# jingsenzhu/i2-sdf

Hardware: AMD Instinct MI355X
Metric: ray-samples/sec (fwd+bwd) (higher is better)
Workload: dtype f32 (bf16x3 split MFMA: fp32 operands as 3 bf16 terms, fp32 accumulate; the 256x256 weight-gradient GEMM blocks and the sampler's depth-choosing sdf-only passes: 2 bf16 terms per operand, 3 products, fp32 accumulate; the saved SDF tensors abar / G(hbar) / G(a) -- operands of those GEMMs and of the s

## Files before the change

i2sdf_amd/csrc/mlp_fwd.hip:

```cpp
#include "epi.h"
#include "mlp_args.h"

using namespace i2sdf;

int i2sdf_hip_check(hipError_t e, const char* what);
void i2sdf_launch_sdf_fwd3(int H, const float* stream, int n_stages, int L, int skip, const PointSpec& ps, const int* skip_flag, int64_t M,
                           float* sdf_out, unsigned grid, hipStream_t st);

void i2sdf_launch_sdf_fwd3h(const float* stream, int n_stages, int L, int skip, const PointSpec& ps, const int* skip_flag, int64_t M, float* sdf_out,
                            int planes, hipStream_t st);

namespace {

template <int H, int F, int LF, bool FULL>
__global__ __launch_bounds__(256) void sdf_fwd_kernel(const float* __restrict__ stream, int n_stages, int L, int skip, PointSpec ps,
                                                       const int* __restrict__ skip_flag, int64_t M, float* __restrict__ sdf_out,
                                                       float* __restrict__ feat_out, int64_t ld_feat) {
  constexpr int NT = H / 32, KC = H / 8, PEC = PE<LF>::PEC;
  extern __shared__ __attribute__((aligned(16))) float lds[];
  if (skip_flag != nullptr && skip_flag[0] != 0) return;
  const int tid = threadIdx.x, lane = tid & 63, wave = tid >> 6, hi = lane >> 5;
  const int64_t m = ((int64_t)blockIdx.x * 4 + wave) * 32 + (lane & 31);
  const bool valid = m < M;
  const int64_t mc = valid ? m : M - 1;
  float px, py, pz;
  fetch_point(ps, mc, px, py, pz);
  float pe[PEC * 4];
  {
    float full[PEC * 8];
    pe_full<LF>(px, py, pz, full);
    to_b_layout<PEC>(full, pe, hi);
  }
  WStream ws;
  ws.begin(stream, lds, n_stages, tid);
  f32x16 acc[NT];
  float h[NT * 16];
  SoftplusEpi sp{nullptr, hi, valid};
  dense_op_epi<NT, PEC, NT * 4, 0, 0, SoftplusEpi>(ws, pe, acc, sp, tid);
  commit_tiles<NT>(acc, h);
  for (int l = 1; l < L - 1; ++l) {
    if (l == skip) {
      constexpr float rs2 = RS2;
      float u[(KC + PEC) * 4];
#pragma unroll
      for (int i = 0; i < KC * 4; ++i) u[i] = h[i] * rs2;
#pragma unroll
      for (int i = 0; i < PEC * 4; ++i) u[KC * 4 + i] = pe[i] * rs2;
      dense_op_epi<NT, KC + PEC, NT * 4, 0, 0, SoftplusEpi>(ws, u, acc, sp, tid);
    } else {
      dense_op_epi<NT, KC, NT * 4, 0, 0, SoftplusEpi>(ws, h, acc, sp, tid);
    }
    commit_tiles<NT>(acc, h);
  }
  float s[1];
  rowvec_op<1, KC>(ws, h, s, tid);
  if (sdf_out != nullptr && valid && hi == 0) sdf_out[m] = s[0];
  if (FULL) {
    constexpr int FT = F / 32;
    f32x16 fa[FT];
    dense_op<FT, KC, 0>(ws, h, fa, tid);
    store_tile<FT>(feat_out + mc * ld_feat, hi, valid, fa);
  }
}

template <int H, int F, int LF>
int launch_sdf_fwd(const i2sdf_plan* p, const float* packed, PointSpec points, const int* skip_flag, int64_t M, float* sdf_out,
                   float* feat_out, int64_t ld_feat, hipStream_t st, bool sampler_pass = false) {
  const i2sdf_mlp_desc& d = p->sdf.d;
  const bool full = feat_out != nullptr;
  const unsigned grid = (unsigned)((M + PTS_PER_WG - 1) / PTS_PER_WG);
  if (!full && sdf_out != nullptr && p->sdf_fwd_bf16x3 && H == 256 && span_chunks(p->sdf, SPAN_FWD3H) > 0) {
    const int PL = (sampler_pass && p->sampler_bf16x2 && span_chunks(p->sdf, SPAN_FWD2H) > 0) ? 2 : 3;
    const Span s3 = span(p, packed, p->sdf, PL == 2 ? SPAN_FWD2H : SPAN_FWD3H_SDF);
    if (!s3.n_stages) return I2SDF_EINVAL;
    i2sdf_launch_sdf_fwd3h(s3.w, s3.n_stages, d.n_lin, d.skip_layer, points, skip_flag, M, sdf_out, PL, st);
    return i2sdf_hip_check(hipGetLastError(), "sdf_forward (bf16x3, 16-point waves) launch");
  }
  if (!full && sdf_out != nullptr && p->sdf_fwd_bf16x3 && H == 64 && span_chunks(p->sdf, SPAN_FWD3) > 0) {
    const Span s3 = span(p, packed, p->sdf, SPAN_FWD3);
    if (!s3.n_stages) return I2SDF_EINVAL;
    i2sdf_launch_sdf_fwd3(H, s3.w, s3.n_stages, d.n_lin, d.skip_layer, points, skip_flag, M, sdf_out, grid, st);
    return i2sdf_hip_check(hipGetLastError(), "sdf_forward (bf16x3) launch");
  }
  if (full && p->sdf_fwd_bf16x3 && H == 256 && F == 256 && span_chunks(p->sdf, SPAN_FWD3H) > 0) {
    const Span s3 = span(p, packed, p->sdf, SPAN_FWD3H);
    if (!s3.n_stages || skip_flag != nullptr) return I2SDF_EINVAL;
    SdfTrainFwdArgs a{};
    a.fwd = s3.w; a.n_fwd = s3.n_stages;
    a.L = d.n_lin; a.skip = d.skip_layer; a.pts = points; a.M = M; a.Mp = M; a.sdf = sdf_out; a.feat = feat_out; a.ldf = ld_feat;
    i2sdf_launch_train_fwd3h(a, grid, st);
    return i2sdf_hip_check(hipGetLastError(), "sdf_forward (features, bf16x3, 16-point waves) launch");
  }
  const Span s = span(p, packed, p->sdf, full ? SPAN_FWD : SPAN_FWD_SDF);
  if (!s.n_stages) return I2SDF_EINVAL;
  if (full)
    launch_lds(sdf_fwd_kernel<H, F, LF, true>, grid, st, s.w, s.n_stages, d.n_lin, d.skip_layer, points, skip_flag, M, sdf_out, feat_out, ld_feat);
  else
    launch_lds(sdf_fwd_kernel<H, F, LF, false>, grid, st, s.w, s.n_stages, d.n_lin, d.skip_layer, points, skip_flag, M, sdf_out, nullptr, 0);
  return i2sdf_hip_check(hipGetLastError(), "sdf_forward launch");
}

}

extern "C" int i2sdf_sdf_forward(const i2sdf_plan* p, const float* packed, const float* points, int64_t M, float* sdf_out,
                                 float* feat_out, int64_t ld_feat, void* stream) {
  if (M == 0) return I2SDF_OK;
  if (!p || !packed || !points || M < 0) return I2SDF_EINVAL;
  if (feat_out && (ld_feat < p->F || ld_feat % 4)) return I2SDF_EINVAL;
  hipStream_t st = (hipStream_t)stream;
  if (p->sdf.d.multires != 6) return I2SDF_EINVAL;
  const PointSpec ps{points, nullptr, nullptr, nullptr, 0, 0, 1};
  if (p->H == 256 && p->F == 256) return launch_sdf_fwd<256, 256, 6>(p, packed, ps, nullptr, M, sdf_out, feat_out, ld_feat, st);
  if (p->H == 64 && p->F == 64) return launch_sdf_fwd<64, 64, 6>(p, packed, ps, nullptr, M, sdf_out, feat_out, ld_feat, st);
  return I2SDF_EINVAL;
}

int i2sdf_sdf_forward_rays_flagged(const i2sdf_plan* p, const float* packed, const float* cam, const float* dirs, const float* z, int64_t ldz,
                                   int32_t n_per_ray, int64_t B, float* sdf_out, const int* skip_flag, void* stream) {
  if (p->sdf.d.multires != 6) return I2SDF_EINVAL;
  const int64_t M = B * n_per_ray;
  const PointSpec ps{nullptr, cam, dirs, z, ldz, M, n_per_ray};
  hipStream_t st = (hipStream_t)stream;
  if (p->H == 256 && p->F == 256) return launch_sdf_fwd<256, 256, 6>(p, packed, ps, skip_flag, M, sdf_out, nullptr, 0, st, true);
  if (p->H == 64 && p->F == 64) return launch_sdf_fwd<64, 64, 6>(p, packed, ps, skip_flag, M, sdf_out, nullptr, 0, st, true);
  return I2SDF_EINVAL;
}
```

i2sdf_amd/csrc/pack.hip:

```cpp
#include "plan.h"

using namespace i2sdf;

int i2sdf_hip_check(hipError_t e, const char* what);

namespace {

struct RowTab {
  int32_t n;
  int32_t rows[3 * I2SDF_MAX_LAYERS], cols[3 * I2SDF_MAX_LAYERS], scale_off[3 * I2SDF_MAX_LAYERS];
  int64_t off_v[3 * I2SDF_MAX_LAYERS], off_g[3 * I2SDF_MAX_LAYERS];
};

__global__ __launch_bounds__(256) void rowscale_kernel(RowTab tab, const float* __restrict__ params, float* __restrict__ scale,
                                                        int n_rows) {
  const int row = blockIdx.x * 4 + (threadIdx.x >> 6);
  const int lane = threadIdx.x & 63;
  if (row >= n_rows) return;
  int e = 0;
  while (e + 1 < tab.n && row >= tab.scale_off[e + 1]) ++e;
  const int r = row - tab.scale_off[e];
  const int cols = tab.cols[e];
  const float* v = params + tab.off_v[e] + (int64_t)r * cols;
  float s = 0.f;
  for (int c = lane; c < cols; c += 64) { float x = v[c]; s = fmaf(x, x, s); }
#pragma unroll
  for (int o = 32; o > 0; o >>= 1) s += __shfl_xor(s, o);
  if (lane == 0) scale[row] = params[tab.off_g[e] + r] / sqrtf(s);
}

__device__ __forceinline__ int map_col(const ColMap& cm, int kp) {
  if (kp < cm.split) return kp < cm.valid0 ? cm.base0 + kp : -1;
  const int j = kp - cm.split;
  return j < cm.valid1 ? cm.base1 + j : -1;
}

__global__ __launch_bounds__(256) void pack_kernel(const Seg* __restrict__ segs, int n_segs, const float* __restrict__ params,
                                                    const float* __restrict__ scale, float* __restrict__ chunks,
                                                    int64_t total_chunks) {
  const int64_t gid = (int64_t)blockIdx.x * 256 + threadIdx.x;
  const int64_t chunk = gid >> 6;
  const int lane = (int)(gid & 63);
  if (chunk >= total_chunks) return;
  int lo = 0, hi_ = n_segs - 1;
  while (lo < hi_) {
    const int mid = (lo + hi_ + 1) >> 1;
    if (segs[mid].chunk0 <= chunk) lo = mid; else hi_ = mid - 1;
  }
  const Seg s = segs[lo];
  const int c = (int)(chunk - s.chunk0);
  const int i32 = lane & 31, hi = lane >> 5;
  f32x4 out = {0.f, 0.f, 0.f, 0.f};
  if (c < s.used) {
    if (s.type == SEG_BIAS) {
      const int nt = c / 4, q = c % 4;
#pragma unroll
      for (int t = 0; t < 4; ++t) {
        const int r = 32 * nt + 8 * q + 4 * hi + t;
        out[t] = (r < s.nrows) ? params[s.off_bias + s.row_off + r] : 0.f;
      }
    } else if (s.type == SEG_WFWD) {
      const int nt = c / s.KC, kc = c % s.KC;
      const int r = 32 * nt + i32;
      if (r < s.nrows) {
        const int row = s.row_off + r;
        const float sc = scale[s.scale_off + row] * s.mult;
        const float* v = params + s.off_v + (int64_t)row * s.cols;
#pragma unroll
        for (int t = 0; t < 4; ++t) {
          const int col = map_col(s.cm, 8 * kc + 4 * hi + t);
          out[t] = col >= 0 ? v[col] * sc : 0.f;
        }
      }
    } else if (s.type == SEG_WFWD3) {
      const int G = s.NT / 2, w = c >> 1, e = c & 1;
      const int kc = w / (3 * G), g = (w / 3) % G, sp = w % 3;
      const int r = 32 * (2 * g + e) + i32;
      unsigned q[4] = {0u, 0u, 0u, 0u};
      if (r < s.nrows) {
        const int row = s.row_off + r;
        const float sc = scale[s.scale_off + row] * s.mult;
        const float* v = params + s.off_v + (int64_t)row * s.cols;
#pragma unroll
        for (int i = 0; i < 4; ++i) {
          float x[2];
#pragma unroll
          for (int h2 = 0; h2 < 2; ++h2) {
            const int j = 2 * i + h2;
            const int col = map_col(s.cm, 16 * kc + (j & 3) + 8 * (j >> 2) + 4 * hi);
            x[h2] = col >= 0 ? v[col] * sc : 0.f;
          }
          unsigned p0, p1, p2;
          split3_pair(x[0], x[1], p0, p1, p2);
          q[i] = sp == 0 ? p0 : (sp == 1 ? p1 : p2);
        }
      }
      out = __builtin_bit_cast(f32x4, u32x4{q[0], q[1], q[2], q[3]});
    } else if (s.type == SEG_WBWD3) {
      const int G = s.NT / 2, w = c >> 1, e = c & 1;
      const int kc = w / (3 * G), g = (w / 3) % G, sp = w % 3;
      const int col = map_col(s.cm, 32 * (2 * g + e) + i32);
      unsigned q[4] = {0u, 0u, 0u, 0u};
      if (col >= 0) {
#pragma unroll
        for (int i = 0; i < 4; ++i) {
          float x[2];
#pragma unroll
          for (int h2 = 0; h2 < 2; ++h2) {
            const int j = 2 * i + h2;
            const int r = 16 * kc + (j & 3) + 8 * (j >> 2) + 4 * hi;
            x[h2] = 0.f;
            if (r < s.nrows) {
              const int row = s.row_off + r;
              x[h2] = params[s.off_v + (int64_t)row * s.cols + col] * scale[s.scale_off + row] * s.mult;
            }
          }
          unsigned p0, p1, p2;
          split3_pair(x[0], x[1], p0, p1, p2);
          q[i] = sp == 0 ? p0 : (sp == 1 ? p1 : p2);
        }
      }
      out = __builtin_bit_cast(f32x4, u32x4{q[0], q[1], q[2], q[3]});
    } else if (s.type == SEG_BIAS_H) {
      const int kg = lane >> 4;
#pragma unroll
      for (int t = 0; t < 4; ++t) {
        const int r = 16 * c + 4 * kg + t;
        out[t] = (r < s.nrows) ? params[s.off_bias + s.row_off + r] : 0.f;
      }
    } else if (s.type == SEG_WFWD3H || s.type == SEG_WBWD3H || s.type == SEG_WFWD2H) {
      const int G = s.NT / 2, w = c >> 1, e = c & 1, PL = s.type == SEG_WFWD2H ? 2 : 3;
      const int kc = w / (PL * G), g = (w / PL) % G, sp = w % PL;
      const int i16 = lane & 15, kg = lane >> 4;
      const int arow = 16 * (2 * g + e) + i16;
      const bool fwd = s.type != SEG_WBWD3H;
      const int acol = fwd ? -1 : map_col(s.cm, arow);
      unsigned q[4] = {0u, 0u, 0u, 0u};
      if (fwd ? (arow < s.nrows) : (acol >= 0)) {
#pragma unroll
        for (int i = 0; i < 4; ++i) {
          float x[2];
#pragma unroll
          for (int h2 = 0; h2 < 2; ++h2) {
            const int j = 2 * i + h2;
            const int k = 32 * kc + 16 * (j >> 2) + 4 * kg + (j & 3);
            x[h2] = 0.f;
            if (fwd) {
              const int row = s.row_off + arow, col = map_col(s.cm, k);
              if (col >= 0) x[h2] = params[s.off_v + (int64_t)row * s.cols + col] * (scale[s.scale_off + row] * s.mult);
            } else if (k < s.nrows) {
              const int row = s.row_off + k;
              x[h2] = params[s.off_v + (int64_t)row * s.cols + acol] * scale[s.scale_off + row] * s.mult;
            }
          }
          unsigned p0, p1, p2;
          split3_pair(x[0], x[1], p0, p1, p2);
          q[i] = sp == 0 ? p0 : (sp == 1 ? p1 : p2);
        }
      }
      out = __builtin_bit_cast(f32x4, u32x4{q[0], q[1], q[2], q[3]});
    } else if (s.type == SEG_ROWVEC_H) {
      const int rr = c / s.KC, nt = c % s.KC, kg = lane >> 4;
      const int row = s.row_off + rr;
      const float sc = scale[s.scale_off + row] * s.mult;
#pragma unroll
      for (int t = 0; t < 4; ++t) {
        const int col = map_col(s.cm, 16 * nt + 4 * kg + t);
        out[t] = col >= 0 ? params[s.off_v + (int64_t)row * s.cols + col] * sc : 0.f;
      }
    } else if (s.type == SEG_WBWD) {
      const int kt = c / s.KC, nc = c % s.KC;
      const int col = map_col(s.cm, 32 * kt + i32);
      if (col >= 0) {
#pragma unroll
        for (int t = 0; t < 4; ++t) {
          const int r = 8 * nc + 4 * hi + t;
          if (r < s.nrows) {
            const int row = s.row_off + r;
            out[t] = params[s.off_v + (int64_t)row * s.cols + col] * scale[s.scale_off + row] * s.mult;
          }
        }
      }
    } else if (s.type == SEG_ROWVEC) {
      const int rr = c / s.KC, kc = c % s.KC;
      const int row = s.row_off + rr;
      const float sc = scale[s.scale_off + row] * s.mult;
#pragma unroll
      for (int t = 0; t < 4; ++t) {
        const int col = map_col(s.cm, 8 * kc + 4 * hi + t);
        out[t] = col >= 0 ? params[s.off_v + (int64_t)row * s.cols + col] * sc : 0.f;
      }
    } else if (s.type == SEG_SCALAR) {
#pragma unroll
      for (int t = 0; t < 4; ++t) out[t] = (t < s.nrows) ? params[s.off_bias + s.row_off + t] : 0.f;
    }
  }
  reinterpret_cast<f32x4*>(chunks)[chunk * 64 + lane] = out;
}

void fill_tab(RowTab& tab, const NetPlan& np) {
  for (int l = 0; l < np.d.n_lin; ++l) {
    const int e = tab.n++;
    tab.rows[e] = np.d.out_dim[l]; tab.cols[e] = np.d.in_dim[l]; tab.scale_off[e] = np.scale_off[l];
    tab.off_v[e] = np.d.off_v[l]; tab.off_g[e] = np.d.off_g[l];
  }
}

}

extern "C" int i2sdf_pack_weights(const i2sdf_plan* p, const float* params, float* packed, void* stream) {
  if (!p || !params || !packed) return I2SDF_EINVAL;
  if (!p->d_segs) return I2SDF_EHIP;
  hipStream_t st = (hipStream_t)stream;
  RowTab tab{};
  fill_tab(tab, p->sdf); fill_tab(tab, p->rgb);
  if (p->light.d.n_lin) fill_tab(tab, p->light);
  rowscale_kernel<<<cdiv(p->n_scale, 4), 256, 0, st>>>(tab, params, packed, p->n_scale);
  const int64_t threads = p->total_chunks * 64;
  pack_kernel<<<(unsigned)((threads + 255) / 256), 256, 0, st>>>(p->d_segs, p->n_segs, params, packed, packed + p->scale_floats,
                                                                 p->total_chunks);
  return i2sdf_hip_check(hipGetLastError(), "pack_weights launch");
}
```

i2sdf_amd/csrc/plan.h:

```cpp
#pragma once
#include <stdint.h>
#include <vector>
#include "../../include/i2sdf.h"
#include "x3h.h"

namespace i2sdf {

enum SegType : int32_t { SEG_ZERO = 0, SEG_BIAS = 1, SEG_WFWD = 2, SEG_WBWD = 3, SEG_ROWVEC = 4, SEG_SCALAR = 5,
                         SEG_WFWD3 = 6 ,
                         SEG_WBWD3 = 7 ,
                         SEG_BIAS_H = 8, SEG_WFWD3H = 9, SEG_WBWD3H = 10, SEG_ROWVEC_H = 11,
                         SEG_WFWD2H = 12  };

struct ColMap { int32_t split, base0, valid0, base1, valid1; };

struct Seg {
  int64_t chunk0;
  int32_t nchunks;
  int32_t type;
  int64_t off_v, off_bias;
  int32_t scale_off;
  int32_t rows, cols;
  int32_t row_off;
  int32_t nrows;
  int32_t NT, KC;
  int32_t used;
  ColMap cm;
  float mult;
};

enum Mark : int {
  FWD, FWD_HIDDEN_END, FWD_SDF_END, FWD_END,
  REV, REV_CHAIN, REV_W0, REV_END,
  FWD3, FWD3_HIDDEN_END, FWD3_END,
  REV3, REV3_CHAIN, REV3_W0, REV3_END,
  FWD3H, FWD3H_SDF_END, FWD3H_END,
  REV3H, REV3H_END,
  FWD2H, FWD2H_END,
  N_MARKS
};
struct SpanId { Mark from, to; int stage_chunks; };
constexpr SpanId SPAN_FWD_HIDDEN{FWD, FWD_HIDDEN_END, SC};
constexpr SpanId SPAN_FWD_SDF{FWD, FWD_SDF_END, SC};
constexpr SpanId SPAN_FWD{FWD, FWD_END, SC};
constexpr SpanId SPAN_REV_SWEEP2{REV, REV_W0, SC};
constexpr SpanId SPAN_REV_CHAIN{REV_CHAIN, REV_END, SC};
constexpr SpanId SPAN_REV{REV, REV_END, SC};
constexpr SpanId SPAN_FWD3_HIDDEN{FWD3, FWD3_HIDDEN_END, SC};
constexpr SpanId SPAN_FWD3{FWD3, FWD3_END, SC};
constexpr SpanId SPAN_REV3_SWEEP2{REV3, REV3_W0, SC};
constexpr SpanId SPAN_REV3_CHAIN{REV3_CHAIN, REV3_END, SC};
constexpr SpanId SPAN_FWD3H_SDF{FWD3H, FWD3H_SDF_END, SCH};
constexpr SpanId SPAN_FWD3H{FWD3H, FWD3H_END, SCH};
constexpr SpanId SPAN_REV3H{REV3H, REV3H_END, SCH};
constexpr SpanId SPAN_FWD2H{FWD2H, FWD2H_END, SCH};

struct NetPlan {
  i2sdf_mlp_desc d;
  int32_t scale_off[I2SDF_MAX_LAYERS];
  int64_t mark[N_MARKS] = {};
  int64_t wgrad_off[I2SDF_MAX_LAYERS];
  int32_t wg_rows[I2SDF_MAX_LAYERS], wg_cols[I2SDF_MAX_LAYERS];
};

}

struct i2sdf_plan {
  i2sdf_net_desc desc;
  i2sdf::NetPlan sdf, rgb, light;
  std::vector<i2sdf::Seg> segs;
  i2sdf::Seg* d_segs = nullptr;
  int32_t n_segs = 0;
  int32_t n_scale = 0;
  int64_t scale_floats = 0;
  int64_t total_chunks = 0;
  int64_t wgrad_floats = 0;
  int32_t H = 0, F = 0;
  int32_t n_cu = 256;
  int32_t rgb_bf16x3 = 0;
  int32_t sdf_bwd_bf16x3 = 0;
  int32_t train_fwd_bf16x3 = 0;
  int32_t wgrad_bf16x3 = 0;
  int32_t sdf_fwd_bf16x3 = 0;
  int32_t sampler_bf16x2 = 0;
  i2sdf_exchange exchange{nullptr, nullptr};
  int32_t dp_flags = 0;
  int32_t wgrad_bf16x2 = 0;
  int32_t blocked_saves = 0;
  int32_t saves24 = 0;
  int32_t tail_overlap = 0;
  mutable hipStream_t side = nullptr;
  mutable hipEvent_t ev_fork = nullptr, ev_join = nullptr;
  int32_t parts = 0;
  mutable hipStream_t part_st[I2SDF_MAX_PARTS - 1] = {nullptr, nullptr, nullptr};
  mutable hipEvent_t part_ev[I2SDF_MAX_PARTS] = {nullptr, nullptr, nullptr, nullptr};
  mutable int32_t chain_active = 0;
  mutable int64_t chain_M = 0;
};

namespace i2sdf {
struct Span { const float* w = nullptr; int n_stages = 0; };
inline int64_t span_chunks(const NetPlan& np, SpanId id) { return np.mark[id.to] - np.mark[id.from]; }
inline Span span(const i2sdf_plan* p, const float* packed, const NetPlan& np, SpanId id) {
  const int64_t n = span_chunks(np, id);
  if (n <= 0 || n % id.stage_chunks) return Span{};
  return Span{packed + p->scale_floats + np.mark[id.from] * CHUNK_FLOATS, (int)(n / id.stage_chunks)};
}
}

struct PartRun {
  int n = 1;
  hipStream_t st[I2SDF_MAX_PARTS];
  int64_t lo[I2SDF_MAX_PARTS], hi[I2SDF_MAX_PARTS];
  bool own = false;
};
bool i2sdf_parts_begin(const i2sdf_plan* p, hipStream_t st, int64_t M, PartRun* pr);
void i2sdf_parts_end(const i2sdf_plan* p, hipStream_t st, PartRun* pr);
void i2sdf_parts_join_all(const i2sdf_plan* p, hipStream_t st);
void i2sdf_parts_fence(const i2sdf_plan* p, hipStream_t st);
#ifndef I2SDF_WG_CH
#define I2SDF_WG_CH 2048
#endif
inline bool i2sdf_parts_on(const i2sdf_plan* p) { return p->parts >= 2; }
struct ChainGuard {
  const i2sdf_plan* p; hipStream_t st; bool on;
  ChainGuard(const i2sdf_plan* p_, hipStream_t st_, bool ranged) : p(p_), st(st_), on(!ranged && p_->chain_active != 0) {
    if (on) i2sdf_parts_join_all(p, st);
  }
  ~ChainGuard() { if (on) i2sdf_parts_fence(p, st); }
};

hipStream_t i2sdf_tail_fork(const i2sdf_plan* p, hipStream_t st);
void i2sdf_tail_join(const i2sdf_plan* p, hipStream_t st, hipStream_t side);

inline int64_t split_bulk_points(int64_t M, int n_cu) {
  const int64_t n_wg = (M + i2sdf::PTS_PER_WG - 1) / i2sdf::PTS_PER_WG;
  const int64_t full = (n_wg / n_cu) * n_cu, rem = n_wg - full;
  if (full == 0 || rem == 0 || rem * 4 > n_cu) return 0;
  if ((full * i2sdf::PTS_PER_WG) % I2SDF_WG_CH != 0) return 0;
  return full * i2sdf::PTS_PER_WG;
}

enum TailOrder { TAIL_FORKED, TAIL_BEHIND };
template <class Full, class Tail>
inline void i2sdf_dispatch_points(const i2sdf_plan* p, hipStream_t st, int64_t M, bool ranged, bool may_split, TailOrder order, Full full, Tail tail) {
  constexpr int64_t WG = i2sdf::PTS_PER_WG;
  if (ranged) {
    PartRun pr;
    i2sdf_parts_begin(p, st, M, &pr);
    for (int q = 0; q < pr.n; ++q)
      if (pr.hi[q] > pr.lo[q]) full(pr.st[q], (int)(pr.lo[q] / WG), (unsigned)((pr.hi[q] - pr.lo[q] + WG - 1) / WG), M);
    i2sdf_parts_end(p, st, &pr);
    return;
  }
  const int64_t bulk = may_split ? split_bulk_points(M, p->n_cu) : 0;
  if (bulk == 0) {
    full(st, 0, (unsigned)((M + WG - 1) / WG), M);
  } else if (order == TAIL_FORKED) {
    hipStream_t ts = i2sdf_tail_fork(p, st);
    tail(ts, bulk);
    full(st, 0, (unsigned)(bulk / WG), bulk);
    i2sdf_tail_join(p, st, ts);
  } else {
    full(st, 0, (unsigned)(bulk / WG), bulk);
    tail(st, bulk);
  }
}
```

i2sdf_amd/csrc/sampler.hip:

```cpp
#include "plan.h"

using namespace i2sdf;

int i2sdf_hip_check(hipError_t e, const char* what);

namespace {

constexpr int NMAX = 640;
constexpr int NNEW = 128;
constexpr int EMAX = NMAX / 64;

enum { ST_DONE = 0, ST_ITERS = 1, ST_FLAG0 = 2 , ST_CNT0 = 16 , ST_WORDS = 32 };

#ifndef SAMPLER_DPP
#define SAMPLER_DPP 1
#endif
template <int CTRL, int ROW_MASK>
__device__ __forceinline__ float dpp_mov(float old, float v) {
  return __builtin_bit_cast(float, __builtin_amdgcn_update_dpp(__builtin_bit_cast(int, old), __builtin_bit_cast(int, v), CTRL, ROW_MASK, 0xf, false));
}
constexpr int DPP_ROW_SHR1 = 0x111, DPP_ROW_SHR2 = 0x112, DPP_ROW_SHR4 = 0x114, DPP_ROW_SHR8 = 0x118, DPP_ROW_BCAST15 = 0x142, DPP_ROW_BCAST31 = 0x143;
__device__ __forceinline__ float wscan_incl(float v, int lane) {
#if SAMPLER_DPP
  (void)lane;
  v += dpp_mov<DPP_ROW_SHR1, 0xf>(0.f, v);
  v += dpp_mov<DPP_ROW_SHR2, 0xf>(0.f, v);
  v += dpp_mov<DPP_ROW_SHR4, 0xf>(0.f, v);
  v += dpp_mov<DPP_ROW_SHR8, 0xf>(0.f, v);
  v += dpp_mov<DPP_ROW_BCAST15, 0xa>(0.f, v);
  v += dpp_mov<DPP_ROW_BCAST31, 0xc>(0.f, v);
  return v;
#else
#pragma unroll
  for (int o = 1; o < 64; o <<= 1) {
    const float t = __shfl_up(v, o);
    if (lane >= o) v += t;
  }
  return v;
#endif
}
__device__ __forceinline__ float wsum(float v) {
#if SAMPLER_DPP
  return __builtin_bit_cast(float, __builtin_amdgcn_readlane(__builtin_bit_cast(int, wscan_incl(v, 0)), 63));
#else
#pragma unroll
  for (int o = 32; o > 0; o >>= 1) v += __shfl_xor(v, o);
  return v;
#endif
}
__device__ __forceinline__ float wmax(float v) {
#if SAMPLER_DPP
  const float lo = -3.4028234663852886e38f;
  v = fmaxf(v, dpp_mov<DPP_ROW_SHR1, 0xf>(lo, v));
  v = fmaxf(v, dpp_mov<DPP_ROW_SHR2, 0xf>(lo, v));
  v = fmaxf(v, dpp_mov<DPP_ROW_SHR4, 0xf>(lo, v));
  v = fmaxf(v, dpp_mov<DPP_ROW_SHR8, 0xf>(lo, v));
  v = fmaxf(v, dpp_mov<DPP_ROW_BCAST15, 0xa>(lo, v));
  v = fmaxf(v, dpp_mov<DPP_ROW_BCAST31, 0xc>(lo, v));
  return __builtin_bit_cast(float, __builtin_amdgcn_readlane(__builtin_bit_cast(int, v), 63));
#else
#pragma unroll
  for (int o = 32; o > 0; o >>= 1) v = fmaxf(v, __shfl_xor(v, o));
  return v;
#endif
}
template <int E>
__device__ __forceinline__ void row_scan_incl(float (&v)[E], int lane) {
#pragma unroll
  for (int e = 1; e < E; ++e) v[e] += v[e - 1];
  const float tot = v[E - 1];
  const float pre = wscan_incl(tot, lane) - tot;
#pragma unroll
  for (int e = 0; e < E; ++e) v[e] += pre;
}

__device__ __forceinline__ float laplace_density(float s, float inv_beta) {
  const float e = expm1f(-fabsf(s) * inv_beta);
  const float sg = (s > 0.f) ? 1.f : ((s < 0.f) ? -1.f : 0.f);
  return inv_beta * (0.5f + 0.5f * sg * e);
}

template <int E>
struct Row {
  float z[E], s[E];
  float a[E], ds[E];
  int n;
};

template <int E>
__device__ __forceinline__ void row_intervals(Row<E>& r, int lane) {
  const float zn_next = __shfl_down(r.z[0], 1), sn_next = __shfl_down(r.s[0], 1);
#pragma unroll
  for (int e = 0; e < E; ++e) {
    const int j = lane * E + e;
    const float z1 = (e + 1 < E) ? r.z[(e + 1 < E) ? e + 1 : e] : zn_next;
    const float s1 = (e + 1 < E) ? r.s[(e + 1 < E) ? e + 1 : e] : sn_next;
    float a = 0.f, d = 0.f;
    if (j < r.n - 1) {
      a = z1 - r.z[e];
      const float b = fabsf(r.s[e]), c = fabsf(s1);
      const bool first = a * a + b * b <= c * c;
      const bool second = a * a + c * c <= b * b;
      const float sp = (a + b + c) / 2.0f;
      const float area = sp * (sp - a) * (sp - b) * (sp - c);
      const bool mask = !first && !second && (b + c - a > 0.f);
      float h = (2.0f * sqrtf(area)) / a;
      if (!(h == h)) h = 0.f;
      else if (h > 3.4028234663852886e38f) h = 3.4028234663852886e38f;
      else if (h < -3.4028234663852886e38f) h = -3.4028234663852886e38f;
      d = ((first && !second) ? b : 0.f) + (second ? c : 0.f) + (mask ? h : 0.f);
      const float sg0 = (r.s[e] > 0.f) ? 1.f : ((r.s[e] < 0.f) ? -1.f : 0.f);
      const float sg1 = (s1 > 0.f) ? 1.f : ((s1 < 0.f) ? -1.f : 0.f);
      if (!(sg0 * sg1 == 1.f)) d = 0.f;
    }
    r.a[e] = a; r.ds[e] = d;
  }
}

template <int E>
__device__ __forceinline__ float row_error_bound(const Row<E>& r, float beta, int lane) {
  const float ib = 1.0f / beta;
  float fe[E], er[E];
#pragma unroll
  for (int e = 0; e < E; ++e) {
    const int j = lane * E + e;
    const bool ok = j < r.n - 1;
    fe[e] = ok ? r.a[e] * laplace_density(r.s[e], ib) : 0.f;
    er[e] = ok ? expf(-r.ds[e] / beta) * (r.a[e] * r.a[e]) / (4.0f * beta * beta) : 0.f;
  }
  float fi[E], ei[E];
#pragma unroll
  for (int e = 0; e < E; ++e) { fi[e] = fe[e]; ei[e] = er[e]; }
  row_scan_incl<E>(fi, lane);
  row_scan_incl<E>(ei, lane);
  float mx = -3.4e38f;
#pragma unroll
  for (int e = 0; e < E; ++e) {
    const int j = lane * E + e;
    if (j < r.n - 1) {
      const float integ = fi[e] - fe[e];
      const float bo = (fminf(expf(ei[e]), 1.0e6f) - 1.0f) * expf(-integ);
      mx = fmaxf(mx, bo);
    }
  }
  return wmax(mx);
}

struct SamplerArgs {
  int64_t B;
  int it, n, n_new;
  int N_eval, N_final, max_iters, beta_iters, force_iters;
  float eps, add_tiny, near, far;
  const float* beta_param; float beta_min;
  int* state;
  float* z_cur; float* z_nxt;
  float* sdf_prev; float* sdf_cur;
  const int* idx;
  int* idx_nxt;
  const float* sdf_new;
  float* samples;
  float* beta;
  const float* u_more; const float* u_final; int64_t ldu_final;
};

template <int E>
__device__ __forceinline__ void load_row(Row<E>& r, const float* z, const float* s, int n, int lane) {
  r.n = n;
#pragma unroll
  for (int e = 0; e < E; ++e) {
    const int j = lane * E + e;
    r.z[e] = (j < n) ? z[j] : 3.0e38f;
    r.s[e] = (j < n) ? s[j] : 0.f;
  }
}

template <int E>
__device__ __forceinline__ float beta_step(const SamplerArgs& a, Row<E>& r, int64_t rc, bool active, int lane) {
  const float beta0 = fabsf(a.beta_param[0]) + a.beta_min;
  const int n = a.n;
  float* sc = a.sdf_cur + rc * NMAX;
  const float* zc = a.z_cur + rc * NMAX;
  r.n = n;
  {
    const int n_old = n - a.n_new;
    const int* ix = a.idx + rc * NMAX;
    const float* sp = a.sdf_prev + rc * NMAX;
    const float* sn = a.sdf_new + rc * a.n_new;
#pragma unroll
    for (int e = 0; e < E; ++e) {
      const int j = lane * E + e;
      float sv = 0.f, zv = 3.0e38f;
      if (j < n) {
        zv = zc[j];
        if (a.it == 0) sv = sn[j];
        else { const int k = ix[j]; sv = (k < n_old) ? sp[k] : sn[k - n_old]; }
        if (active) sc[j] = sv;
      }
      r.z[e] = zv; r.s[e] = sv;
    }
  }
  row_intervals<E>(r, lane);
  float beta = a.beta[rc];
  const float err0 = row_error_bound<E>(r, beta0, lane);
  if (err0 <= a.eps) beta = beta0;
  float bmin = beta0, bmax = beta;
  for (int k = 0; k < a.beta_iters; ++k) {
    const float bmid = (bmin + bmax) / 2.0f;
    const float err = row_error_bound<E>(r, bmid, lane);
    if (err <= a.eps) bmax = bmid; else bmin = bmid;
  }
  return bmax;
}
template <int E>
__global__ __launch_bounds__(256) void sampler_beta_kernel(SamplerArgs a) {
  if (a.state[ST_DONE]) return;
  const int lane = threadIdx.x & 63;
  const int64_t ray = (int64_t)blockIdx.x * 4 + (threadIdx.x >> 6);
  if (ray >= a.B) return;
  Row<E> r;
  const float beta = beta_step<E>(a, r, ray, true, lane);
  if (lane == 0) {
    a.beta[ray] = beta;
    if (beta > fabsf(a.beta_param[0]) + a.beta_min) atomicOr(&a.state[ST_FLAG0 + a.it], 1);
  }
}

template <int E>
__device__ __forceinline__ void resample_step(const SamplerArgs& a, const Row<E>& r, float beta, bool more, int64_t ray, int64_t rc, bool active,
                                              float (&s_cdf)[4][NMAX + 1], float (&s_z)[4][NMAX], float (&s_new)[4][NNEW], int lane, int wv) {
  const int n = a.n;
  const float ib = 1.0f / beta;
  float fe[E], cum[E];
#pragma unroll
  for (int e = 0; e < E; ++e) {
    const int j = lane * E + e;
    const float dist = (j < n - 1) ? r.a[e] : 1.0e10f;
    fe[e] = (j < n) ? dist * laplace_density(r.s[e], ib) : 0.f;
    cum[e] = (j < n - 1) ? fe[e] : 0.f;
  }
  row_scan_incl<E>(cum, lane);
  float pdf[E];
  if (more) {
    float er[E];
#pragma unroll
    for (int e = 0; e < E; ++e) {
      const int j = lane * E + e;
      er[e] = (j < n - 1) ? expf(-r.ds[e] / beta) * (r.a[e] * r.a[e]) / (4.0f * beta * beta) : 0.f;
    }
    row_scan_incl<E>(er, lane);
#pragma unroll
    for (int e = 0; e < E; ++e) {
      const int j = lane * E + e;
      const float T = expf(-(cum[e] - ((j < n - 1) ? fe[e] : 0.f)));
      pdf[e] = (j < n - 1) ? (fminf(expf(er[e]), 1.0e6f) - 1.0f) * T + a.add_tiny : 0.f;
    }
  } else {
#pragma unroll
    for (int e = 0; e < E; ++e) {
      const int j = lane * E + e;
      const float T = expf(-(cum[e] - ((j < n - 1) ? fe[e] : 0.f)));
      const float w = (1.0f - expf(-fe[e])) * T;
      pdf[e] = (j < n - 1) ? w + 1e-5f : 0.f;
    }
  }
  float tot = 0.f;
#pragma unroll
  for (int e = 0; e < E; ++e) tot += pdf[e];
  tot = wsum(tot);
  float cd[E];
#pragma unroll
  for (int e = 0; e < E; ++e) { pdf[e] = pdf[e] / tot; cd[e] = pdf[e]; }
  row_scan_incl<E>(cd, lane);
#pragma unroll
  for (int e = 0; e < E; ++e) {
    const int j = lane * E + e;
    if (j < n) { s_cdf[wv][j] = cd[e] - pdf[e]; s_z[wv][j] = r.z[e]; }
  }
  __syncthreads();
  const int N = more ? a.N_eval : a.N_final;
  for (int k = lane; k < N; k += 64) {
    float u;
    if (more) u = a.u_more[k];
    else u = a.u_final[rc * a.ldu_final + k];
    int lo = 0, hi = n;
    while (lo < hi) {
      const int mid = (lo + hi) >> 1;
      if (s_cdf[wv][mid] <= u) lo = mid + 1; else hi = mid;
    }
    const int below = (lo - 1 > 0) ? lo - 1 : 0;
    const int above = (lo < n - 1) ? lo : n - 1;
    const float c0 = s_cdf[wv][below], c1 = s_cdf[wv][above];
    const float b0 = s_z[wv][below], b1 = s_z[wv][above];
    float denom = c1 - c0;
    if (denom < 1e-5f) denom = 1.0f;
    const float t = (u - c0) / denom;
    const float smp = b0 + t * (b1 - b0);
    s_new[wv][k] = smp;
    if (active) a.samples[ray * NNEW + k] = smp;
  }
  __syncthreads();
  if (!more) return;
  if (active) {
    float* zn = a.z_nxt + ray * NMAX;
    int* ixn = a.idx_nxt + ray * NMAX;
    for (int j = lane; j < n; j += 64) {
      const float v = s_z[wv][j];
      int lo = 0, hi = N;
      while (lo < hi) { const int mid = (lo + hi) >> 1; if (s_new[wv][mid] < v) lo = mid + 1; else hi = mid; }
      zn[j + lo] = v; ixn[j + lo] = j;
    }
    for (int k = lane; k < N; k += 64) {
      const float v = s_new[wv][k];
      int lo = 0, hi = n;
      while (lo < hi) { const int mid = (lo + hi) >> 1; if (s_z[wv][mid] <= v) lo = mid + 1; else hi = mid; }
      zn[k + lo] = v; ixn[k + lo] = n + k;
    }
  }
}

__device__ __forceinline__ void iteration_done(const SamplerArgs& a, bool more) {
  __syncthreads();
  if (threadIdx.x == 0) {
    __threadfence();
    const int c = atomicAdd(&a.state[ST_CNT0 + a.it], 1);
    if (c == (int)gridDim.x - 1 && !more) { a.state[ST_ITERS] = a.it + 1; __threadfence(); a.state[ST_DONE] = 1; }
  }
}

template <int E>
__global__ __launch_bounds__(256) void sampler_resample_kernel(SamplerArgs a) {
  __shared__ float s_cdf[4][NMAX + 1];
  __shared__ float s_z[4][NMAX];
  __shared__ float s_new[4][NNEW];
  if (a.state[ST_DONE]) return;
  const int lane = threadIdx.x & 63, wv = threadIdx.x >> 6;
  const int64_t ray = (int64_t)blockIdx.x * 4 + wv;
  const bool active = ray < a.B;
  const int64_t rc = active ? ray : a.B - 1;
  bool not_conv = a.state[ST_FLAG0 + a.it] != 0;
  if (a.force_iters > 0) not_conv = (a.it + 1) < a.force_iters;
  const bool more = not_conv && (a.it + 1 < a.max_iters);
  Row<E> r;
  load_row<E>(r, a.z_cur + rc * NMAX, a.sdf_cur + rc * NMAX, a.n, lane);
  row_intervals<E>(r, lane);
  resample_step<E>(a, r, a.beta[rc], more, ray, rc, active, s_cdf, s_z, s_new, lane, wv);
  iteration_done(a, more);
}

template <int E>
__global__ __launch_bounds__(256) void sampler_iter_fixed_kernel(SamplerArgs a) {
  __shared__ float s_cdf[4][NMAX + 1];
  __shared__ float s_z[4][NMAX];
  __shared__ float s_new[4][NNEW];
  const int lane = threadIdx.x & 63, wv = threadIdx.x >> 6;
  const int64_t ray = (int64_t)blockIdx.x * 4 + wv;
  const bool active = ray < a.B;
  const int64_t rc = active ? ray : a.B - 1;
  const bool more = ((a.it + 1) < a.force_iters) && (a.it + 1 < a.max_iters);
  Row<E> r;
  const float beta = beta_step<E>(a, r, rc, active, lane);
  if (active && lane == 0) a.beta[ray] = beta;
  resample_step<E>(a, r, beta, more, ray, rc, active, s_cdf, s_z, s_new, lane, wv);
  iteration_done(a, more);
}

__global__ __launch_bounds__(256) void sampler_init_kernel(int64_t B, int N, const float* __restrict__ t_lin, const float* __restrict__ strat_u,
                                                            float near, float far, float eps, float* __restrict__ z_cur,
                                                            float* __restrict__ samples, float* __restrict__ beta, int* __restrict__ state) {
  const int lane = threadIdx.x & 63;
  const int64_t ray = (int64_t)blockIdx.x * 4 + (threadIdx.x >> 6);
  if (blockIdx.x == 0 && threadIdx.x < ST_WORDS) state[threadIdx.x] = 0;
  if (ray >= B) return;
  float acc = 0.f, carry = 0.f;
  for (int base = 0; base < N; base += 64) {
    const int j = base + lane;
    float z = 0.f;
    if (j < N) {
      const float t = t_lin[j];
      z = near * (1.0f - t) + far * t;
      if (strat_u) {
        const float tm = t_lin[j > 0 ? j - 1 : 0], tp = t_lin[j < N - 1 ? j + 1 : N - 1];
        const float zm = near * (1.0f - tm) + far * tm, zq = near * (1.0f - tp) + far * tp;
        const float lower = (j > 0) ? 0.5f * (z + zm) : z;
        const float upper = (j < N - 1) ? 0.5f * (zq + z) : z;
        z = lower + (upper - lower) * strat_u[ray * N + j];
      }
      z_cur[ray * NMAX + j] = z;
      samples[ray * NNEW + j] = z;
    }
    float zp = __shfl_up(z, 1);
    if (lane == 0) zp = carry;
    if (j < N && j > 0) { const float d = z - zp; acc = fmaf(d, d, acc); }
    carry = __shfl(z, 63);
  }
  acc = wsum(acc);
  if (lane == 0) beta[ray] = sqrtf((1.0f / (4.0f * logf(eps + 1.0f))) * acc);
}

__global__ __launch_bounds__(256) void sampler_final_kernel(int64_t B, const int* __restrict__ state, int N_eval, const float* z_a,
                                                             const float* z_b, const float* __restrict__ samples, int N_final, int N_extra,
                                                             const int* __restrict__ extra_idx, const int* __restrict__ extra_tab,
                                                             float near, float far, const int* __restrict__ eik_idx, float* __restrict__ z_out,
                                                             int64_t ldz, float* __restrict__ z_eik, int* __restrict__ iters_out) {
  __shared__ float buf[4][256];
  const int lane = threadIdx.x & 63, wv = threadIdx.x >> 6;
  const int64_t ray = (int64_t)blockIdx.x * 4 + wv;
  const bool active = ray < B;
  const int64_t rc = active ? ray : B - 1;
  const int iters = state[ST_ITERS];
  if (iters_out != nullptr && blockIdx.x == 0 && threadIdx.x == 0) iters_out[0] = iters;
  const int n_row = N_eval * iters;
  const float* zr = ((iters & 1) ? z_a : z_b) + rc * NMAX;
  const int total = N_final + 2 + N_extra;
  for (int k = lane; k < 256; k += 64) {
    float v = 3.0e38f;
    if (k < N_final) v = samples[rc * NNEW + k];
    else if (k == N_final) v = near;
    else if (k == N_final + 1) v = far;
    else if (k < total) {
      const int e = k - N_final - 2;
      int id;
      if (extra_idx) id = extra_idx[(iters - 1) * N_extra + e];
      else id = extra_tab[(iters - 1) * N_extra + e];
      id = id < 0 ? 0 : (id > n_row - 1 ? n_row - 1 : id);
      v = zr[id];
    }
    buf[wv][k] = v;
  }
  __syncthreads();
  for (int k = 2; k <= 256; k <<= 1) {
    for (int j = k >> 1; j > 0; j >>= 1) {
      for (int i = lane; i < 256; i += 64) {
        const int l = i ^ j;
        if (l > i) {
          const float x = buf[wv][i], y = buf[wv][l];
          const bool up = (i & k) == 0;
          if ((x > y) == up) { buf[wv][i] = y; buf[wv][l] = x; }
        }
      }
      __syncthreads();
    }
  }
  if (active) {
    for (int k = lane; k < total; k += 64) z_out[ray * ldz + k] = buf[wv][k];
    if (lane == 0 && z_eik) {
      int id = eik_idx ? eik_idx[ray] : 0;
      id = id < 0 ? 0 : (id > total - 1 ? total - 1 : id);
      z_eik[ray] = buf[wv][id];
    }
  }
}

template <int E>
__global__ __launch_bounds__(256) void error_bound_kernel(int64_t B, int n, const float* __restrict__ z, const float* __restrict__ sdf,
                                                           const float* __restrict__ beta, int64_t ldbeta, const float* __restrict__ d_star_in,
                                                           float* __restrict__ d_star_out, float* __restrict__ bound) {
  const int lane = threadIdx.x & 63;
  const int64_t ray = (int64_t)blockIdx.x * 4 + (threadIdx.x >> 6);
  if (ray >= B) return;
  Row<E> r;
  load_row<E>(r, z + ray * n, sdf + ray * n, n, lane);
  row_intervals<E>(r, lane);
#pragma unroll
  for (int e = 0; e < E; ++e) {
    const int j = lane * E + e;
    if (j < n - 1) {
      if (d_star_in) r.ds[e] = d_star_in[ray * (n - 1) + j];
      if (d_star_out) d_star_out[ray * (n - 1) + j] = r.ds[e];
    }
  }
  if (bound) {
    const float eb = row_error_bound<E>(r, beta[ray * ldbeta], lane);
    if (lane == 0) bound[ray] = eb;
  }
}

template <int E>
int launch_iter(const SamplerArgs& a, hipStream_t st, const i2sdf_exchange* ex) {
  const unsigned grid = (unsigned)((a.B + 3) / 4);
  if (a.force_iters > 0 && !ex) {
    sampler_iter_fixed_kernel<E><<<grid, 256, 0, st>>>(a);
    return I2SDF_OK;
  }
  sampler_beta_kernel<E><<<grid, 256, 0, st>>>(a);
  if (ex) {
    const int rc = ex->allreduce(ex->ctx, a.state + ST_FLAG0 + a.it, 1, I2SDF_XCHG_I32, I2SDF_XCHG_MAX, (void*)st);
    if (rc) return rc;
  }
  sampler_resample_kernel<E><<<grid, 256, 0, st>>>(a);
  return I2SDF_OK;
}

}

extern "C" int64_t i2sdf_sampler_workspace_floats(int64_t B) {
  return B * (int64_t)(NMAX * 6 + NNEW * 2 + 1) + ST_WORDS + 64;
}

extern "C" int i2sdf_error_bound(const float* z, const float* sdf, int64_t B, int32_t n, const float* beta, int64_t ldbeta,
                                 const float* d_star_in, float* d_star_out, float* bound, void* stream) {
  if (B == 0) return I2SDF_OK;
  if (!z || !sdf || B < 0 || n < 2 || n > NMAX || (bound && !beta) || (!bound && !d_star_out) || (ldbeta != 0 && ldbeta != 1)) return I2SDF_EINVAL;
  hipStream_t st = (hipStream_t)stream;
  const unsigned grid = (unsigned)((B + 3) / 4);
#define I2SDF_EB(E_) error_bound_kernel<E_><<<grid, 256, 0, st>>>(B, n, z, sdf, beta, ldbeta, d_star_in, d_star_out, bound)
  switch (cdiv(n, 64)) {
    case 1: I2SDF_EB(1); break;
    case 2: I2SDF_EB(2); break;
    case 3: I2SDF_EB(3); break;
    case 4: I2SDF_EB(4); break;
    case 5: I2SDF_EB(5); break;
    case 6: I2SDF_EB(6); break;
    case 7: I2SDF_EB(7); break;
    case 8: I2SDF_EB(8); break;
    case 9: I2SDF_EB(9); break;
    default: I2SDF_EB(10); break;
  }
#undef I2SDF_EB
  return i2sdf_hip_check(hipGetLastError(), "error_bound launch");
}

int i2sdf_sdf_forward_rays_flagged(const i2sdf_plan* p, const float* packed, const float* cam, const float* dirs, const float* z, int64_t ldz,
                                   int32_t n_per_ray, int64_t B, float* sdf_out, const int* skip_flag, void* stream);

extern "C" int i2sdf_sample_rays(const i2sdf_plan* p, const float* packed, const float* params, const i2sdf_sampler_cfg* sc,
                                 const float* cam, const float* dirs, int64_t B, int32_t training, const float* t_lin, const float* u_more,
                                 const float* u_final, int64_t ldu_final, const int32_t* extra_tab, const float* strat_u,
                                 const int32_t* extra_idx, const int32_t* eik_idx, int32_t force_iters, float* workspace, float* z_out,
                                 int64_t ldz, float* z_eik, int32_t* iters_out, void* stream) {
  if (B == 0) return I2SDF_OK;
  if (!p || !packed || !params || !sc || !cam || !dirs || !t_lin || !u_more || !u_final || !workspace || !z_out || B < 0) return I2SDF_EINVAL;
  if (sc->N_samples_eval > NNEW || sc->N_samples > NNEW || sc->N_samples_eval * sc->max_total_iters > NMAX || sc->max_total_iters > 12)
    return I2SDF_EINVAL;
  if (sc->N_samples + 2 + sc->N_samples_extra > 256 || ldz < sc->N_samples + 2 + sc->N_samples_extra) return I2SDF_EINVAL;
  if (training && (!strat_u || (sc->N_samples_extra > 0 && !extra_idx))) return I2SDF_EINVAL;
  if (!training && sc->N_samples_extra > 0 && !extra_tab) return I2SDF_EINVAL;
  hipStream_t st = (hipStream_t)stream;
  float* w = workspace;
  float* zA = w; w += B * NMAX;
  float* zB = w; w += B * NMAX;
  float* sA = w; w += B * NMAX;
  float* sB = w; w += B * NMAX;
  int* iA = (int*)w; w += B * NMAX;
  int* iB = (int*)w; w += B * NMAX;
  float* samples = w; w += B * NNEW;
  float* sdf_new = w; w += B * NNEW;
  float* beta = w; w += B;
  int* state = (int*)w;
  const float near = sc->near, far = 2.0f * p->desc.scene_bounding_sphere;
  const unsigned grid = (unsigned)((B + 3) / 4);
  const i2sdf_exchange* gcomm = (training && p->exchange.allreduce && (p->dp_flags & I2SDF_DP_GLOBAL_SAMPLER) && force_iters <= 0) ? &p->exchange : nullptr;
  sampler_init_kernel<<<grid, 256, 0, st>>>(B, sc->N_samples_eval, t_lin, training ? strat_u : nullptr, near, far, sc->eps, zA, samples, beta, state);
  const int n_it = (force_iters > 0 && force_iters < sc->max_total_iters) ? force_iters : sc->max_total_iters;
  for (int it = 0; it < n_it; ++it) {
    const int n_new = sc->N_samples_eval;
    int rc = i2sdf_sdf_forward_rays_flagged(p, packed, cam, dirs, samples, NNEW, n_new, B, sdf_new, state + ST_DONE, stream);
    if (rc) return rc;
    SamplerArgs a{};
    a.B = B; a.it = it; a.n = sc->N_samples_eval * (it + 1); a.n_new = n_new;
    a.N_eval = sc->N_samples_eval; a.N_final = sc->N_samples; a.max_iters = sc->max_total_iters; a.beta_iters = sc->beta_iters;
    a.force_iters = force_iters;
    a.eps = sc->eps; a.add_tiny = sc->add_tiny; a.near = near; a.far = far;
    a.beta_param = params + p->desc.off_beta; a.beta_min = p->desc.beta_min;
    a.state = state;
    const bool even = (it & 1) == 0;
    a.z_cur = even ? zA : zB; a.z_nxt = even ? zB : zA;
    a.sdf_cur = even ? sA : sB; a.sdf_prev = even ? sB : sA;
    a.idx = even ? iB : iA; a.idx_nxt = even ? iA : iB;
    a.sdf_new = sdf_new; a.samples = samples; a.beta = beta;
    a.u_more = u_more; a.u_final = u_final; a.ldu_final = ldu_final;
    const int E = cdiv(a.n, 64);
    int xrc = I2SDF_OK;
    switch (E) {
      case 1: xrc = launch_iter<1>(a, st, gcomm); break;
      case 2: xrc = launch_iter<2>(a, st, gcomm); break;
      case 3: xrc = launch_iter<3>(a, st, gcomm); break;
      case 4: xrc = launch_iter<4>(a, st, gcomm); break;
      case 5: xrc = launch_iter<5>(a, st, gcomm); break;
      case 6: xrc = launch_iter<6>(a, st, gcomm); break;
      case 7: xrc = launch_iter<7>(a, st, gcomm); break;
      case 8: xrc = launch_iter<8>(a, st, gcomm); break;
      case 9: xrc = launch_iter<9>(a, st, gcomm); break;
      default: xrc = launch_iter<10>(a, st, gcomm); break;
    }
    if (xrc) return xrc;
  }
  sampler_final_kernel<<<grid, 256, 0, st>>>(B, state, sc->N_samples_eval, zA, zB, samples, sc->N_samples, sc->N_samples_extra,
                                             training ? (const int*)extra_idx : nullptr, (const int*)extra_tab, near, far, (const int*)eik_idx, z_out, ldz,
                                             z_eik, iters_out);
  return i2sdf_hip_check(hipGetLastError(), "sample_rays launch");
}
```

i2sdf_amd/csrc/wgrad.hip:

```cpp
#include <algorithm>
#include <stdlib.h>
#include "mlp_common.h"

using namespace i2sdf;

int i2sdf_hip_check(hipError_t e, const char* what);

namespace {

#ifndef WGN_AUX
#define WGN_AUX 2
#endif
#ifndef W3_NT_LD
#define W3_NT_LD 1
#endif
#ifndef W3_RAW_SETS
#define W3_RAW_SETS 1
#endif
#ifndef W3_P24_NT
#define W3_P24_NT 0
#endif
constexpr int WG_CH = I2SDF_WG_CH;
constexpr int PFW = 6;
constexpr int MAX_TASKS = 30;

struct WgJob { const float* A; const float* B; int32_t lda, ldb, a_w, b_w; int64_t m_count; int64_t a_blk, b_blk; int32_t a_c0, b_c0; int32_t a_p24, b_p24; };
struct WgTask {
  WgJob j[2];
  int32_t njobs, relu_b, has_bias, rows_store, cols_store, ldo;
  int32_t variant, pad;
  int64_t out_off, bias_off;
};
struct WgLaunch { WgTask t[MAX_TASKS]; int32_t n; int32_t chunk0; int64_t chunk_stride; float* partials; };

template <int AM, int BM, int PF>
__device__ __forceinline__ void wgrad_accumulate(const WgTask& t, int64_t lo, int64_t hi_cap, int lane,
                                                 f32x16 (&acc)[AM ? 1 : 4][BM ? BM : 4], float (&bsum)[AM ? 1 : 4]) {
  constexpr int TA = AM ? 1 : 4, TB = BM ? BM : 4;
  const int i32 = lane & 31, hi = lane >> 5;
#pragma unroll
  for (int a = 0; a < TA; ++a)
#pragma unroll
    for (int b = 0; b < TB; ++b)
#pragma unroll
      for (int r = 0; r < 16; ++r) acc[a][b][r] = 0.f;
#pragma unroll
  for (int a = 0; a < TA; ++a) bsum[a] = 0.f;
  for (int jb = 0; jb < t.njobs; ++jb) {
    const WgJob job = t.j[jb];
    const int64_t m_lo = lo;
    const int64_t m_hi = (hi_cap < job.m_count) ? hi_cap : job.m_count;
    if (m_hi <= m_lo) continue;
    const int npairs = (int)((m_hi - m_lo + 1) / 2);
    const int rows = (int)(m_hi - m_lo);
    const __amdgpu_buffer_rsrc_t ra = __builtin_amdgcn_make_buffer_rsrc(const_cast<float*>(job.A + m_lo * job.lda), 0,
                                                                      rows * job.lda * 4, 0x00020000);
    const __amdgpu_buffer_rsrc_t rb = __builtin_amdgcn_make_buffer_rsrc(const_cast<float*>(job.B + m_lo * job.ldb), 0,
                                                                      rows * job.ldb * 4, 0x00020000);
    const unsigned OOB = 0x7fffffffu;
    const int a_col = AM ? i32 : 4 * i32;
    const unsigned a_off = (a_col < job.a_w) ? (unsigned)((hi * job.lda + a_col) * 4) : OOB;
    unsigned b_off[BM ? BM : 1];
    if (BM) {
#pragma unroll
      for (int tb = 0; tb < (BM ? BM : 1); ++tb) b_off[tb] = (i32 + 32 * tb < job.b_w) ? (unsigned)((hi * job.ldb + i32 + 32 * tb) * 4) : OOB;
    } else {
      b_off[0] = (4 * i32 < job.b_w) ? (unsigned)((hi * job.ldb + 4 * i32) * 4) : OOB;
    }
    const unsigned a_step = 2u * job.lda * 4u, b_step = 2u * job.ldb * 4u;
    const bool ablk = !AM && m_lo < job.a_blk, bblk = !BM && m_lo < job.b_blk;
    const unsigned a_cb = ablk ? (unsigned)((((job.a_c0 + 4 * i32) >> 4) * 512 + ((4 * i32) & 15)) * 4) : (unsigned)((job.a_c0 + 4 * i32) * 4);
    const unsigned b_cb = bblk ? (unsigned)((((job.b_c0 + 4 * i32) >> 4) * 512 + ((4 * i32) & 15)) * 4) : (unsigned)((job.b_c0 + 4 * i32) * 4);
    const __amdgpu_buffer_rsrc_t ra_b = __builtin_amdgcn_make_buffer_rsrc(const_cast<float*>(job.A - job.a_c0 + m_lo * job.lda), 0, 0x7ffffff0, 0x00020000);
    const __amdgpu_buffer_rsrc_t rb_b = __builtin_amdgcn_make_buffer_rsrc(const_cast<float*>(job.B - job.b_c0 + m_lo * job.ldb), 0, 0x7ffffff0, 0x00020000);
    auto off16 = [&](unsigned cb, bool is_blk, unsigned ld, unsigned pn, bool col_ok) -> unsigned {
      const unsigned r = 2u * pn + (unsigned)hi;
      const unsigned ro = is_blk ? ((r >> 5) * 8192u + (r & 31u) * 16u) * 4u : r * ld * 4u;
      return (col_ok && (int)r < rows) ? cb + ro : OOB;
    };
    const float relu_lo = t.relu_b != 0 ? 0.f : -3.0e38f;
    const float bias_w = (t.has_bias && jb == 0) ? 1.f : 0.f;
    float a0[PF][TA], b0[PF][TB], a1[PF][TA], b1[PF][TB];
    auto ldw = [&](const __amdgpu_buffer_rsrc_t& rs, unsigned off, unsigned add) -> float {
      return __builtin_bit_cast(float, __builtin_amdgcn_raw_buffer_load_b32(rs, off == OOB ? OOB : off + add, 0, 0));
    };
    auto load_group = [&](float (&A)[PF][TA], float (&Bv)[PF][TB], unsigned pbase) {
#pragma unroll
      for (int u = 0; u < PF; ++u) {
        const unsigned pn = pbase + u;
        if (AM) A[u][0] = ldw(ra, a_off, pn * a_step);
        else {
          const f32x4 x = __builtin_bit_cast(f32x4, __builtin_amdgcn_raw_buffer_load_b128(ra_b, off16(a_cb, ablk, (unsigned)job.lda, pn, a_off != OOB), 0, 0));
#pragma unroll
          for (int q = 0; q < TA; ++q) A[u][q] = x[q];
        }
        if (BM) {
#pragma unroll
          for (int tb = 0; tb < TB; ++tb) Bv[u][tb] = ldw(rb, b_off[tb < (BM ? BM : 1) ? tb : 0], pn * b_step);
        } else {
          const f32x4 x = __builtin_bit_cast(f32x4, __builtin_amdgcn_raw_buffer_load_b128(rb_b, off16(b_cb, bblk, (unsigned)job.ldb, pn, b_off[0] != OOB), 0, 0));
#pragma unroll
          for (int q = 0; q < TB; ++q) Bv[u][q] = x[q];
        }
      }
    };
    auto compute_group = [&](const float (&A)[PF][TA], const float (&Bv)[PF][TB]) {
#pragma unroll
      for (int u = 0; u < PF; ++u) {
        float bq[TB];
#pragma unroll
        for (int tb = 0; tb < TB; ++tb) bq[tb] = fmaxf(Bv[u][tb], relu_lo);
#pragma unroll
        for (int ta = 0; ta < TA; ++ta) bsum[ta] = fmaf(A[u][ta], bias_w, bsum[ta]);
#pragma unroll
        for (int ta = 0; ta < TA; ++ta)
#pragma unroll
          for (int tb = 0; tb < TB; ++tb) acc[ta][tb] = mfma(A[u][ta], bq[tb], acc[ta][tb]);
      }
    };
    load_group(a0, b0, 0);
    for (int p = 0; p < npairs; p += 2 * PF) {
      load_group(a1, b1, (unsigned)(p + PF));
      __builtin_amdgcn_sched_barrier(0);
      compute_group(a0, b0);
      __builtin_amdgcn_sched_barrier(0);
      load_group(a0, b0, (unsigned)(p + 2 * PF));
      __builtin_amdgcn_sched_barrier(0);
      compute_group(a1, b1);
      __builtin_amdgcn_sched_barrier(0);
    }
  }
}

#define W3_ALL_AGPRS "a0","a1","a2","a3","a4","a5","a6","a7","a8","a9","a10","a11","a12","a13","a14","a15","a16","a17","a18","a19","a20","a21","a22","a23","a24","a25","a26","a27","a28","a29","a30","a31","a32","a33","a34","a35","a36","a37","a38","a39","a40","a41","a42","a43","a44","a45","a46","a47","a48","a49","a50","a51","a52","a53","a54","a55","a56","a57","a58","a59","a60","a61","a62","a63","a64","a65","a66","a67","a68","a69","a70","a71","a72","a73","a74","a75","a76","a77","a78","a79","a80","a81","a82","a83","a84","a85","a86","a87","a88","a89","a90","a91","a92","a93","a94","a95","a96","a97","a98","a99","a100","a101","a102","a103","a104","a105","a106","a107","a108","a109","a110","a111","a112","a113","a114","a115","a116","a117","a118","a119","a120","a121","a122","a123","a124","a125","a126","a127","a128","a129","a130","a131","a132","a133","a134","a135","a136","a137","a138","a139","a140","a141","a142","a143","a144","a145","a146","a147","a148","a149","a150","a151","a152","a153","a154","a155","a156","a157","a158","a159","a160","a161","a162","a163","a164","a165","a166","a167","a168","a169","a170","a171","a172","a173","a174","a175","a176","a177","a178","a179","a180","a181","a182","a183","a184","a185","a186","a187","a188","a189","a190","a191","a192","a193","a194","a195","a196","a197","a198","a199","a200","a201","a202","a203","a204","a205","a206","a207","a208","a209","a210","a211","a212","a213","a214","a215","a216","a217","a218","a219","a220","a221","a222","a223","a224","a225","a226","a227","a228","a229","a230","a231","a232","a233","a234","a235","a236","a237","a238","a239","a240","a241","a242","a243","a244","a245","a246","a247","a248","a249","a250","a251","a252","a253","a254","a255"
__device__ __forceinline__ void w3_mfma(int k, f32x16& c, u32x4 a, u32x4 b) {
  (void)c;
  asm volatile("v_mfma_f32_32x32x16_bf16 a[%0:%1], %2, %3, a[%0:%1]" :: "n"(16 * k), "n"(16 * k + 15), "v"(a), "v"(b) : W3_ALL_AGPRS);
}
__device__ __forceinline__ void w3_acc_zero() {
  asm volatile(".set w3i, 0\n.rept 256\n\tv_accvgpr_write_b32 a[w3i], 0\n\t.set w3i, w3i+1\n.endr" ::: W3_ALL_AGPRS);
}
__device__ __forceinline__ float w3_acc_read(int n) {
  float x;
  asm volatile("v_accvgpr_read_b32 %0, a[%1]" : "=v"(x) : "n"(n));
  return x;
}
__device__ __forceinline__ void w3_mfma_drain() {
  asm volatile("s_nop 15\n\ts_nop 15" ::: "memory");
}
__device__ __forceinline__ void w3_mfma_valu(int k, u32x4 a, u32x4 b) {
  asm volatile("s_nop 1\n\tv_mfma_f32_32x32x16_bf16 a[%0:%1], %2, %3, a[%0:%1]" :: "n"(16 * k), "n"(16 * k + 15), "v"(a), "v"(b) : W3_ALL_AGPRS);
}

template <int AM, int BM, int NPL, bool A24 = false>
__device__ __forceinline__ void wgrad_accumulate_x_core(const WgTask& t, int64_t lo, int64_t hi_cap, int lane, float (&bsum)[AM ? 1 : 4]) {
  constexpr int TA = AM ? 1 : 4, TB = BM ? BM : 4, NBV = BM ? BM : 1;
  const int i32 = lane & 31, hi = lane >> 5;
  w3_acc_zero();
#pragma unroll
  for (int a = 0; a < TA; ++a) bsum[a] = 0.f;
  for (int jb = 0; jb < t.njobs; ++jb) {
    const WgJob job = t.j[jb];
    const int64_t m_lo = lo;
    const int64_t m_hi = (hi_cap < job.m_count) ? hi_cap : job.m_count;
    if (m_hi <= m_lo) continue;
    const int rows = (int)(m_hi - m_lo);
    const int nst = (rows + 15) / 16;
    const unsigned OOB = 0x7fffffffu;
    const bool ablk = !AM && m_lo < job.a_blk, bblk = !BM && m_lo < job.b_blk;
    constexpr bool a24 = A24 && !AM;
    const __amdgpu_buffer_rsrc_t ra = __builtin_amdgcn_make_buffer_rsrc(const_cast<float*>(job.A - (AM ? 0 : job.a_c0) + m_lo * (a24 ? P24_BLOCK / 32 : job.lda)), 0, 0x7ffffff0, 0x00020000);
    const __amdgpu_buffer_rsrc_t rb = __builtin_amdgcn_make_buffer_rsrc(const_cast<float*>(job.B - (BM ? 0 : job.b_c0) + m_lo * job.ldb), 0, 0x7ffffff0, 0x00020000);
    const char* pa24 = reinterpret_cast<const char*>(job.A - (AM ? 0 : job.a_c0) + m_lo * (P24_BLOCK / 32));
    unsigned aoff[8], boff[8][NBV], amid_k = 0;
    auto p24_offs = [&](unsigned col, unsigned c, unsigned& oh, unsigned& mid_k) __attribute__((always_inline)) {
      const unsigned kc = col >> 4, q = (col >> 2) & 3u;
      oh = (kc * P24_KCS + c * 8u + (q & 1u) * 4u + (q >> 1) * 2u) * 4u;
      mid_k = (kc * P24_KCS * 4u >> 1) + P24_MID * 4u;
    };
#pragma unroll
    for (int q = 0; q < 8; ++q) {
      const unsigned c = (unsigned)(2 * q + hi);
      if (AM) aoff[q] = (i32 < job.a_w) ? (c * (unsigned)job.lda + (unsigned)i32) * 4u : OOB;
      else {
        const unsigned col = (unsigned)(job.a_c0 + 4 * i32);
        aoff[q] = (4 * i32 < job.a_w) ? (ablk ? ((col >> 4) * 512u + (col & 15u) + c * 16u) * 4u : (c * (unsigned)job.lda + col) * 4u) : OOB;
        if (a24) p24_offs(col, c, aoff[q], amid_k);
      }
      if (BM) {
#pragma unroll
        for (int tb = 0; tb < NBV; ++tb) boff[q][tb] = (i32 + 32 * tb < job.b_w) ? (c * (unsigned)job.ldb + (unsigned)(i32 + 32 * tb)) * 4u : OOB;
      } else {
        const unsigned col = (unsigned)(job.b_c0 + 4 * i32);
        boff[q][0] = (4 * i32 < job.b_w) ? (bblk ? ((col >> 4) * 512u + (col & 15u) + c * 16u) * 4u : (c * (unsigned)job.ldb + col) * 4u) : OOB;
      }
    }
    auto stage_off = [&](int s, bool blk, int ld) -> unsigned {
      return blk ? (unsigned)(((s >> 1) * 8192 + (s & 1) * 256) * 4) : (unsigned)(s * 16 * ld * 4);
    };
    auto stage_off24 = [&](int s, int part) -> unsigned { return part == 0 ? (unsigned)(((s >> 1) * P24_BLOCK + (s & 1) * 128) * 4) : (unsigned)((s >> 1) * P24_BLOCK * 2); };
    const float relu_lo = t.relu_b != 0 ? 0.f : -3.0e38f;
    const float bias_w = (t.has_bias && jb == 0) ? 1.f : 0.f;
    float A0[8][TA], B0[8][TB], A1[8][TA], B1[8][TB];
    auto load_stage = [&](float (&A)[8][TA], float (&Bv)[8][TB], int s) __attribute__((always_inline)) {
      const unsigned sa = stage_off(s, ablk, job.lda), sb = stage_off(s, bblk, job.ldb);
      if (!AM && a24) {
        const unsigned sh = stage_off24(s, 0), sm = stage_off24(s, 1);
#pragma unroll
        for (int q = 0; q < 8; ++q) {
          const f32x2 hh = *reinterpret_cast<const f32x2*>(pa24 + (sh + aoff[q]));
          A[q][0] = hh[0]; A[q][1 % TA] = hh[1];
          A[q][2 % TA] = *reinterpret_cast<const float*>(pa24 + sm + (((aoff[q] + sh) >> 1) + amid_k));
        }
      }
#pragma unroll
      for (int q = 0; q < 8; ++q) {
        if (AM) A[q][0] = __builtin_bit_cast(float, __builtin_amdgcn_raw_buffer_load_b32(ra, aoff[q], sa, WGN_AUX));
        else if (!a24) {
          const f32x4 x = __builtin_bit_cast(f32x4, __builtin_amdgcn_raw_buffer_load_b128(ra, aoff[q], sa, WGN_AUX));
#pragma unroll
          for (int ta = 0; ta < TA; ++ta) A[q][ta] = x[ta];
        }
        if (BM) {
#pragma unroll
          for (int tb = 0; tb < TB; ++tb) Bv[q][tb] = __builtin_bit_cast(float, __builtin_amdgcn_raw_buffer_load_b32(rb, boff[q][tb < NBV ? tb : 0], sb, WGN_AUX));
        } else {
          const f32x4 x = __builtin_bit_cast(f32x4, __builtin_amdgcn_raw_buffer_load_b128(rb, boff[q][0], sb, WGN_AUX));
#pragma unroll
          for (int tb = 0; tb < TB; ++tb) Bv[q][tb] = x[tb];
        }
      }
    };
    auto unpack24 = [&](float (&X)[4]) __attribute__((always_inline)) {
      const unsigned h0 = __builtin_bit_cast(unsigned, X[0]), h1 = __builtin_bit_cast(unsigned, X[1]), mm = __builtin_bit_cast(unsigned, X[2]);
      X[0] = __builtin_bit_cast(float, __builtin_amdgcn_perm(h0, mm, 0x0504000cu));
      X[1] = __builtin_bit_cast(float, __builtin_amdgcn_perm(h0, mm, 0x0706010cu));
      X[2] = __builtin_bit_cast(float, __builtin_amdgcn_perm(h1, mm, 0x0504020cu));
      X[3] = __builtin_bit_cast(float, __builtin_amdgcn_perm(h1, mm, 0x0706030cu));
    };
    auto split = [&](const float (&X)[8], u32x4 (&pl)[NPL]) __attribute__((always_inline)) {
#pragma unroll
      for (int i = 0; i < 4; ++i) {
        if (NPL == 2) { unsigned p0, p1; split2_pair(X[2 * i], X[2 * i + 1], p0, p1); pl[0][i] = p0; pl[1][i] = p1; }
        else { unsigned p0, p1, p2; split3_pair(X[2 * i], X[2 * i + 1], p0, p1, p2); pl[0][i] = p0; pl[1][i] = p1; pl[NPL - 1][i] = p2; }
      }
    };
    auto compute_stage = [&](float (&A)[8][TA], float (&Bv)[8][TB], int nv) __attribute__((always_inline)) {
      if constexpr (!AM) {
        if (a24) {
#pragma unroll
          for (int q = 0; q < 8; ++q) unpack24(A[q]);
        }
      }
      if (nv < 16) {
#pragma unroll
        for (int q = 0; q < 8; ++q) {
          const bool ok = 2 * q + hi < nv;
#pragma unroll
          for (int ta = 0; ta < TA; ++ta) A[q][ta] = ok ? A[q][ta] : 0.f;
#pragma unroll
          for (int tb = 0; tb < TB; ++tb) Bv[q][tb] = ok ? Bv[q][tb] : 0.f;
        }
      }
      u32x4 pa[TA][NPL], pb[TB][NPL];
#pragma unroll
      for (int ta = 0; ta < TA; ++ta) {
        float x[8];
#pragma unroll
        for (int q = 0; q < 8; ++q) { x[q] = A[q][ta]; bsum[ta] = fmaf(x[q], bias_w, bsum[ta]); }
        split(x, pa[ta]);
      }
#pragma unroll
      for (int tb = 0; tb < TB; ++tb) {
        float x[8];
#pragma unroll
        for (int q = 0; q < 8; ++q) x[q] = fmaxf(Bv[q][tb], relu_lo);
        split(x, pb[tb]);
      }
#pragma unroll
      for (int pa_i = 0; pa_i < NPL; ++pa_i)
#pragma unroll
        for (int pb_i = 0; pb_i < NPL; ++pb_i) {
          if (pa_i + pb_i >= NPL) continue;
#pragma unroll
          for (int ta = 0; ta < TA; ++ta)
#pragma unroll
            for (int tb = 0; tb < TB; ++tb) w3_mfma_valu(ta + 4 * tb, pa[ta][pa_i], pb[tb][pb_i]);
        }
    };
    load_stage(A0, B0, 0);
    for (int s = 0; s < nst; s += 2) {
      load_stage(A1, B1, s + 1 < nst ? s + 1 : nst - 1);
      __builtin_amdgcn_sched_barrier(0);
      compute_stage(A0, B0, rows - 16 * s);
      __builtin_amdgcn_sched_barrier(0);
      load_stage(A0, B0, s + 2 < nst ? s + 2 : nst - 1);
      __builtin_amdgcn_sched_barrier(0);
      if (s + 1 < nst) compute_stage(A1, B1, rows - 16 * (s + 1));
      __builtin_amdgcn_sched_barrier(0);
    }
  }
  w3_mfma_drain();
}
template <int AM, int BM, int NPL>
__device__ __forceinline__ void wgrad_accumulate_x(const WgTask& t, int64_t lo, int64_t hi_cap, int lane,
                                                   f32x16 (&acc)[AM ? 1 : 4][BM ? BM : 4], float (&bsum)[AM ? 1 : 4]) {
  constexpr int TA = AM ? 1 : 4, TB = BM ? BM : 4;
  wgrad_accumulate_x_core<AM, BM, NPL>(t, lo, hi_cap, lane, bsum);
#pragma unroll
  for (int ta = 0; ta < TA; ++ta)
#pragma unroll
    for (int tb = 0; tb < TB; ++tb)
#pragma unroll
      for (int r = 0; r < 16; ++r) acc[ta][tb][r] = w3_acc_read(16 * (ta + 4 * tb) + r);
}

template <int AM, int BM>
__device__ __forceinline__ void wgrad_store(const WgTask& t, float* __restrict__ out, int lane,
                                            const f32x16 (&acc)[AM ? 1 : 4][BM ? BM : 4], float (&bsum)[AM ? 1 : 4]) {
  constexpr int TA = AM ? 1 : 4, TB = BM ? BM : 4;
  const int i32 = lane & 31, hi = lane >> 5;
#pragma unroll
  for (int ta = 0; ta < TA; ++ta)
#pragma unroll
    for (int r = 0; r < 16; ++r) {
      const int ri = (r & 3) + 8 * (r >> 2) + 4 * hi;
      const int n = AM ? ri : 4 * ri + ta;
      if (n < t.rows_store) {
        if (BM) {
#pragma unroll
          for (int tb = 0; tb < TB; ++tb)
            if (i32 + 32 * tb < t.cols_store) out[t.out_off + (int64_t)n * t.ldo + i32 + 32 * tb] = acc[ta][tb][r];
        } else if (4 * i32 < t.cols_store) {
          const f32x4 v = {acc[ta][0][r], acc[ta][1][r], acc[ta][2][r], acc[ta][3][r]};
          *reinterpret_cast<f32x4*>(out + t.out_off + (int64_t)n * t.ldo + 4 * i32) = v;
        }
      }
    }
  if (t.has_bias) {
#pragma unroll
    for (int ta = 0; ta < TA; ++ta) bsum[ta] += __shfl_xor(bsum[ta], 32);
    if (hi == 0) {
      if (AM) { if (i32 < t.rows_store) out[t.bias_off + i32] = bsum[0]; }
      else if (4 * i32 < t.rows_store) *reinterpret_cast<f32x4*>(out + t.bias_off + 4 * i32) = f32x4{bsum[0], bsum[TA > 1 ? 1 : 0], bsum[TA > 2 ? 2 : 0], bsum[TA > 3 ? 3 : 0]};
    }
  }
}

template <int AM, int BM>
__global__ __launch_bounds__(64) void wgrad_kernel(WgLaunch L) {
  constexpr int TA = AM ? 1 : 4, TB = BM ? BM : 4;
  const int lane = threadIdx.x & 63;
  const WgTask& t = L.t[blockIdx.y];
  const int64_t chunk = blockIdx.x + L.chunk0;
  f32x16 acc[TA][TB];
  float bsum[TA];
  wgrad_accumulate<AM, BM, PFW>(t, chunk * WG_CH, chunk * WG_CH + WG_CH, lane, acc, bsum);
  wgrad_store<AM, BM>(t, L.partials + chunk * L.chunk_stride, lane, acc, bsum);
}

constexpr int PFN = 8;
constexpr int WGW_SLOT = (16 * 16 + 4) * 64;
constexpr int WGN_LDS_BYTES = 2 * WGW_SLOT * 4;

template <int AM, int BM, int NPL, bool A24 = false>
__device__ __forceinline__ void wgrad_narrow_body(const WgLaunch& L, const WgTask& t, int64_t chunk, int wave, int lane, float* lds) {
  constexpr int TA = AM ? 1 : 4, TB = BM ? BM : 4, NW = TA * TB * 16 + TA;
  const int64_t lo = chunk * WG_CH + wave * (WG_CH / 4);
  if constexpr (NPL != 0 && BM != 0) {
    float bsum[TA];
    wgrad_accumulate_x_core<AM, BM, NPL == 0 ? 2 : NPL, A24>(t, lo, lo + WG_CH / 4, lane, bsum);
    if (wave > 0) {
      float* dst = lds + (wave - 1) * NW * 64 + lane;
#pragma unroll
      for (int a = 0; a < TA; ++a)
#pragma unroll
        for (int b = 0; b < TB; ++b) {
#pragma unroll
          for (int r = 0; r < 16; ++r) dst[((a * TB + b) * 16 + r) * 64] = w3_acc_read(16 * (a + 4 * b) + r);
          __builtin_amdgcn_sched_barrier(0);
        }
#pragma unroll
      for (int a = 0; a < TA; ++a) dst[(TA * TB * 16 + a) * 64] = bsum[a];
    }
    __syncthreads();
    if (wave == 0) {
      const int i32 = lane & 31, hi = lane >> 5;
      float* out = L.partials + chunk * L.chunk_stride;
#pragma unroll
      for (int a = 0; a < TA; ++a)
#pragma unroll
        for (int b = 0; b < TB; ++b) {
          float x[16];
#pragma unroll
          for (int r = 0; r < 16; ++r) x[r] = w3_acc_read(16 * (a + 4 * b) + r);
#pragma unroll
          for (int w = 0; w < 3; ++w)
#pragma unroll
            for (int r = 0; r < 16; ++r) x[r] += lds[(w * NW + (a * TB + b) * 16 + r) * 64 + lane];
          if (i32 + 32 * b < t.cols_store) {
#pragma unroll
            for (int r = 0; r < 16; ++r) {
              const int ri = (r & 3) + 8 * (r >> 2) + 4 * hi, n = AM ? ri : 4 * ri + a;
              if (n < t.rows_store) out[t.out_off + (int64_t)n * t.ldo + i32 + 32 * b] = x[r];
            }
          }
          __builtin_amdgcn_sched_barrier(0);
        }
      if (t.has_bias) {
#pragma unroll
        for (int w = 0; w < 3; ++w)
#pragma unroll
          for (int a = 0; a < TA; ++a) bsum[a] += lds[(w * NW + TA * TB * 16 + a) * 64 + lane];
#pragma unroll
        for (int a = 0; a < TA; ++a) bsum[a] += __shfl_xor(bsum[a], 32);
        if (hi == 0) {
          if (AM) { if (i32 < t.rows_store) out[t.bias_off + i32] = bsum[0]; }
          else if (4 * i32 < t.rows_store) *reinterpret_cast<f32x4*>(out + t.bias_off + 4 * i32) = f32x4{bsum[0], bsum[TA > 1 ? 1 : 0], bsum[TA > 2 ? 2 : 0], bsum[TA > 3 ? 3 : 0]};
        }
      }
    }
    return;
  }
  f32x16 acc[TA][TB];
  float bsum[TA];
  if (NPL == 0) wgrad_accumulate<AM, BM, PFN>(t, lo, lo + WG_CH / 4, lane, acc, bsum);
  else wgrad_accumulate_x<AM, BM, NPL == 0 ? 2 : NPL>(t, lo, lo + WG_CH / 4, lane, acc, bsum);
  if (wave > 0) {
    float* dst = lds + (wave - 1) * NW * 64 + lane;
#pragma unroll
    for (int a = 0; a < TA; ++a)
#pragma unroll
      for (int b = 0; b < TB; ++b) {
#pragma unroll
        for (int r = 0; r < 16; ++r) dst[((a * TB + b) * 16 + r) * 64] = acc[a][b][r];
        __builtin_amdgcn_sched_barrier(0);
      }
#pragma unroll
    for (int a = 0; a < TA; ++a) dst[(TA * TB * 16 + a) * 64] = bsum[a];
  }
  __syncthreads();
  if (wave == 0) {
#pragma unroll
    for (int a = 0; a < TA; ++a)
#pragma unroll
      for (int b = 0; b < TB; ++b) {
#pragma unroll
        for (int w = 0; w < 3; ++w)
#pragma unroll
          for (int r = 0; r < 16; ++r) acc[a][b][r] += lds[(w * NW + (a * TB + b) * 16 + r) * 64 + lane];
        __builtin_amdgcn_sched_barrier(0);
      }
#pragma unroll
    for (int w = 0; w < 3; ++w)
#pragma unroll
      for (int a = 0; a < TA; ++a) bsum[a] += lds[(w * NW + TA * TB * 16 + a) * 64 + lane];
    wgrad_store<AM, BM>(t, L.partials + chunk * L.chunk_stride, lane, acc, bsum);
  }
}

template <int NPL>
__device__ __forceinline__ void wgrad_wide_body(const WgLaunch& L, const WgTask& t, int64_t chunk, int wave, int lane, float* lds) {
  float bsum[4];
  const int64_t lo = chunk * WG_CH + wave * (WG_CH / 4);
  wgrad_accumulate_x_core<0, 0, NPL>(t, lo, lo + WG_CH / 4, lane, bsum);
  if (wave >= 2) {
    float* d = lds + (wave - 2) * WGW_SLOT + lane;
#pragma unroll
    for (int k = 0; k < 16; ++k)
#pragma unroll
      for (int r = 0; r < 16; ++r) d[(k * 16 + r) * 64] = w3_acc_read(16 * k + r);
#pragma unroll
    for (int a = 0; a < 4; ++a) d[(256 + a) * 64] = bsum[a];
  }
  __syncthreads();
  if (wave == 1) {
    float* d = lds + WGW_SLOT + lane;
#pragma unroll
    for (int k = 0; k < 16; ++k)
#pragma unroll
      for (int r = 0; r < 16; ++r) d[(k * 16 + r) * 64] += w3_acc_read(16 * k + r);
#pragma unroll
    for (int a = 0; a < 4; ++a) d[(256 + a) * 64] += bsum[a];
  }
  __syncthreads();
  if (wave == 0) {
    const float* s0 = lds + lane;
    const float* s1 = lds + WGW_SLOT + lane;
    const int i32 = lane & 31, hi = lane >> 5;
    float* out = L.partials + chunk * L.chunk_stride;
#pragma unroll
    for (int ta = 0; ta < 4; ++ta) {
#pragma unroll
      for (int r = 0; r < 16; ++r) {
        f32x4 v;
#pragma unroll
        for (int tb = 0; tb < 4; ++tb) {
          const int k = ta + 4 * tb;
          v[tb] = (w3_acc_read(16 * (ta + 4 * tb) + r) + s0[(k * 16 + r) * 64]) + s1[(k * 16 + r) * 64];
        }
        const int ri = (r & 3) + 8 * (r >> 2) + 4 * hi, n = 4 * ri + ta;
        if (n < t.rows_store && 4 * i32 < t.cols_store) *reinterpret_cast<f32x4*>(out + t.out_off + (int64_t)n * t.ldo + 4 * i32) = v;
      }
      __builtin_amdgcn_sched_barrier(0);
    }
    if (t.has_bias) {
#pragma unroll
      for (int a = 0; a < 4; ++a) {
        bsum[a] = (bsum[a] + s0[(256 + a) * 64]) + s1[(256 + a) * 64];
        bsum[a] += __shfl_xor(bsum[a], 32);
      }
      if (hi == 0 && 4 * i32 < t.rows_store) *reinterpret_cast<f32x4*>(out + t.bias_off + 4 * i32) = f32x4{bsum[0], bsum[1], bsum[2], bsum[3]};
    }
  }
}

template <int NPL>
__global__ __launch_bounds__(256) void wgrad_narrow_kernel(WgLaunch L) {
  extern __shared__ __attribute__((aligned(16))) float wgn_lds[];
  const int lane = threadIdx.x & 63, wave = __builtin_amdgcn_readfirstlane(threadIdx.x >> 6);
  const WgTask& t = L.t[blockIdx.y];
  const int64_t chunk = blockIdx.x + L.chunk0;
  if (NPL != 0 && t.variant == 0) wgrad_wide_body<NPL == 0 ? 3 : NPL>(L, t, chunk, wave, lane, wgn_lds);
  else if (t.variant == 1) wgrad_narrow_body<1, 0, NPL>(L, t, chunk, wave, lane, wgn_lds);
  else if (t.variant == 2) { if (NPL != 0 && t.j[0].a_p24) wgrad_narrow_body<0, 1, NPL, NPL != 0>(L, t, chunk, wave, lane, wgn_lds); else wgrad_narrow_body<0, 1, NPL>(L, t, chunk, wave, lane, wgn_lds); }
  else { if (NPL != 0 && t.j[0].a_p24) wgrad_narrow_body<0, 2, NPL, NPL != 0>(L, t, chunk, wave, lane, wgn_lds); else wgrad_narrow_body<0, 2, NPL>(L, t, chunk, wave, lane, wgn_lds); }
}

constexpr int W3_PTS = 16;

constexpr int W3P_PL = 4 * 4 * 3 * 256;
constexpr int W3P_SLOTS = 2;
constexpr int W3P_LDS_BYTES = W3P_SLOTS * W3P_PL * 4;

template <int LAY, int NPL, bool PLAIN>
__device__ __forceinline__ void w3p_job(const WgTask& t, const WgJob& job, int jb, int64_t chunk, float* plb, float (&bsum)[4], int w, int lane) {
  const int wa = w >> 1, wb = w & 1, i32 = lane & 31, kg = lane >> 5;
  const bool opB = (w >> 1) != 0;
  f32x16 acc_unused;
  {
    const int64_t m_lo = chunk * WG_CH;
    const int64_t m_hi = (m_lo + WG_CH < job.m_count) ? m_lo + WG_CH : job.m_count;
    const int rows = (int)(m_hi - m_lo);
    const int nst = (rows + W3_PTS - 1) / W3_PTS;
    const int dld = opB ? job.ldb : job.lda;
    constexpr bool blk = LAY != 0, P24 = LAY == 2;
    const float* ubase = P24 ? (opB ? job.B - job.b_c0 : job.A - job.a_c0) + m_lo * (P24_BLOCK / 32) + (8 * wb) * P24_KCS
                       : blk ? (opB ? job.B - job.b_c0 : job.A - job.a_c0) + m_lo * 256 + (8 * wb) * 512
                             : (opB ? job.B : job.A) + m_lo * dld + 128 * wb;
    unsigned voff[4];
    unsigned voffm[P24 ? 4 : 1];
    const unsigned vnext = 2u * 4u * (unsigned)(P24 ? 8 : (blk ? 16 : dld));
#pragma unroll
    for (int i = 0; i < 4; ++i) {
      const int r = 4 * i + kg;
      voff[i] = 4u * (unsigned)(P24 ? (i32 >> 2) * P24_KCS + r * 8 + (i32 & 1) * 4 + ((i32 >> 1) & 1) * 2
                                    : (blk ? r * 16 + (i32 >> 2) * 512 + 4 * (i32 & 3) : r * dld + 4 * i32));
      if (P24) voffm[i] = 4u * (unsigned)((i32 >> 2) * P24_KCS + P24_MID + r * 4 + (i32 & 1) * 2 + ((i32 >> 1) & 1));
    }
    const float relu_lo = (opB && t.relu_b != 0) ? 0.f : -3.0e38f;
    const float bias_w = (!opB && t.has_bias != 0 && jb == 0) ? 1.f : 0.f;
    constexpr int RS = W3_RAW_SETS;
    f32x4 rlo[RS][P24 ? 1 : 4], rhi[RS][P24 ? 1 : 4];
    u32x2 hlo[RS][P24 ? 4 : 1], hhi[RS][P24 ? 4 : 1];
    unsigned mlo[RS][P24 ? 4 : 1], mhi[RS][P24 ? 4 : 1];
    auto gload = [&](int st, int s, int i, int half) __attribute__((always_inline)) {
      const int sc = s < nst ? s : nst - 1;
      if constexpr (P24) {
        const int64_t sblk = (int64_t)(sc >> 1) * P24_BLOCK;
        const char* sh = reinterpret_cast<const char*>(ubase + sblk + (sc & 1) * 128) + voff[i];
        const char* sm = reinterpret_cast<const char*>(ubase + sblk + (sc & 1) * 64) + voffm[i];
#if W3_P24_NT
        if (half == 0) { hlo[st][i] = __builtin_nontemporal_load(reinterpret_cast<const u32x2*>(sh)); mlo[st][i] = __builtin_nontemporal_load(reinterpret_cast<const unsigned*>(sm)); }
        else { hhi[st][i] = __builtin_nontemporal_load(reinterpret_cast<const u32x2*>(sh + vnext)); mhi[st][i] = __builtin_nontemporal_load(reinterpret_cast<const unsigned*>(sm + vnext / 2)); }
#else
        if (half == 0) { hlo[st][i] = *reinterpret_cast<const u32x2*>(sh); mlo[st][i] = *reinterpret_cast<const unsigned*>(sm); }
        else { hhi[st][i] = *reinterpret_cast<const u32x2*>(sh + vnext); mhi[st][i] = *reinterpret_cast<const unsigned*>(sm + vnext / 2); }
#endif
      } else {
      const int64_t soff = blk ? (int64_t)(sc >> 1) * 8192 + (sc & 1) * 256 : (int64_t)sc * W3_PTS * dld;
      const char* src = reinterpret_cast<const char*>(ubase + soff) + voff[i];
#if W3_NT_LD
      if (half == 0) rlo[st][i] = __builtin_nontemporal_load(reinterpret_cast<const f32x4*>(src));
      else rhi[st][i] = __builtin_nontemporal_load(reinterpret_cast<const f32x4*>(src + vnext));
#else
      if (half == 0) rlo[st][i] = *reinterpret_cast<const f32x4*>(src);
      else rhi[st][i] = *reinterpret_cast<const f32x4*>(src + vnext);
#endif
      }
    };
    auto raw_lo = [&](int st, int i, int tt) __attribute__((always_inline)) -> float {
      if constexpr (P24) return p24_quad_value(hlo[st][i], mlo[st][i], tt);
      else return rlo[st][i][tt];
    };
    auto raw_hi = [&](int st, int i, int tt) __attribute__((always_inline)) -> float {
      if constexpr (P24) return p24_quad_value(hhi[st][i], mhi[st][i], tt);
      else return rhi[st][i][tt];
    };
    unsigned pl[4][NPL][4];
    auto prep = [&](int s, int i, float lo, float hi_, float& x0, float& x1) __attribute__((always_inline)) {
      if (PLAIN) { x0 = lo; x1 = hi_; return; }
      const int p0 = s * W3_PTS + (4 * i + kg);
      x0 = p0 < rows ? fmaxf(lo, relu_lo) : 0.f;
      x1 = p0 + (2) < rows ? fmaxf(hi_, relu_lo) : 0.f;
    };
    auto write_tile = [&](int so, int tt, int p) __attribute__((always_inline)) {
      float* dst = plb + so + w * (4 * 3 * 256) + lane * 4;
      *reinterpret_cast<u32x4*>(dst + (tt * 3 + p) * 256) = u32x4{pl[tt][p][0], pl[tt][p][1], pl[tt][p][2], pl[tt][p][3]};
    };
    auto plane = [&](int so, int quarter, int tile, int p) __attribute__((always_inline)) -> u32x4 {
      return *reinterpret_cast<const u32x4*>(plb + so + quarter * (4 * 3 * 256) + (tile * 3 + p) * 256 + lane * 4);
    };
    auto load_all = [&](int st, int s) __attribute__((always_inline)) {
#pragma unroll
      for (int i = 0; i < 4; ++i) { gload(st, s, i, 0); gload(st, s, i, 1); }
    };
    auto split_all = [&](int s) __attribute__((always_inline)) {
#pragma unroll
      for (int i = 0; i < 4; ++i) {
#pragma unroll
        for (int tt = 0; tt < 4; ++tt) {
          float x0, x1;
          prep(s, i, raw_lo(0, i, tt), raw_hi(0, i, tt), x0, x1);
          bsum[tt] = fmaf(x0 + x1, bias_w, bsum[tt]);
          if (NPL == 3) split3_pair(x0, x1, pl[tt][0][i], pl[tt][1][i], pl[tt][NPL - 1][i]);
          else split2_pair(x0, x1, pl[tt][0][i], pl[tt][1][i]);
        }
      }
    };
    auto write_all = [&](int so) __attribute__((always_inline)) {
#pragma unroll
      for (int tt = 0; tt < 4; ++tt)
#pragma unroll
        for (int p = 0; p < NPL; ++p) write_tile(so, tt, p);
    };
    constexpr int NQ = (NPL == 3 ? 6 : 3), PH = 4 * NQ, NM = 4 * PH, GPI = NM / 16;
    using BT = std::integral_constant<bool, true>; using BF = std::integral_constant<bool, false>;
    load_all(0, 0);
    __syncthreads();
    split_all(0);
    load_all(1 % RS, 1);
    if (RS == 2) load_all(0, 2);
    write_all(0);
    auto stage = [&](int s, auto Mc, auto Pc) __attribute__((always_inline)) {
      constexpr bool MORE = decltype(Mc)::value;
      constexpr int so0 = decltype(Pc)::value * W3P_PL, so1 = W3P_PL - so0;
      constexpr int NX = (decltype(Pc)::value + 1) % RS;
      __syncthreads();
      u32x4 ap[4][NPL], bp[2][NPL];
#pragma unroll
      for (int p = 0; p < NPL; ++p) {
        bp[0][p] = plane(so0, 2 + wb, 0, p);
#pragma unroll
        for (int ta = 0; ta < 4; ++ta) ap[ta][p] = plane(so0, wa, ta, p);
      }
      float x0 = 0.f, x1 = 0.f, ra = 0.f, rb = 0.f;
      __builtin_amdgcn_sched_barrier(0);
#pragma unroll
      for (int g = 0; g < NM; ++g) {
        const int tb = g / PH, gg = g % PH, q = gg / 4, ta = g % 4;
        const int sa = (q == 2 || q == 5) ? 1 : (q == 4 ? NPL - 1 : 0);
        const int sb = (q == 1 || q == 5) ? 1 : (q == 3 ? NPL - 1 : 0);
        w3_mfma(ta + 4 * tb, acc_unused, ap[ta][sa], bp[tb & 1][sb]);
        if (MORE) {
          const int it = g / GPI, st = g % GPI, i = it / 4, tt = it % 4;
          if (st == 0) prep(s + 1, i, raw_lo(NX, i, tt), raw_hi(NX, i, tt), x0, x1);
          if (st == 1) { pl[tt][0][i] = pk_bf16(x0, x1); bsum[tt] = fmaf(x0 + x1, bias_w, bsum[tt]); }
          if (NPL == 3) {
            if (st == 2) { ra = x0 - bf16_lo(pl[tt][0][i]); rb = x1 - bf16_hi(pl[tt][0][i]); }
            if (st == 3) pl[tt][1][i] = pk_bf16(ra, rb);
            if (st == 4) { ra -= bf16_lo(pl[tt][1][i]); rb -= bf16_hi(pl[tt][1][i]); }
            if (st == 5) pl[tt][NPL - 1][i] = pk_bf16(ra, rb);
          } else {
            if (st == 2) pl[tt][1][i] = pk_bf16(x0 - bf16_lo(pl[tt][0][i]), x1 - bf16_hi(pl[tt][0][i]));
          }
          if (it >= 13 && st < NPL) write_tile(so1, tt - 1, st);
          if (tt == 3 && st == 1) gload(NX, s + 1 + RS, i, 0);
          if (tt == 3 && st == 2) gload(NX, s + 1 + RS, i, 1);
        }
        if (tb < 3 && gg >= PH / 2 && gg < PH / 2 + NPL) bp[(tb + 1) & 1][gg - PH / 2] = plane(so0, 2 + wb, tb + 1, gg - PH / 2);
        __builtin_amdgcn_sched_barrier(0);
      }
      if (MORE) {
#pragma unroll
        for (int p = 0; p < NPL; ++p) write_tile(so1, 3, p);
      }
    };
    using P0 = std::integral_constant<int, 0>; using P1 = std::integral_constant<int, 1>;
    {
      int s = 0;
      for (; s + 2 < nst; s += 2) { stage(s, BT{}, P0{}); stage(s + 1, BT{}, P1{}); }
      if (s + 1 < nst) { stage(s, BT{}, P0{}); stage(s + 1, BF{}, P1{}); }
      else stage(s, BF{}, P0{});
    }
  }
  (void)wa;
}

template <int NPL, bool PLAIN>
__device__ __forceinline__ void wgrad3p_body(const WgLaunch& L, float* lds) {
  float* plb = lds;
  const int tid = threadIdx.x, lane = tid & 63;
  const int w = __builtin_amdgcn_readfirstlane(tid >> 6);
  const int wa = w >> 1, wb = w & 1, i32 = lane & 31, kg = lane >> 5;
  const WgTask& t = L.t[blockIdx.y];
  const int64_t chunk = blockIdx.x + L.chunk0;
  w3_acc_zero();
  float bsum[4] = {0.f, 0.f, 0.f, 0.f};
  const bool opB = (w >> 1) != 0;
  for (int jb = 0; jb < t.njobs; ++jb) {
    const WgJob& job = t.j[jb];
    const int64_t m_lo = chunk * WG_CH;
    const int64_t m_hi = (m_lo + WG_CH < job.m_count) ? m_lo + WG_CH : job.m_count;
    if (m_hi <= m_lo) continue;
    const bool blk = m_lo < (opB ? job.b_blk : job.a_blk);
    const int lay = __builtin_amdgcn_readfirstlane(!blk ? 0 : ((opB ? job.b_p24 : job.a_p24) != 0 ? 2 : 1));
    if (lay == 2) {
      if constexpr (NPL == 2) w3p_job<2, NPL, PLAIN>(t, job, jb, chunk, plb, bsum, w, lane);
    } else if (lay == 1) w3p_job<1, NPL, PLAIN>(t, job, jb, chunk, plb, bsum, w, lane);
    else w3p_job<0, NPL, PLAIN>(t, job, jb, chunk, plb, bsum, w, lane);
  }
  w3_mfma_drain();
  float* out = L.partials + chunk * L.chunk_stride;
  const int64_t toff = t.out_off + (int64_t)(wa * 128) * t.ldo + wb * 128;
#pragma unroll
  for (int ta = 0; ta < 4; ++ta)
#pragma unroll
    for (int r = 0; r < 16; ++r) {
      const int ri = (r & 3) + 8 * (r >> 2) + 4 * kg;
      const f32x4 v = {w3_acc_read(16 * ta + r), w3_acc_read(16 * (ta + 4) + r), w3_acc_read(16 * (ta + 8) + r), w3_acc_read(16 * (ta + 12) + r)};
      *reinterpret_cast<f32x4*>(out + toff + (int64_t)(4 * ri + ta) * t.ldo + 4 * i32) = v;
    }
  if (t.has_bias != 0 && !opB) {
#pragma unroll
    for (int tt = 0; tt < 4; ++tt) bsum[tt] += __shfl_xor(bsum[tt], 32);
    if (kg == 0) *reinterpret_cast<f32x4*>(out + t.bias_off + (w & 1) * 128 + 4 * i32) = f32x4{bsum[0], bsum[1], bsum[2], bsum[3]};
  }
}

template <int NPL>
__global__ __launch_bounds__(256) void wgrad3p_kernel(WgLaunch L) {
  extern __shared__ __attribute__((aligned(16))) float lds[];
  const WgTask& t = L.t[blockIdx.y];
  const int64_t m_lo = (int64_t)(blockIdx.x + L.chunk0) * WG_CH;
  bool plain = t.relu_b == 0;
  for (int jb = 0; jb < t.njobs; ++jb) {
    const int64_t left = t.j[jb].m_count - m_lo;
    plain = plain && (left >= WG_CH || left <= 0 || left % W3_PTS == 0);
  }
  if (plain) wgrad3p_body<NPL, true>(L, lds);
  else wgrad3p_body<NPL, false>(L, lds);
}

template <int NPL>
__global__ __launch_bounds__(256) void wgrad_all_kernel(WgLaunch L) {
  extern __shared__ __attribute__((aligned(16))) float lds[];
  const WgTask& t = L.t[blockIdx.y];
  if (t.variant == 4) {
    const int64_t m_lo = (int64_t)(blockIdx.x + L.chunk0) * WG_CH;
    bool plain = t.relu_b == 0;
    for (int jb = 0; jb < t.njobs; ++jb) {
      const int64_t left = t.j[jb].m_count - m_lo;
      plain = plain && (left >= WG_CH || left <= 0 || left % W3_PTS == 0);
    }
    if (plain) wgrad3p_body<NPL, true>(L, lds);
    else wgrad3p_body<NPL, false>(L, lds);
    return;
  }
  const int lane = threadIdx.x & 63, wave = __builtin_amdgcn_readfirstlane(threadIdx.x >> 6);
  const int64_t chunk = blockIdx.x + L.chunk0;
  if (t.variant == 0) wgrad_wide_body<3>(L, t, chunk, wave, lane, lds);
  else if (t.variant == 1) wgrad_narrow_body<1, 0, 3>(L, t, chunk, wave, lane, lds);
  else if (t.variant == 2) { if (t.j[0].a_p24) wgrad_narrow_body<0, 1, 3, true>(L, t, chunk, wave, lane, lds); else wgrad_narrow_body<0, 1, 3>(L, t, chunk, wave, lane, lds); }
  else { if (t.j[0].a_p24) wgrad_narrow_body<0, 2, 3, true>(L, t, chunk, wave, lane, lds); else wgrad_narrow_body<0, 2, 3>(L, t, chunk, wave, lane, lds); }
}

struct WnLayer {
  int64_t off_v, off_g, off_bias, blk_off, bias_blk_off;
  int32_t rows, cols, row0, ldo, rsplit, rbase, split, base1, valid0;
  float mult;
};
struct WnTab { WnLayer l[3 * I2SDF_MAX_LAYERS]; int32_t n; int32_t n_rows; };

__global__ __launch_bounds__(256) void wn_backward_kernel(WnTab tab, const float* __restrict__ params, const float* __restrict__ partials,
                                                           int n_chunks, int64_t chunk_stride, float* __restrict__ grad) {
  __shared__ float s_dw[4][5 * 64];
  __shared__ float s_b[4];
  const int row = blockIdx.x;
  const int lane = threadIdx.x & 63, wv = threadIdx.x >> 6;
  int e = 0;
  while (e + 1 < tab.n && row >= tab.l[e + 1].row0) ++e;
  const WnLayer& y = tab.l[e];
  const int r = row - y.row0;
  const int brow = r < y.rsplit ? r : r - y.rsplit + y.rbase;
  const float* v = params + y.off_v + (int64_t)r * y.cols;
  constexpr int MAXC = 5;
  const float* src[MAXC];
  float sacc[MAXC];
#pragma unroll
  for (int q = 0; q < MAXC; ++q) {
    const int c = lane + 64 * q;
    const int kp = c < y.valid0 ? c : y.split + (c - y.base1);
    src[q] = (c < y.cols) ? partials + y.blk_off + (int64_t)brow * y.ldo + kp : nullptr;
    sacc[q] = 0.f;
  }
#pragma unroll 2
  for (int ch = wv; ch < n_chunks; ch += 4) {
    float x[MAXC];
#pragma unroll
    for (int q = 0; q < MAXC; ++q) x[q] = src[q] ? src[q][ch * chunk_stride] : 0.f;
#pragma unroll
    for (int q = 0; q < MAXC; ++q) sacc[q] += x[q];
  }
#pragma unroll
  for (int q = 0; q < MAXC; ++q) s_dw[wv][lane + 64 * q] = sacc[q];
  if (lane == 0) {
    float b = 0.f;
    const float* bs = partials + y.bias_blk_off + brow;
    for (int ch = wv; ch < n_chunks; ch += 4) b += bs[ch * chunk_stride];
    s_b[wv] = b;
  }
  __syncthreads();
  if (wv != 0) return;
  float dw[MAXC], vv[MAXC];
  float dot = 0.f, nrm2 = 0.f;
#pragma unroll
  for (int q = 0; q < MAXC; ++q) {
    const int c = lane + 64 * q;
    dw[q] = 0.f; vv[q] = 0.f;
    if (c < y.cols) {
      dw[q] = (s_dw[0][c] + s_dw[1][c] + s_dw[2][c] + s_dw[3][c]) * y.mult;
      vv[q] = v[c];
      dot = fmaf(dw[q], vv[q], dot);
      nrm2 = fmaf(vv[q], vv[q], nrm2);
    }
  }
#pragma unroll
  for (int o = 32; o > 0; o >>= 1) { dot += __shfl_xor(dot, o); nrm2 += __shfl_xor(nrm2, o); }
  const float nrm = sqrtf(nrm2);
  const float g = params[y.off_g + r];
  const float gs = g / nrm, dn = dot / nrm2;
#pragma unroll
  for (int q = 0; q < MAXC; ++q) {
    const int c = lane + 64 * q;
    if (c < y.cols) grad[y.off_v + (int64_t)r * y.cols + c] = gs * (dw[q] - vv[q] * dn);
  }
  if (lane == 0) {
    grad[y.off_g + r] = dot / nrm;
    grad[y.off_bias + r] = s_b[0] + s_b[1] + s_b[2] + s_b[3];
  }
}

struct Src { const float* p; int ld; int w; int64_t blk = 0; int p24 = 0; };

struct TaskList {
  std::vector<WgTask> tasks;
  bool quads = false;
  void add_block(int64_t blk_off, int ldo, int64_t bias_off, const std::vector<Src>& A0, const std::vector<Src>& A1,
                 const std::vector<int>& row0, const std::vector<int64_t>& mA0, const std::vector<Src>& B0, const std::vector<Src>& B1,
                 int64_t m1, bool relu_b) {
    int col0 = 0;
    for (size_t k = 0; k < B0.size(); ++k) {
      if (quads && B0[k].w == 256) {
        for (size_t i = 0; i < A0.size(); ++i) {
          if (A0[i].w != 256) continue;
          WgTask t{};
          t.j[0] = WgJob{A0[i].p, B0[k].p, A0[i].ld, B0[k].ld, 256, 256, mA0[i], A0[i].blk, B0[k].blk, 0, 0, A0[i].p24, B0[k].p24};
          t.njobs = 1;
          if (!A1.empty() && A1[i].p != nullptr && !B1.empty()) {
            t.j[1] = WgJob{A1[i].p, B1[k].p, A1[i].ld, B1[k].ld, 256, 256, m1, A1[i].blk, B1[k].blk, 0, 0, A1[i].p24, B1[k].p24};
            t.njobs = 2;
          }
          t.relu_b = relu_b ? 1 : 0;
          t.has_bias = (k == 0) ? 1 : 0;
          t.rows_store = 256; t.cols_store = 256; t.ldo = ldo;
          t.out_off = blk_off + (int64_t)row0[i] * ldo + col0;
          t.bias_off = bias_off + row0[i];
          tasks.push_back(t);
        }
      }
      for (int ct = 0; ct * 128 < B0[k].w; ++ct) {
        for (size_t i = 0; i < A0.size(); ++i) {
          if (quads && B0[k].w == 256 && A0[i].w == 256) continue;
          for (int rt = 0; rt * 128 < A0[i].w; ++rt) {
            WgTask t{};
            const int aw = std::min(128, A0[i].w - rt * 128), bw = std::min(128, B0[k].w - ct * 128);
            t.j[0] = WgJob{A0[i].p + rt * 128, B0[k].p + ct * 128, A0[i].ld, B0[k].ld, aw, bw, mA0[i], A0[i].blk, B0[k].blk, rt * 128, ct * 128, A0[i].p24, B0[k].p24};
            t.njobs = 1;
            if (!A1.empty() && A1[i].p != nullptr && !B1.empty()) {
              t.j[1] = WgJob{A1[i].p + rt * 128, B1[k].p + ct * 128, A1[i].ld, B1[k].ld, aw, bw, m1, A1[i].blk, B1[k].blk, rt * 128, ct * 128, A1[i].p24, B1[k].p24};
              t.njobs = 2;
            }
            t.relu_b = relu_b ? 1 : 0;
            t.has_bias = (k == 0 && ct == 0) ? 1 : 0;
            t.rows_store = aw; t.cols_store = bw; t.ldo = ldo;
            t.out_off = blk_off + (int64_t)(row0[i] + rt * 128) * ldo + col0 + ct * 128;
            t.bias_off = bias_off + row0[i] + rt * 128;
            tasks.push_back(t);
          }
        }
      }
      col0 += B0[k].w;
    }
  }
};

void fill_wn(WnTab& tab, const NetPlan& np, int kind, int& row0) {
  const i2sdf_mlp_desc& d = np.d;
  const int PEC8 = (d.multires > 0 ? cdiv(d.d_in + 2 * d.d_in * d.multires, 8) : 0) * 8;
  const int PED = d.multires > 0 ? d.d_in + 2 * d.d_in * d.multires : d.d_in;
  for (int l = 0; l < d.n_lin; ++l) {
    WnLayer& y = tab.l[tab.n++];
    y.off_v = d.off_v[l]; y.off_g = d.off_g[l]; y.off_bias = d.off_bias[l];
    y.rows = d.out_dim[l]; y.cols = d.in_dim[l]; y.row0 = row0; row0 += y.rows;
    y.ldo = np.wg_cols[l];
    y.blk_off = np.wgrad_off[l];
    y.bias_blk_off = np.wgrad_off[l] + (int64_t)np.wg_rows[l] * np.wg_cols[l];
    y.rsplit = 1 << 30; y.rbase = 0; y.split = 0; y.base1 = 0; y.valid0 = y.cols; y.mult = 1.0f;
    const bool last = l == d.n_lin - 1;
    if (kind == 0) {
      if (l == d.skip_layer) { y.valid0 = y.cols - PED; y.split = d.hidden; y.base1 = y.cols - PED; y.mult = 0.70710678118654752440f; }
      if (last) { y.rsplit = 1; y.rbase = 32; }
    } else if (kind == 1) {
      if (l == 0) { y.valid0 = PED; y.split = PEC8; y.base1 = PED; }
    }
  }
}

}

extern "C" int64_t i2sdf_wgrad_chunk_points(void) { return WG_CH; }

extern "C" int i2sdf_weight_grads(const i2sdf_plan* p, const i2sdf_train_buffers* tb, const float* params, float* partials,
                                  int64_t n_chunks_cap, float* grad_flat, void* stream) {
  if (!p || !tb || !params || !partials || !grad_flat) return I2SDF_EINVAL;
  const int64_t Mp = tb->Mp, Ms = tb->M_sdf, Mm = tb->M_main;
  if (Ms <= 0 || Mm < 0 || Mm > Ms || Mp < Ms || Mp % 128 != 0) return I2SDF_EINVAL;
  const int n_chunks = (int)((Ms + WG_CH - 1) / WG_CH);
  if (n_chunks > n_chunks_cap) return I2SDF_EWORKSPACE;
  hipStream_t st = (hipStream_t)stream;
  TaskList tl;
  tl.quads = p->wgrad_bf16x3 != 0;
  {
    const NetPlan& np = p->sdf;
    const i2sdf_mlp_desc& d = np.d;
    const int L = d.n_lin, H = d.hidden, F = p->F, PEC8 = cdiv(d.in0, 8) * 8;
    const int64_t ls = Mp * H;
    const int64_t bs = (H == 256) ? sdf_blocked_points(p, Ms, Mp) : 0;
    const int s24 = (H == 256 && sdf_saves24(p) && bs == Mp) ? 1 : 0;
    for (int l = 0; l < L - 1; ++l) {
      std::vector<Src> B0, B1;
      if (l == 0) { B0 = {{tb->pe, PEC8, PEC8}}; B1 = {{tb->gpbar, PEC8, PEC8}}; }
      else {
        B0 = {{tb->hs + (l - 1) * ls, H, H, bs}}; B1 = {{tb->gus + l * ls, H, H, bs, s24}};
        if (l == d.skip_layer) { B0.push_back({tb->pe, PEC8, PEC8}); B1.push_back({tb->gpbar, PEC8, PEC8}); }
      }
      tl.add_block(np.wgrad_off[l], np.wg_cols[l], np.wgrad_off[l] + (int64_t)np.wg_rows[l] * np.wg_cols[l],
                   {{tb->gas + l * ls, H, H, bs, s24}}, {{tb->abars + l * ls, H, H, bs, s24}}, {0}, {Ms}, B0, B1, Ms, false);
    }
    {
      const int l = L - 1;
      std::vector<Src> A0 = {{tb->ga_last4, 4, 4}}, A1 = {{tb->ones4, 4, 4}};
      std::vector<int> row0 = {0};
      std::vector<int64_t> mA0 = {Ms};
      if (F > 0 && Mm > 0 && tb->fbar) { A0.push_back({tb->fbar, F, F}); A1.push_back({nullptr, 0, 0}); row0.push_back(32); mA0.push_back(Mm); }
      tl.add_block(np.wgrad_off[l], np.wg_cols[l], np.wgrad_off[l] + (int64_t)np.wg_rows[l] * np.wg_cols[l], A0, A1, row0, mA0,
                   {{tb->hs + (L - 2) * ls, H, H, bs}}, {{tb->gus + (L - 1) * ls, H, H, bs}}, Ms, false);
    }
  }
  if (Mm > 0 && tb->gar) {
    const NetPlan& np = p->rgb;
    const i2sdf_mlp_desc& d = np.d;
    const int L = d.n_lin, H = d.hidden, F = p->F, PV8 = cdiv(d.in0 - F, 8) * 8;
    const int64_t ls = Mp * H;
    const int64_t br = (H == 256) ? rgb_blocked_points(p, Mm, Mp) : 0;
    for (int l = 0; l < L; ++l) {
      std::vector<Src> B0;
      if (l == 0) B0 = {{tb->pev, PV8, PV8}, {tb->feat, F, F}};
      else B0 = {{tb->rs + (l - 1) * ls, H, H, br}};
      std::vector<Src> A0;
      if (l < L - 1) A0 = {{tb->gar + l * ls, H, H, br}};
      else A0 = {{tb->ga_last_rgb, 4, 4}};
      tl.add_block(np.wgrad_off[l], np.wg_cols[l], np.wgrad_off[l] + (int64_t)np.wg_rows[l] * np.wg_cols[l], A0, {}, {0}, {Mm}, B0, {}, 0,
                   false);
    }
  }
  const bool has_light = p->light.d.n_lin > 0 && Mm > 0 && tb->gal0;
  if (has_light) {
    const NetPlan& np = p->light;
    const int H = np.d.hidden, F = p->F;
    tl.add_block(np.wgrad_off[0], np.wg_cols[0], np.wgrad_off[0] + (int64_t)np.wg_rows[0] * np.wg_cols[0], {{tb->gal0, H, H}}, {}, {0}, {Mm},
                 {{tb->feat, F, F}}, {}, 0, true);
    tl.add_block(np.wgrad_off[1], np.wg_cols[1], np.wgrad_off[1] + (int64_t)np.wg_rows[1] * np.wg_cols[1], {{tb->gal_last, 4, 4}}, {}, {0},
                 {Mm}, {{tb->hl, H, H}}, {}, 0, false);
  }
  auto variant = [](const WgTask& x) {
    return x.j[0].a_w == 256 ? 4 : (x.j[0].a_w <= 32 ? 1 : (x.j[0].b_w <= 32 ? 2 : (x.j[0].b_w <= 64 ? 3 : 0)));
  };
  for (WgTask& x : tl.tasks) x.variant = variant(x);
  hipStream_t st_main = st;
  int c_lo = 0, c_hi = n_chunks;
  auto launch = [&](const std::vector<WgTask>& sel, int var) {
    for (size_t off = 0; off < sel.size(); off += MAX_TASKS) {
      WgLaunch L{};
      L.n = (int32_t)std::min<size_t>(MAX_TASKS, sel.size() - off);
      for (int i = 0; i < L.n; ++i) L.t[i] = sel[off + i];
      L.chunk_stride = p->wgrad_floats; L.partials = partials;
      L.chunk0 = c_lo;
      dim3 grid((unsigned)(c_hi - c_lo), (unsigned)L.n);
      if (var == 5) {
        constexpr int LB = W3P_LDS_BYTES > WGN_LDS_BYTES ? W3P_LDS_BYTES : WGN_LDS_BYTES;
        if (p->wgrad_bf16x2) {
          (void)hipFuncSetAttribute((const void*)wgrad_all_kernel<2>, hipFuncAttributeMaxDynamicSharedMemorySize, LB);
          wgrad_all_kernel<2><<<grid, 256, LB, st>>>(L);
        } else {
          (void)hipFuncSetAttribute((const void*)wgrad_all_kernel<3>, hipFuncAttributeMaxDynamicSharedMemorySize, LB);
          wgrad_all_kernel<3><<<grid, 256, LB, st>>>(L);
        }
      } else if (var == 4) {
        if (p->wgrad_bf16x2) {
          (void)hipFuncSetAttribute((const void*)wgrad3p_kernel<2>, hipFuncAttributeMaxDynamicSharedMemorySize, W3P_LDS_BYTES);
          wgrad3p_kernel<2><<<grid, 256, W3P_LDS_BYTES, st>>>(L);
        } else {
          (void)hipFuncSetAttribute((const void*)wgrad3p_kernel<3>, hipFuncAttributeMaxDynamicSharedMemorySize, W3P_LDS_BYTES);
          wgrad3p_kernel<3><<<grid, 256, W3P_LDS_BYTES, st>>>(L);
        }
      } else if (var == 0) {
        wgrad_kernel<0, 0><<<grid, 64, 0, st>>>(L);
      } else {
        if (p->wgrad_bf16x3) {
          (void)hipFuncSetAttribute((const void*)wgrad_narrow_kernel<3>, hipFuncAttributeMaxDynamicSharedMemorySize, WGN_LDS_BYTES);
          wgrad_narrow_kernel<3><<<grid, 256, WGN_LDS_BYTES, st>>>(L);
        } else {
          (void)hipFuncSetAttribute((const void*)wgrad_narrow_kernel<0>, hipFuncAttributeMaxDynamicSharedMemorySize, WGN_LDS_BYTES);
          wgrad_narrow_kernel<0><<<grid, 256, WGN_LDS_BYTES, st>>>(L);
        }
      }
    }
  };
  std::vector<WgTask> sel_narrow, sel_blocks[2];
  const bool wide_in_narrow = p->wgrad_bf16x3 != 0;
  if (wide_in_narrow)
    for (const WgTask& x : tl.tasks) if (x.variant == 0) sel_narrow.push_back(x);
  for (int var : {3, 1, 2})
    for (int nj = 2; nj >= 1; --nj)
      for (const WgTask& x : tl.tasks) if (x.variant == var && x.njobs == nj) sel_narrow.push_back(x);
  for (int v = 0; v < 2; ++v) {
    for (const WgTask& x : tl.tasks) if (x.variant == (v == 0 ? 4 : 0) && !(v == 1 && wide_in_narrow)) sel_blocks[v].push_back(x);
    std::stable_sort(sel_blocks[v].begin(), sel_blocks[v].end(), [](const WgTask& x, const WgTask& y) { return x.njobs > y.njobs; });
  }
  static const bool merged_env = [] { const char* e = getenv("I2SDF_WGRAD_MERGED"); return !(e && e[0] == '0'); }();
  const bool merged = merged_env && p->wgrad_bf16x3 != 0 && sel_narrow.size() + sel_blocks[0].size() <= (size_t)MAX_TASKS && !sel_blocks[0].empty();
  std::vector<WgTask> sel_all;
  static const bool blocks_first = [] { const char* e = getenv("I2SDF_WGRAD_BLOCKS_FIRST"); return !(e && e[0] == '0'); }();
  if (merged) {
    if (blocks_first) { sel_all = sel_blocks[0]; sel_all.insert(sel_all.end(), sel_narrow.begin(), sel_narrow.end()); }
    else { sel_all = sel_narrow; sel_all.insert(sel_all.end(), sel_blocks[0].begin(), sel_blocks[0].end()); }
  }
  PartRun pr;
  if (i2sdf_parts_on(p) && i2sdf_parts_begin(p, st_main, Ms, &pr)) {
    for (int q = 0; q < pr.n; ++q) {
      if (pr.hi[q] <= pr.lo[q]) continue;
      c_lo = (int)(pr.lo[q] / WG_CH); c_hi = (int)((pr.hi[q] + WG_CH - 1) / WG_CH);
      st = pr.st[q];
      if (merged) launch(sel_all, 5);
      else {
        launch(sel_narrow, 1);
        launch(sel_blocks[0], 4);
      }
      launch(sel_blocks[1], 0);
    }
    st = st_main; c_lo = 0; c_hi = n_chunks;
    i2sdf_parts_join_all(p, st_main);
  } else {
    hipStream_t side = i2sdf_tail_fork(p, st_main);
    st = side;
    launch(sel_narrow, 1);
    st = st_main;
    launch(sel_blocks[0], 4);
    launch(sel_blocks[1], 0);
    i2sdf_tail_join(p, st_main, side);
  }
  WnTab tab{};
  int row0 = 0;
  fill_wn(tab, p->sdf, 0, row0);
  if (Mm > 0 && tb->gar) fill_wn(tab, p->rgb, 1, row0);
  if (has_light) fill_wn(tab, p->light, 2, row0);
  tab.n_rows = row0;
  wn_backward_kernel<<<row0, 256, 0, st>>>(tab, params, partials, n_chunks, p->wgrad_floats, grad_flat);
  return i2sdf_hip_check(hipGetLastError(), "weight_grads launch");
}
```

i2sdf_amd/engine.py:

```python
from __future__ import annotations

import ctypes as C
from typing import Optional

import os

import torch

from . import lib as L
from .config import NetConfig
from .params import ParamLayout


class RenderEngine:
    def __init__(self, cfg: NetConfig, device="cuda"):
        self.cfg = cfg
        self.layout = ParamLayout(cfg)
        self.device = torch.device(device)
        self._lib = L.load()
        self._desc = self.layout.net_desc()
        plan = C.c_void_p()
        L.check(self._lib.i2sdf_plan_create(C.byref(self._desc), C.byref(plan)), "i2sdf_plan_create")
        self._plan = plan
        self.pack_floats = int(self._lib.i2sdf_plan_pack_floats(plan))
        self.wgrad_floats = int(self._lib.i2sdf_plan_wgrad_floats(plan))
        self.packed = torch.zeros(self.pack_floats, dtype=torch.float32, device=self.device)
        self._pack_stream, self._pack_event, self._pack_readers = None, None, {}
        self.F = cfg.feature_size
        wide = cfg.sdf.hidden == 256 and cfg.feature_size == 256
        self.set_sdf_forward_bf16x3(bool(cfg.bf16x3 and cfg.sdf.hidden % 64 == 0))
        self.set_wgrad_bf16x3(bool(cfg.bf16x3))
        self.set_train_forward_bf16x3(bool(cfg.bf16x3 and wide))
        self.set_sdf_backward_bf16x3(bool(cfg.bf16x3 and wide))
        self.set_rgb_bf16x3(bool(cfg.bf16x3 and cfg.rgb.hidden == 256 and cfg.feature_size == 256 and cfg.rgb.n_lin >= 3))
        self.wgrad_bf16x2 = False
        x2 = os.environ.get("I2SDF_WGRAD_BF16X2", "")
        self.set_wgrad_bf16x2(bool(cfg.bf16x3 and ((x2 != "0") if x2 != "" else cfg.wgrad_bf16x2)))
        self.sampler_bf16x2 = False
        sx2 = os.environ.get("I2SDF_SAMPLER_BF16X2", "")
        if wide:
            self.set_sampler_bf16x2(bool(self.sdf_forward_bf16x3 and ((sx2 != "0") if sx2 != "" else getattr(cfg, "sampler_bf16x2", False))))
        self.set_blocked_saves(bool(cfg.bf16x3 and os.environ.get("I2SDF_BLOCKED_SAVES", "1") != "0"))
        self.saves24 = False
        s24 = os.environ.get("I2SDF_SAVES24", "")
        if wide:
            self.set_saves24(bool(cfg.bf16x3 and ((s24 != "0") if s24 != "" else getattr(cfg, "saves24", True))))
        self.set_tail_overlap(os.environ.get("I2SDF_TAIL_OVERLAP", "1") != "0")
        self.parts = 0
        n_parts = int(os.environ.get("I2SDF_PARTS", "2"))
        self._parts_wanted = n_parts if (cfg.bf16x3 and n_parts >= 2) else 0
        self._sync_parts()
        sc = cfg.sampler
        self._scfg = L.SamplerCfg(near=sc.near, eps=sc.eps, add_tiny=sc.add_tiny, N_samples=sc.N_samples, N_samples_eval=sc.N_samples_eval,
                                  N_samples_extra=sc.N_samples_extra, beta_iters=sc.beta_iters, max_total_iters=sc.max_total_iters)
        dev = self.device
        self.t_lin = torch.linspace(0.0, 1.0, steps=sc.N_samples_eval, device=dev)
        self.u_more = torch.linspace(0.0, 1.0, steps=sc.N_samples_eval, device=dev)
        self.u_final = torch.linspace(0.0, 1.0, steps=sc.N_samples, device=dev)
        if sc.N_samples_extra > 0:
            self.extra_tab = torch.stack([torch.linspace(0, sc.N_samples_eval * (it + 1) - 1, sc.N_samples_extra).long()
                                          for it in range(sc.max_total_iters)]).to(torch.int32).to(dev).contiguous()
        else:
            self.extra_tab = None
        self.n_z = sc.N_samples + sc.N_samples_extra + 2

    def start_timing(self):
        self._timing = []
        eng = self

        class _Timed:
            def __init__(self, fn, name):
                self.fn, self.name = fn, name

            def __call__(self, *a):
                e0, e1 = torch.cuda.Event(enable_timing=True), torch.cuda.Event(enable_timing=True)
                e0.record()
                rc = self.fn(*a)
                e1.record()
                eng._timing.append((self.name, e0, e1))
                return rc

        self._timed_lib = type("TimedLib", (), {})()
        for name in L.SIGNATURES:
            fn = getattr(self._lib, name)
            if name in ("i2sdf_sdf_forward", "i2sdf_sdf_forward_grad", "i2sdf_rgb_forward", "i2sdf_rgb_backward", "i2sdf_sdf_backward",
                        "i2sdf_weight_grads", "i2sdf_sample_rays", "i2sdf_composite_forward", "i2sdf_composite_backward", "i2sdf_pack_weights",
                        "i2sdf_ray_setup", "i2sdf_light_forward", "i2sdf_light_backward"):
                fn = _Timed(fn, name)
            setattr(self._timed_lib, name, fn)
        self._real_lib, self._lib = self._lib, self._timed_lib

    def stop_timing(self):
        self._lib = self._real_lib
        out = {}
        for name, e0, e1 in self._timing:
            tot, cnt = out.get(name, (0.0, 0))
            out[name] = (tot + e0.elapsed_time(e1), cnt + 1)
        self._timing = []
        return out

    def __del__(self):
        try:
            if getattr(self, "_plan", None):
                self._lib.i2sdf_plan_destroy(self._plan)
                self._plan = None
        except Exception:
            pass

    def pack(self, flat_params: torch.Tensor):
        assert flat_params.is_cuda and flat_params.dtype == torch.float32 and flat_params.numel() == self.layout.n_params
        if os.environ.get("I2SDF_PACK_ASYNC", "1") == "0":
            L.check(self._lib.i2sdf_pack_weights(self._plan, L.ptr(flat_params), L.ptr(self.packed), L.stream_ptr()), "i2sdf_pack_weights")
            return
        dev = flat_params.device
        side = self._pack_stream
        if side is None:
            side = self._pack_stream = torch.cuda.Stream(device=dev)
        cur = torch.cuda.current_stream(dev)
        side.wait_stream(cur)
        for st in getattr(self, "_pack_readers", {}):
            if st != cur:
                side.wait_stream(st)
        with torch.cuda.stream(side):
            L.check(self._lib.i2sdf_pack_weights(self._plan, L.ptr(flat_params), L.ptr(self.packed), L.stream_ptr()), "i2sdf_pack_weights")
            self._pack_event = side.record_event()
        flat_params.record_stream(side)
        self._pack_readers = {}

    def _pk(self):
        ev = self._pack_event
        if ev is not None:
            cur = torch.cuda.current_stream(self.packed.device)
            readers = self.__dict__.setdefault("_pack_readers", {})
            if cur not in readers:
                cur.wait_event(ev)
                readers[cur] = True
        return L.ptr(self.packed)

    def set_sdf_forward_bf16x3(self, on: bool):
        L.check(self._lib.i2sdf_plan_set_option(self._plan, L.OPT_SDF_FWD_BF16X3, int(bool(on))), "i2sdf_plan_set_option")
        self.sdf_forward_bf16x3 = bool(on)

    def set_train_forward_bf16x3(self, on: bool):
        L.check(self._lib.i2sdf_plan_set_option(self._plan, L.OPT_TRAIN_FWD_BF16X3, int(bool(on))), "i2sdf_plan_set_option")
        self.train_forward_bf16x3 = bool(on)
        if hasattr(self, "_parts_wanted"):
            self._sync_parts()

    def set_sdf_backward_bf16x3(self, on: bool):
        L.check(self._lib.i2sdf_plan_set_option(self._plan, L.OPT_SDF_BWD_BF16X3, int(bool(on))), "i2sdf_plan_set_option")
        self.sdf_backward_bf16x3 = bool(on)
        if hasattr(self, "_parts_wanted"):
            self._sync_parts()

    def set_rgb_bf16x3(self, on: bool):
        L.check(self._lib.i2sdf_plan_set_option(self._plan, L.OPT_RGB_BF16X3, int(bool(on))), "i2sdf_plan_set_option")
        self.rgb_bf16x3 = bool(on)
        if hasattr(self, "_parts_wanted"):
            self._sync_parts()

    def set_wgrad_bf16x2(self, on: bool):
        L.check(self._lib.i2sdf_plan_set_option(self._plan, L.OPT_WGRAD_BF16X2, int(bool(on))), "i2sdf_plan_set_option")
        self.wgrad_bf16x2 = bool(on)

    def set_sampler_bf16x2(self, on: bool):
        rc = self._lib.i2sdf_plan_set_option(self._plan, L.OPT_SAMPLER_BF16X2, int(bool(on)))
        if on or rc == 0:
            L.check(rc, "i2sdf_plan_set_option")
        self.sampler_bf16x2 = bool(on) and rc == 0

    def set_blocked_saves(self, on: bool):
        L.check(self._lib.i2sdf_plan_set_option(self._plan, L.OPT_BLOCKED_SAVES, int(bool(on))), "i2sdf_plan_set_option")
        self.blocked_saves = bool(on)

    def set_saves24(self, on: bool):
        rc = self._lib.i2sdf_plan_set_option(self._plan, L.OPT_SAVES24, int(bool(on)))
        if on or rc == 0:
            L.check(rc, "i2sdf_plan_set_option")
        self.saves24 = bool(on) and rc == 0

    def blocked_points(self, which: int, M: int, Mp: int, has_feat: bool = True) -> int:
        return int(self._lib.i2sdf_blocked_points(self._plan, which, M, Mp, int(has_feat)))

    def saves24_points(self, M: int, Mp: int, has_feat: bool = True) -> int:
        return int(self._lib.i2sdf_blocked_points(self._plan, 2, M, Mp, int(has_feat))) if self.saves24 else 0

    @staticmethod
    def saved_to_point_major(t: torch.Tensor, n_blocked: int, p24_layers=None) -> torch.Tensor:
        if n_blocked <= 0:
            return t.clone()
        Lr, Mp, H = t.shape
        assert H == 256 and n_blocked % 32 == 0
        out = t.clone()
        out[:, :n_blocked] = t[:, :n_blocked].reshape(Lr, n_blocked // 32, 16, 32, 16).permute(0, 1, 3, 2, 4).reshape(Lr, n_blocked, 256)
        if p24_layers is not None and any(p24_layers):
            assert n_blocked == Mp, "packed records: every point is blocked"
            nb = Mp // 32
            for l in range(Lr):
                if not p24_layers[l]:
                    continue
                raw = t[l].reshape(-1)[: nb * 6144].view(torch.int32).reshape(nb, 16, 384)
                hi16 = raw[:, :, :256].contiguous().view(torch.int16).reshape(nb, 16, 32, 2, 8).to(torch.int32) & 0xFFFF
                mid = raw[:, :, 256:].contiguous().view(torch.uint8).reshape(nb, 16, 32, 2, 8).to(torch.int32)
                val = ((hi16 << 16) | (mid << 8)).view(torch.float32)
                v = val.reshape(nb, 16, 32, 2, 2, 4).permute(0, 2, 1, 4, 3, 5)
                out[l] = v.reshape(Mp, 256)
        return out

    def saved_pm(self, name: str, t: torch.Tensor, M: int, has_feat: bool = True) -> torch.Tensor:
        Mp = t.shape[1]
        if name in ("rs", "gar"):
            return self.saved_to_point_major(t, self.blocked_points(1, M, Mp))[:, :M]
        nb = self.blocked_points(0, M, Mp, has_feat)
        p24 = None
        if name in ("abars", "gus", "gas") and self.saves24_points(M, Mp, has_feat) == Mp:
            p24 = [True] * t.shape[0]
            if name == "gus":
                p24[-1] = False
                p24[0] = False
        return self.saved_to_point_major(t, nb, p24)[:, :M]

    def set_tail_overlap(self, on: bool):
        L.check(self._lib.i2sdf_plan_set_option(self._plan, L.OPT_TAIL_OVERLAP, int(bool(on))), "i2sdf_plan_set_option")
        self.tail_overlap = bool(on)

    def _sync_parts(self):
        want = self._parts_wanted if (self.train_forward_bf16x3 and self.sdf_backward_bf16x3 and self.rgb_bf16x3) else 0
        if want != self.parts:
            n = int(want) if int(want) >= 2 else 0
            L.check(self._lib.i2sdf_plan_set_option(self._plan, L.OPT_PARTS, n), "i2sdf_plan_set_option")
            self.parts = n

    def set_parts(self, n: int):
        self._parts_wanted = int(n) if int(n) >= 2 else 0
        self._sync_parts()

    def chain(self, M: int):
        eng = self
        if not getattr(self, "use_chain", True) or not self.parts:
            import contextlib
            return contextlib.nullcontext()

        class _Chain:
            def __enter__(self_):
                L.check(eng._lib.i2sdf_chain_begin(eng._plan, int(M), L.stream_ptr()), "i2sdf_chain_begin")
                return self_

            def __exit__(self_, *exc):
                L.check(eng._lib.i2sdf_chain_end(eng._plan, L.stream_ptr()), "i2sdf_chain_end")
                return False

            def fence(self_):
                L.check(eng._lib.i2sdf_chain_fence(eng._plan, L.stream_ptr()), "i2sdf_chain_fence")

        return _Chain()

    def set_exchange(self, ex, flags: int = 0):
        self._exchange = ex
        L.check(self._lib.i2sdf_plan_set_exchange(self._plan, C.byref(ex) if ex is not None else None, int(flags)), "i2sdf_plan_set_exchange")

    def set_wgrad_bf16x3(self, on: bool):
        L.check(self._lib.i2sdf_plan_set_option(self._plan, L.OPT_WGRAD_BF16X3, int(bool(on))), "i2sdf_plan_set_option")
        self.wgrad_bf16x3 = bool(on)

    def sdf_forward(self, points: torch.Tensor, want_features: bool = False):
        pts = points.detach().to(torch.float32).contiguous()
        M = pts.shape[0]
        sdf = torch.empty(M, 1, dtype=torch.float32, device=pts.device)
        feat = torch.empty(M, self.F, dtype=torch.float32, device=pts.device) if want_features else None
        L.check(self._lib.i2sdf_sdf_forward(self._plan, self._pk(), L.ptr(pts), M, L.ptr(sdf), L.ptr(feat), self.F,
                                            L.stream_ptr()), "i2sdf_sdf_forward")
        return (sdf, feat) if want_features else sdf

    @staticmethod
    def pad_rows(M: int) -> int:
        return (M + 127) // 128 * 128

    def _ws(self, *shape, device=None):
        return torch.empty(*shape, dtype=torch.float32, device=device)

    def sdf_forward_grad(self, points=None, rays=None, want_grad=True, save=True, want_feat=True):
        cfgs = self.cfg.sdf
        H, NL = cfgs.hidden, cfgs.n_lin
        pts = cam = dirs = z = None
        n_ray, ldz, npr = 0, 0, 1
        if rays is not None:
            cam, dirs, z = (t.detach().to(torch.float32).contiguous() for t in rays[:3])
            npr = rays[3] if len(rays) > 3 else z.shape[1]
            n_ray, ldz = z.shape[0] * npr, z.shape[1]
            dev = z.device
        if points is not None:
            pts = points.detach().to(torch.float32).contiguous()
            dev = pts.device
        M = n_ray + (pts.shape[0] if pts is not None else 0)
        Mp = self.pad_rows(M)
        out = {"Mp": Mp, "M": M, "n_ray_pts": n_ray, "pts": pts, "rays": (cam, dirs, z, npr), "sdf": torch.empty(M, 1, dtype=torch.float32, device=dev),
               "blk": self.blocked_points(0, M, Mp, want_feat)}
        out["feat"] = self._ws(Mp, self.F, device=dev) if want_feat else None
        out["grad"] = torch.empty(M, 3, dtype=torch.float32, device=dev) if want_grad else None
        out["hs"] = self._ws(NL - 1, Mp, H, device=dev) if (save or want_grad) else None
        out["abars"] = self._ws(NL - 1, Mp, H, device=dev) if (save and want_grad) else None
        out["pe"] = self._ws(Mp, 40, device=dev) if save else None
        L.check(self._lib.i2sdf_sdf_forward_grad(self._plan, self._pk(), L.ptr(pts), L.ptr(cam), L.ptr(dirs), L.ptr(z),
                                                  ldz, npr, n_ray, M, Mp, L.ptr(out["sdf"]), L.ptr(out["feat"]), L.ptr(out["grad"]),
                                                  L.ptr(out["hs"]), L.ptr(out["abars"]), L.ptr(out["pe"]), L.stream_ptr()),
                 "i2sdf_sdf_forward_grad")
        return out

    def rgb_forward(self, dirs, n_per_ray, feat, M, save=True):
        Mp = feat.shape[0]
        rgb = torch.empty(M, 3, dtype=torch.float32, device=feat.device)
        Lr, Hr = self.cfg.rgb.n_lin, self.cfg.rgb.hidden
        rs = self._ws(Lr - 1, Mp, Hr, device=feat.device) if save else None
        pev = self._ws(Mp, 32, device=feat.device) if save else None
        L.check(self._lib.i2sdf_rgb_forward(self._plan, self._pk(), L.ptr(dirs.contiguous()), n_per_ray, L.ptr(feat), M, Mp,
                                             L.ptr(rgb), L.ptr(rs), L.ptr(pev), L.stream_ptr()), "i2sdf_rgb_forward")
        return rgb, rs, pev

    def rgb_backward(self, rgb, rgb_bar, rs, M):
        Mp, dev = rs.shape[1], rs.device
        Lr, Hr = self.cfg.rgb.n_lin, self.cfg.rgb.hidden
        gar = self._ws(Lr - 1, Mp, Hr, device=dev)
        ga_last = self._ws(Mp, 4, device=dev)
        fbar = self._ws(Mp, self.F, device=dev)
        L.check(self._lib.i2sdf_rgb_backward(self._plan, self._pk(), L.ptr(rgb), L.ptr(rgb_bar.contiguous()), L.ptr(rs), M, Mp,
                                              L.ptr(gar), L.ptr(ga_last), L.ptr(fbar), L.stream_ptr()), "i2sdf_rgb_backward")
        return gar, ga_last, fbar

    def sdf_backward(self, fw, sbar=None, fbar=None, m_fbar=0, nbar=None):
        cfgs = self.cfg.sdf
        H, NL = cfgs.hidden, cfgs.n_lin
        Mp, M, dev = fw["Mp"], fw["M"], fw["hs"].device
        cam, dirs, z, npr = fw["rays"]
        o = {"gus": self._ws(NL, Mp, H, device=dev), "gpbar": self._ws(Mp, 40, device=dev), "gas": self._ws(NL - 1, Mp, H, device=dev),
             "ga_last4": self._ws(Mp, 4, device=dev), "ones4": self._ws(Mp, 4, device=dev)}
        c = lambda t: None if t is None else t.contiguous()
        L.check(self._lib.i2sdf_sdf_backward(self._plan, self._pk(), L.ptr(fw["pts"]), L.ptr(cam), L.ptr(dirs), L.ptr(z),
                                              z.shape[1] if z is not None else 0, npr, fw["n_ray_pts"], M, Mp,
                                              L.ptr(fw["hs"]), L.ptr(fw["abars"]), L.ptr(c(sbar)), L.ptr(c(fbar)), m_fbar, L.ptr(c(nbar)),
                                              L.ptr(o["gus"]), L.ptr(o["gpbar"]), L.ptr(o["gas"]), L.ptr(o["ga_last4"]), L.ptr(o["ones4"]),
                                              L.stream_ptr()), "i2sdf_sdf_backward")
        return o

    def weight_grads(self, flat_params, grad_flat, fw, bw, M_main=0, fbar=None, rgb_fw=None, rgb_bw=None, light=None):
        tb = L.TrainBuffers()
        tb.M_sdf, tb.M_main, tb.Mp = fw["M"], M_main, fw["Mp"]
        P = lambda t: None if t is None else t.data_ptr()
        tb.pe, tb.hs, tb.abars = P(fw["pe"]), P(fw["hs"]), P(fw["abars"])
        tb.gus, tb.gpbar, tb.gas, tb.ga_last4, tb.ones4 = P(bw["gus"]), P(bw["gpbar"]), P(bw["gas"]), P(bw["ga_last4"]), P(bw["ones4"])
        tb.fbar = P(fbar)
        tb.feat = P(fw["feat"])
        if rgb_fw is not None:
            tb.pev, tb.rs = P(rgb_fw["pev"]), P(rgb_fw["rs"])
            tb.gar, tb.ga_last_rgb = P(rgb_bw["gar"]), P(rgb_bw["ga_last"])
        if light is not None:
            tb.hl, tb.gal0, tb.gal_last = P(light["hl"]), P(light["gal0"]), P(light["gal_last"])
        ch = int(self._lib.i2sdf_wgrad_chunk_points())
        n_chunks = (fw["M"] + ch - 1) // ch
        partials = torch.empty(n_chunks * self.wgrad_floats, dtype=torch.float32, device=flat_params.device)
        L.check(self._lib.i2sdf_weight_grads(self._plan, C.byref(tb), L.ptr(flat_params), L.ptr(partials), n_chunks, L.ptr(grad_flat),
                                              L.stream_ptr()), "i2sdf_weight_grads")
        return partials

    def ray_setup(self, uv, pose, intrinsics):
        uv, pose, intrinsics = (t.detach().to(torch.float32).contiguous() for t in (uv, pose, intrinsics))
        quat = pose.dim() == 2 and pose.shape[1] == 7
        if not quat and tuple(pose.shape[1:]) != (4, 4):
            raise ValueError(f"pose must be (batch,4,4) or (batch,7), got {tuple(pose.shape)}")
        batch, pixels = uv.shape[0], uv.shape[1]
        N = batch * pixels
        cam = torch.empty(N, 3, dtype=torch.float32, device=uv.device)
        dirs = torch.empty_like(cam)
        dnorm = torch.empty(N, dtype=torch.float32, device=uv.device)
        L.check(self._lib.i2sdf_ray_setup_ex(L.ptr(uv), L.ptr(pose), int(quat), L.ptr(intrinsics), batch, pixels, L.ptr(cam),
                                              L.ptr(dirs), L.ptr(dnorm), L.stream_ptr()), "i2sdf_ray_setup_ex")
        return cam, dirs, dnorm

    def sphere_intersections(self, cam_loc, dirs, radius):
        cam_loc, dirs = cam_loc.detach().float().contiguous(), dirs.detach().float().contiguous()
        N = cam_loc.shape[0]
        out = torch.empty(N, 2, dtype=torch.float32, device=cam_loc.device)
        miss = torch.zeros(1, dtype=torch.int32, device=cam_loc.device)
        L.check(self._lib.i2sdf_sphere_intersections(L.ptr(cam_loc), L.ptr(dirs), N, float(radius), L.ptr(out), L.ptr(miss),
                                                      L.stream_ptr()), "i2sdf_sphere_intersections")
        if int(miss.item()) > 0:
            raise ValueError(f"BOUNDING SPHERE PROBLEM: {int(miss.item())} rays do not intersect the sphere of radius {radius}")
        return out

    def composite_forward(self, beta_param, z_all, sdf, rgb, grad, lmask, dnorm, want_normal, save=True, eik_grad=None):
        B, n = z_all.shape[0], z_all.shape[1] - 1
        dev = z_all.device
        o = {"rgb": torch.empty(B, 3, device=dev), "depth": torch.empty(B, device=dev), "wsum": torch.empty(B, 1, device=dev)}
        o["normal"] = torch.empty(B, 3, device=dev) if want_normal else None
        o["lmask"] = torch.empty(B, 1, device=dev) if lmask is not None else None
        o["w"] = torch.empty(B, n, device=dev) if save else None
        o["nsum"] = torch.empty(B, 3, device=dev) if (save and want_normal) else None
        if eik_grad is not None and eik_grad.shape[0] == 3 * B and B > 0:
            o["grad_theta"], o["diff_norm"] = torch.empty(2 * B, 3, device=dev), torch.empty(B, device=dev)
            L.check(self._lib.i2sdf_composite_forward_eik(L.ptr(beta_param), self.cfg.beta_min, L.ptr(z_all), z_all.shape[1], L.ptr(sdf),
                                                           L.ptr(rgb), L.ptr(grad) if want_normal else None, L.ptr(lmask), L.ptr(dnorm), B, n,
                                                           L.ptr(o["rgb"]), L.ptr(o["depth"]), L.ptr(o["wsum"]), L.ptr(o["normal"]),
                                                           L.ptr(o["lmask"]), L.ptr(o["w"]), L.ptr(o["nsum"]), L.ptr(eik_grad.contiguous()),
                                                           L.ptr(o["grad_theta"]), L.ptr(o["diff_norm"]), L.stream_ptr()), "i2sdf_composite_forward_eik")
            return o
        L.check(self._lib.i2sdf_composite_forward(L.ptr(beta_param), self.cfg.beta_min, L.ptr(z_all), z_all.shape[1], L.ptr(sdf),
                                                   L.ptr(rgb), L.ptr(grad) if want_normal else None, L.ptr(lmask), L.ptr(dnorm), B, n,
                                                   L.ptr(o["rgb"]), L.ptr(o["depth"]), L.ptr(o["wsum"]), L.ptr(o["normal"]),
                                                   L.ptr(o["lmask"]), L.ptr(o["w"]), L.ptr(o["nsum"]), L.stream_ptr()),
                 "i2sdf_composite_forward")
        return o

    def composite_backward(self, beta_param, z_all, sdf, rgb, grad, dnorm, nsum, g_rgb, g_depth, g_wsum, g_normal, g_lmask,
                           beta_grad_accum=None, sdf_bar_out=None, grad_bar_out=None):
        B, n = z_all.shape[0], z_all.shape[1] - 1
        dev = z_all.device
        M = B * n
        o = {"sdf_bar": sdf_bar_out if sdf_bar_out is not None else torch.empty(M, device=dev), "rgb_bar": torch.empty(M, 3, device=dev)}
        o["grad_bar"] = grad_bar_out if grad_bar_out is not None else (torch.empty(M, 3, device=dev) if g_normal is not None else None)
        o["lmask_bar"] = torch.empty(M, device=dev) if g_lmask is not None else None
        part = torch.empty(B, device=dev)
        c = lambda t: None if t is None else t.contiguous()
        L.check(self._lib.i2sdf_composite_backward(L.ptr(beta_param), self.cfg.beta_min, L.ptr(z_all), z_all.shape[1], L.ptr(sdf),
                                                    L.ptr(rgb), L.ptr(grad), L.ptr(dnorm), L.ptr(nsum), B, n, L.ptr(c(g_rgb)),
                                                    L.ptr(c(g_depth)), L.ptr(c(g_wsum)), L.ptr(c(g_normal)), L.ptr(c(g_lmask)),
                                                    L.ptr(o["sdf_bar"]), L.ptr(o["rgb_bar"]), L.ptr(o["grad_bar"]), L.ptr(o["lmask_bar"]),
                                                    L.ptr(part), L.ptr(beta_grad_accum), L.stream_ptr()), "i2sdf_composite_backward")
        o["beta_partial"] = part
        return o

    def training_draws(self, B: int, seed: int, device, eik_radius: float = 0.0, want_eik: bool = True):
        sc = self.cfg.sampler
        e = lambda *s, dt=torch.float32: torch.empty(*s, dtype=dt, device=device)
        d = {"strat_u": e(B, sc.N_samples_eval), "cdf_u": e(B, sc.N_samples),
             "extra_idx": e(sc.max_total_iters, sc.N_samples_extra, dt=torch.int32) if sc.N_samples_extra > 0 else None,
             "eik_idx": e(B, dt=torch.int32), "eik_pts": e(B, 3) if want_eik else None, "nbr_off": e(B, 3) if want_eik else None}
        L.check(self._lib.i2sdf_training_draws(int(seed) & (2 ** 64 - 1), B, sc.N_samples_eval, sc.N_samples, sc.N_samples_extra, sc.max_total_iters,
                                               self.n_z, float(eik_radius), 0.005, L.ptr(d["strat_u"]), L.ptr(d["cdf_u"]), L.ptr(d["extra_idx"]),
                                               L.ptr(d["eik_idx"]), L.ptr(d["eik_pts"]), L.ptr(d["nbr_off"]), L.stream_ptr()), "i2sdf_training_draws")
        return d

    def sample_rays(self, flat_params, cam, dirs, training=False, strat_u=None, cdf_u=None, extra_idx=None, eik_idx=None, force_iters=0):
        B, dev = cam.shape[0], cam.device
        ws = torch.empty(int(self._lib.i2sdf_sampler_workspace_floats(B)), dtype=torch.float32, device=dev)
        z_out = torch.empty(B, self.n_z, dtype=torch.float32, device=dev)
        z_eik = torch.empty(B, 1, dtype=torch.float32, device=dev)
        iters = torch.empty(1, dtype=torch.int32, device=dev) if B > 0 else torch.zeros(1, dtype=torch.int32, device=dev)
        i32 = lambda t: None if t is None else t.to(torch.int32).contiguous()
        if training:
            u_final, ldu = cdf_u.contiguous(), cdf_u.shape[1]
        else:
            u_final, ldu = self.u_final, 0
        ex, ek = i32(extra_idx), i32(eik_idx)
        su = None if strat_u is None else strat_u.contiguous()
        L.check(self._lib.i2sdf_sample_rays(self._plan, self._pk(), L.ptr(flat_params), C.byref(self._scfg), L.ptr(cam.contiguous()),
                                             L.ptr(dirs.contiguous()), B, 1 if training else 0, L.ptr(self.t_lin), L.ptr(self.u_more),
                                             L.ptr(u_final), ldu, L.ptr(self.extra_tab), L.ptr(su), L.ptr(ex), L.ptr(ek), force_iters,
                                             L.ptr(ws), L.ptr(z_out), self.n_z, L.ptr(z_eik), L.ptr(iters), L.stream_ptr()),
                 "i2sdf_sample_rays")
        self._last_sampler_ws = ws
        return z_out, z_eik, iters

    def error_bound(self, z, sdf, beta, d_star=None, want_d_star=False):
        z, sdf = z.detach().float().contiguous(), sdf.detach().float().reshape(z.shape).contiguous()
        B, n = z.shape
        beta = beta.detach().float().reshape(-1).contiguous().to(z.device)
        if beta.numel() not in (1, B):
            raise ValueError("beta must be a scalar or one value per ray")
        bound = torch.empty(B, dtype=torch.float32, device=z.device)
        ds_out = torch.empty(B, n - 1, dtype=torch.float32, device=z.device) if want_d_star else None
        ds_in = None if d_star is None else d_star.detach().float().contiguous()
        L.check(self._lib.i2sdf_error_bound(L.ptr(z), L.ptr(sdf), B, n, L.ptr(beta), 0 if beta.numel() == 1 else 1, L.ptr(ds_in),
                                            L.ptr(ds_out), L.ptr(bound), L.stream_ptr()), "i2sdf_error_bound")
        return (bound, ds_out) if want_d_star else bound

    def render_image(self, flat_params, uv, pose, intrinsics, chunk, want_normal=True, want_z=False):
        uv = uv.detach().to(torch.float32).reshape(-1, 2).contiguous()
        pose = pose.detach().to(torch.float32).contiguous()
        intrinsics = intrinsics.detach().to(torch.float32).reshape(4, 4).contiguous()
        quat = pose.numel() == 7
        if not quat and pose.numel() != 16:
            raise ValueError(f"one view: pose must be (4,4) or (7,), got {tuple(pose.shape)}")
        P, dev = uv.shape[0], uv.device
        chunk = int(max(1, min(chunk, max(P, 1))))
        n_ws = int(self._lib.i2sdf_render_image_workspace_floats(self._plan, C.byref(self._scfg), chunk))
        ws = getattr(self, "_img_ws", None)
        if ws is None or ws.numel() < n_ws or ws.device != dev:
            ws = torch.empty(n_ws, dtype=torch.float32, device=dev)
            self._img_ws = ws
        e = lambda *s: torch.empty(*s, dtype=torch.float32, device=dev)
        o = {"rgb": e(P, 3), "depth": e(P), "wsum": e(P, 1), "normal": e(P, 3) if want_normal else None,
             "lmask": e(P, 1) if self.cfg.light is not None else None, "z": e(P, self.n_z) if want_z else None,
             "iters": torch.zeros((P + chunk - 1) // chunk, dtype=torch.int32, device=dev)}
        L.check(self._lib.i2sdf_render_image(self._plan, self._pk(), L.ptr(flat_params), C.byref(self._scfg), L.ptr(uv), L.ptr(pose),
                                             int(quat), L.ptr(intrinsics), P, chunk, L.ptr(self.t_lin), L.ptr(self.u_more), L.ptr(self.u_final),
                                             L.ptr(self.extra_tab), L.ptr(ws), L.ptr(o["rgb"]), L.ptr(o["depth"]), L.ptr(o["wsum"]),
                                             L.ptr(o["normal"]), L.ptr(o["lmask"]), L.ptr(o["z"]), L.ptr(o["iters"]), L.stream_ptr()),
                "i2sdf_render_image")
        return o

    def sdf_grid(self, x, y, z, rot=None, trans=None, order: int = L.GRID_ORDER_VOLUME, first: int = 0, count: Optional[int] = None,
                 chunk: int = 1 << 21):
        x, y, z = (t.detach().to(torch.float32).contiguous() for t in (x, y, z))
        dev = x.device
        nx, ny, nz = x.numel(), y.numel(), z.numel()
        total = nx * ny * nz
        count = total - first if count is None else count
        chunk = int(max(128, min(chunk, max(count, 128))))
        ws = getattr(self, "_grid_ws", None)
        n_ws = int(self._lib.i2sdf_sdf_grid_workspace_floats(chunk))
        if ws is None or ws.numel() < n_ws or ws.device != dev:
            ws = torch.empty(n_ws, dtype=torch.float32, device=dev)
            self._grid_ws = ws
        out = torch.empty(count, dtype=torch.float32, device=dev)
        host = lambda v, n: None if v is None else (C.c_float * n)(*[float(a) for a in torch.as_tensor(v, dtype=torch.float32).reshape(-1).tolist()])
        r, t = host(rot, 9), host(trans, 3)
        L.check(self._lib.i2sdf_sdf_grid(self._plan, self._pk(), L.ptr(x), L.ptr(y), L.ptr(z), nx, ny, nz, int(order),
                                         C.cast(r, C.c_void_p) if r is not None else None, C.cast(t, C.c_void_p) if t is not None else None,
                                         int(first), int(count), L.ptr(out), L.ptr(ws), chunk, L.stream_ptr()), "i2sdf_sdf_grid")
        return out

    def light_forward(self, feat, M, save=True):
        Mp, dev = feat.shape[0], feat.device
        HL = self.cfg.light.hidden
        lm = torch.empty(M, dtype=torch.float32, device=dev)
        hl = self._ws(Mp, HL, device=dev) if save else None
        L.check(self._lib.i2sdf_light_forward(self._plan, self._pk(), L.ptr(feat), M, Mp, L.ptr(lm), L.ptr(hl), L.stream_ptr()),
                 "i2sdf_light_forward")
        return lm, hl

    def light_backward(self, lm, lm_bar, hl, M):
        Mp, dev = hl.shape[0], hl.device
        gal0 = self._ws(Mp, hl.shape[1], device=dev)
        gal_last = self._ws(Mp, 4, device=dev)
        L.check(self._lib.i2sdf_light_backward(self._plan, self._pk(), L.ptr(lm), L.ptr(lm_bar.contiguous()), L.ptr(hl), M, Mp,
                                                L.ptr(gal0), L.ptr(gal_last), L.stream_ptr()), "i2sdf_light_backward")
        return gal0, gal_last
```

i2sdf_amd/lib.py:

```python
from __future__ import annotations

import ctypes as C
import os

MAX_LAYERS = 12
_HERE = os.path.dirname(os.path.abspath(__file__))
LIB_PATH = os.environ.get("I2SDF_LIB_PATH") or os.path.join(_HERE, "lib", "libi2sdf_hip.so")


class MlpDesc(C.Structure):
    _fields_ = [("n_lin", C.c_int32), ("hidden", C.c_int32), ("d_in", C.c_int32), ("in0", C.c_int32), ("d_out", C.c_int32),
                ("multires", C.c_int32), ("skip_layer", C.c_int32), ("reserved", C.c_int32),
                ("out_dim", C.c_int32 * MAX_LAYERS), ("in_dim", C.c_int32 * MAX_LAYERS),
                ("off_bias", C.c_int64 * MAX_LAYERS), ("off_g", C.c_int64 * MAX_LAYERS), ("off_v", C.c_int64 * MAX_LAYERS)]


class NetDesc(C.Structure):
    _fields_ = [("sdf", MlpDesc), ("rgb", MlpDesc), ("light", MlpDesc), ("off_beta", C.c_int64), ("n_params", C.c_int64),
                ("beta_min", C.c_float), ("scene_bounding_sphere", C.c_float)]


class TrainBuffers(C.Structure):
    _fields_ = [("M_sdf", C.c_int64), ("M_main", C.c_int64), ("Mp", C.c_int64)] + [(n, C.c_void_p) for n in (
        "pe", "hs", "abars", "gus", "gpbar", "gas", "ga_last4", "ones4", "fbar", "pev", "feat", "rs", "gar", "ga_last_rgb",
        "hl", "gal0", "gal_last")]


class SamplerCfg(C.Structure):
    _fields_ = [("near", C.c_float), ("eps", C.c_float), ("add_tiny", C.c_float), ("N_samples", C.c_int32), ("N_samples_eval", C.c_int32),
                ("N_samples_extra", C.c_int32), ("beta_iters", C.c_int32), ("max_total_iters", C.c_int32)]


EXCHANGE_FN = C.CFUNCTYPE(C.c_int, C.c_void_p, C.c_void_p, C.c_int64, C.c_int32, C.c_int32, C.c_void_p)


class Exchange(C.Structure):
    _fields_ = [("allreduce", EXCHANGE_FN), ("ctx", C.c_void_p)]


class LossCfg(C.Structure):
    _fields_ = [(n, C.c_float) for n in ("eikonal_w", "smooth_w", "mask_w", "depth_w", "normal_w", "angular_w", "bubble_w", "light_w")] + \
               [("smooth_on", C.c_int32), ("reserved", C.c_int32), ("exchange", C.POINTER(Exchange))]


XCHG_F32, XCHG_I32 = 0, 1
XCHG_SUM, XCHG_AVG, XCHG_MAX = 0, 1, 2
DP_GLOBAL_SAMPLER = 1
COMM_UNIQUE_ID_BYTES = 128


class RayTables(C.Structure):
    _fields_ = [("intrinsics", C.c_void_p), ("pose", C.c_void_p), ("pose_is_quat", C.c_int32), ("n_images", C.c_int32),
                ("height", C.c_int32), ("width", C.c_int32)] + \
               [(n, C.c_void_p) for n in ("rgb", "depth", "normal", "mask", "light_mask", "depth_mask", "normal_mask")]


class RayBatch(C.Structure):
    _fields_ = [(n, C.c_void_p) for n in ("image_idx", "uv", "cam_loc", "dirs", "dnorm", "rgb", "depth", "normal", "mask", "light_mask",
                                          "depth_mask", "normal_mask", "n_bad")]


OPT_SDF_FWD_BF16X3 = 1
OPT_WGRAD_BF16X3 = 2
OPT_TRAIN_FWD_BF16X3 = 4
OPT_SDF_BWD_BF16X3 = 8
OPT_RGB_BF16X3 = 16
OPT_TAIL_OVERLAP = 32
OPT_BLOCKED_SAVES = 128
OPT_WGRAD_BF16X2 = 256
OPT_PARTS = 512
OPT_SAMPLER_BF16X2 = 1024
OPT_SAVES24 = 2048
MAX_PARTS = 4
GRID_ORDER_MESHGRID, GRID_ORDER_VOLUME = 0, 1


class I2SDFError(RuntimeError):
    pass


_lib = None

_P, _I64, _I32, _F, _D = C.c_void_p, C.c_int64, C.c_int32, C.c_float, C.c_double
SIGNATURES = {
    "i2sdf_version": (C.c_int, []),
    "i2sdf_strerror": (C.c_char_p, [C.c_int]),
    "i2sdf_last_hip_error": (C.c_char_p, []),
    "i2sdf_plan_create": (C.c_int, [C.POINTER(NetDesc), C.POINTER(_P)]),
    "i2sdf_plan_destroy": (None, [_P]),
    "i2sdf_plan_set_option": (C.c_int, [_P, _I32, _I32]),
    "i2sdf_chain_begin": (C.c_int, [_P, _I64, _P]),
    "i2sdf_chain_fence": (C.c_int, [_P, _P]),
    "i2sdf_chain_end": (C.c_int, [_P, _P]),
    "i2sdf_blocked_points": (_I64, [_P, _I32, _I64, _I64, _I32]),
    "i2sdf_plan_pack_floats": (_I64, [_P]),
    "i2sdf_plan_wgrad_floats": (_I64, [_P]),
    "i2sdf_pack_weights": (C.c_int, [_P, _P, _P, _P]),
    "i2sdf_sdf_forward": (C.c_int, [_P, _P, _P, _I64, _P, _P, _I64, _P]),
    "i2sdf_sdf_forward_grad": (C.c_int, [_P] * 6 + [_I64, _I32, _I64, _I64, _I64] + [_P] * 7),
    "i2sdf_rgb_forward": (C.c_int, [_P, _P, _P, _I32, _P, _I64, _I64, _P, _P, _P, _P]),
    "i2sdf_rgb_backward": (C.c_int, [_P] * 5 + [_I64, _I64] + [_P] * 4),
    "i2sdf_sdf_backward": (C.c_int, [_P] * 6 + [_I64, _I32, _I64, _I64, _I64] + [_P] * 4 + [_I64] + [_P] * 7),
    "i2sdf_wgrad_chunk_points": (_I64, []),
    "i2sdf_weight_grads": (C.c_int, [_P, C.POINTER(TrainBuffers), _P, _P, _I64, _P, _P]),
    "i2sdf_comm_available": (_I32, []),
    "i2sdf_comm_unique_id": (C.c_int, [_P, _I64]),
    "i2sdf_comm_init_rank": (C.c_int, [_P, _I32, _I32, C.POINTER(_P)]),
    "i2sdf_comm_destroy": (None, [_P]),
    "i2sdf_comm_size": (_I32, [_P]),
    "i2sdf_comm_rank": (_I32, [_P]),
    "i2sdf_last_comm_error": (C.c_char_p, []),
    "i2sdf_allreduce_grads": (C.c_int, [_P, _I64, _P, _P]),
    "i2sdf_allreduce_max_i32": (C.c_int, [_P, _I64, _P, _P]),
    "i2sdf_broadcast": (C.c_int, [_P, _I64, _I32, _P, _P]),
    "i2sdf_comm_as_exchange": (C.c_int, [_P, C.POINTER(Exchange)]),
    "i2sdf_plan_set_exchange": (C.c_int, [_P, C.POINTER(Exchange), _I32]),
    "i2sdf_adam_step": (C.c_int, [_P, _P, _P, _P, _I64, _D, _D, _D, _D, _D, _I64, _D, _P]),
    "i2sdf_error_bound": (C.c_int, [_P, _P, _I64, _I32, _P, _I64, _P, _P, _P, _P]),
    "i2sdf_sampler_workspace_floats": (_I64, [_I64]),
    "i2sdf_sample_rays": (C.c_int, [_P, _P, _P, C.POINTER(SamplerCfg), _P, _P, _I64, _I32, _P, _P, _P, _I64, _P, _P, _P, _P, _I32, _P, _P,
                                    _I64, _P, _P, _P]),
    "i2sdf_render_image_workspace_floats": (_I64, [_P, C.POINTER(SamplerCfg), _I64]),
    "i2sdf_render_image": (C.c_int, [_P, _P, _P, C.POINTER(SamplerCfg), _P, _P, _I32, _P, _I64, _I64] + [_P] * 13),
    "i2sdf_sdf_grid_workspace_floats": (_I64, [_I64]),
    "i2sdf_sdf_grid": (C.c_int, [_P, _P, _P, _P, _P, _I32, _I32, _I32, _I32, _P, _P, _I64, _I64, _P, _P, _I64, _P]),
    "i2sdf_marching_cubes_workspace_bytes": (_I64, [_I32, _I32, _I32]),
    "i2sdf_marching_cubes_count": (C.c_int, [_P, _I32, _I32, _I32, _F, _P, _P, _P]),
    "i2sdf_marching_cubes_emit": (C.c_int, [_P, _I32, _I32, _I32, _F, _P, _P, _P, _P, _P, _P, _I64, _I64, _P]),
    "i2sdf_mesh_scan_workspace_bytes": (_I64, [_I64]),
    "i2sdf_mesh_status": (C.c_int, [_P, _P]),
    "i2sdf_mesh_edge_keys": (C.c_int, [_P, _I64, _I64, _P, _P, _P]),
    "i2sdf_mesh_face_components": (C.c_int, [_P, _P, _I64, _P, _P]),
    "i2sdf_mesh_face_areas": (C.c_int, [_P, _I64, _P, _I64, _P, _P, _P]),
    "i2sdf_mesh_cumsum_f64": (C.c_int, [_P, _I64, _P, _I64, _P, _P, _P]),
    "i2sdf_mesh_largest_label": (C.c_int, [_P, _P, _I64, _P, _P]),
    "i2sdf_mesh_compact_mark": (C.c_int, [_P, _P, _I64, _I64, _P, _P, _P, _P]),
    "i2sdf_mesh_compact_gather": (C.c_int, [_P, _P, _I64, _P, _I64, _P, _P, _P, _P, _P, _P, _P, _I64, _I64, _P]),
    "i2sdf_mesh_sample_surface": (C.c_int, [_P, _I64, _P, _I64, _P, _P, _P, _I64, _P, _P, _P, _P]),
    "i2sdf_points_bounds": (C.c_int, [_P, _I64, _P, _P, _P]),
    "i2sdf_points_voxel_keys": (C.c_int, [_P, _I64, _P, _D, _P, _P, _P]),
    "i2sdf_points_voxel_heads": (C.c_int, [_P, _I64, _P, _P]),
    "i2sdf_points_voxel_mean": (C.c_int, [_P, _I64, _P, _P, _P, _P, _P, _I64, _P]),
    "i2sdf_points_grid_workspace_bytes": (_I64, [_I64]),
    "i2sdf_points_grid_keys": (C.c_int, [_P, _I64, _P, _P, _P, _P]),
    "i2sdf_points_grid_build": (C.c_int, [_P, _I64, _P, _P, _P, _P, _P]),
    "i2sdf_points_nn_query": (C.c_int, [_P, _I64, _P, _I64, _P, _I32, _P, _P, _P, _P, _P]),
    "i2sdf_points_nn_fallback": (C.c_int, [_P, _I64, _P, _I64, _P, _P, _P, _P, _P]),
    "i2sdf_points_reduce_workspace_bytes": (_I64, [_I64]),
    "i2sdf_points_threshold_reduce": (C.c_int, [_P, _I64, _D, _P, _P, _P]),
    "i2sdf_pdf_update": (C.c_int, [_P, _P, _I32, _P, _I64, _I64, _P, _I64, C.c_double, C.c_double, _P, _I64, _P, _P]),
    "i2sdf_training_draws": (C.c_int, [C.c_uint64, _I64, _I32, _I32, _I32, _I32, _I32, C.c_float, C.c_float, _P, _P, _P, _P, _P, _P, _P]),
    "i2sdf_light_forward": (C.c_int, [_P, _P, _P, _I64, _I64, _P, _P, _P]),
    "i2sdf_light_backward": (C.c_int, [_P, _P, _P, _P, _P, _I64, _I64, _P, _P, _P]),
    "i2sdf_loss_scratch_floats": (_I64, []),
    "i2sdf_loss_forward_backward": (C.c_int, [C.POINTER(LossCfg), _I64, _I64] + [_P] * 27),
    "i2sdf_eikonal_outputs_forward": (C.c_int, [_P, _I64, _P, _P, _P]),
    "i2sdf_extra_points": (C.c_int, [_P, _P, _P, _P, _P, _I64, _P, _P]),
    "i2sdf_render_loss_scratch_floats": (_I64, [_I64]),
    "i2sdf_render_loss_backward": (C.c_int, [C.POINTER(LossCfg), _I64, _I32, _I64, _I64, _I64, _I64, _P, C.c_float, _P, _I64] + [_P] * 5 + [_P] * 8 + [_P] * 7 +
                                   [_P] * 3 + [_P] * 8 + [_P, _P, _P, _I32, _P, _P, _P]),
    "i2sdf_scale_seeds": (C.c_int, [_P, _P, _I64, _P, _I64, _P, _I64, _P, _I64, _P, _P, _P]),
    "i2sdf_backward_seeds": (C.c_int, [_P, _I64, _P, _P, _I64, _I64, _P, _I64, _P, _I64, C.c_int32, _P]),
    "i2sdf_eikonal_outputs_backward": (C.c_int, [_P, _P, _P, _I64, _P, _P]),
    "i2sdf_ray_setup": (C.c_int, [_P, _P, _P, _I64, _I32, _P, _P, _P, _P]),
    "i2sdf_ray_setup_ex": (C.c_int, [_P, _P, _I32, _P, _I64, _I32, _P, _P, _P, _P]),
    "i2sdf_ray_batch": (C.c_int, [C.POINTER(RayTables), _P, _I64, C.POINTER(RayBatch), _P]),
    "i2sdf_sphere_intersections": (C.c_int, [_P, _P, _I64, _F, _P, _P, _P]),
    "i2sdf_composite_forward": (C.c_int, [_P, _F, _P, _I64, _P, _P, _P, _P, _P, _I64, _I32] + [_P] * 8),
    "i2sdf_composite_forward_eik": (C.c_int, [_P, _F, _P, _I64, _P, _P, _P, _P, _P, _I64, _I32] + [_P] * 11),
    "i2sdf_composite_backward": (C.c_int, [_P, _F, _P, _I64] + [_P] * 5 + [_I64, _I32] + [_P] * 12),
}


def load():
    global _lib
    if _lib is not None:
        return _lib
    import torch
    if not os.path.exists(LIB_PATH):
        raise I2SDFError(f"{LIB_PATH} not found: build it with `python -c 'import __graft_entry__ as g; g.build()'` "
                         "(hipcc --offload-arch=gfx950). There is no CPU fallback.")
    lib = C.CDLL(LIB_PATH)
    for name, (res, args) in SIGNATURES.items():
        fn = getattr(lib, name)
        fn.restype, fn.argtypes = res, args
    _lib = lib
    return lib


def check(rc: int, what: str = ""):
    if rc != 0:
        lib = load()
        msg = lib.i2sdf_strerror(rc).decode()
        if rc == -2 or (rc == -1 and what == "i2sdf_plan_create"):
            msg += ": " + lib.i2sdf_last_hip_error().decode()
        if rc == -5:
            msg += ": " + lib.i2sdf_last_comm_error().decode()
        raise I2SDFError(f"{what} failed ({rc}): {msg}")


def ptr(t):
    if t is None:
        return None
    assert t.is_contiguous(), "C ABI needs contiguous tensors"
    return C.c_void_p(t.data_ptr())


def stream_ptr():
    import torch
    return C.c_void_p(torch.cuda.current_stream().cuda_stream)
```

include/i2sdf.h:

```cpp
#ifndef I2SDF_H
#define I2SDF_H

#include <stddef.h>
#include <stdint.h>

#ifdef __cplusplus
extern "C" {
#endif

#define I2SDF_VERSION 100
#define I2SDF_MAX_LAYERS 12
#define I2SDF_MAX_PARTS 4

#define I2SDF_OK 0
#define I2SDF_EINVAL (-1)
#define I2SDF_EHIP (-2)
#define I2SDF_ESPHERE (-3)
#define I2SDF_EWORKSPACE (-4)
#define I2SDF_ECOMM (-5)

typedef struct i2sdf_mlp_desc {
  int32_t n_lin;
  int32_t hidden;
  int32_t d_in;
  int32_t in0;
  int32_t d_out;
  int32_t multires;
  int32_t skip_layer;
  int32_t reserved;
  int32_t out_dim[I2SDF_MAX_LAYERS];
  int32_t in_dim[I2SDF_MAX_LAYERS];
  int64_t off_bias[I2SDF_MAX_LAYERS];
  int64_t off_g[I2SDF_MAX_LAYERS];
  int64_t off_v[I2SDF_MAX_LAYERS];
} i2sdf_mlp_desc;

typedef struct i2sdf_net_desc {
  i2sdf_mlp_desc sdf;
  i2sdf_mlp_desc rgb;
  i2sdf_mlp_desc light;
  int64_t off_beta;
  int64_t n_params;
  float beta_min;
  float scene_bounding_sphere;
} i2sdf_net_desc;

typedef struct i2sdf_plan i2sdf_plan;

int i2sdf_version(void);
const char* i2sdf_strerror(int code);
const char* i2sdf_last_hip_error(void);

int i2sdf_plan_create(const i2sdf_net_desc* desc, i2sdf_plan** out);
void i2sdf_plan_destroy(i2sdf_plan* plan);
#define I2SDF_OPT_SDF_FWD_BF16X3 1
#define I2SDF_OPT_WGRAD_BF16X3 2
#define I2SDF_OPT_TRAIN_FWD_BF16X3 4
#define I2SDF_OPT_SDF_BWD_BF16X3 8
#define I2SDF_OPT_RGB_BF16X3 16
#define I2SDF_OPT_TAIL_OVERLAP 32
#define I2SDF_OPT_BLOCKED_SAVES 128
#define I2SDF_OPT_WGRAD_BF16X2 256
#define I2SDF_OPT_PARTS 512
#define I2SDF_OPT_SAMPLER_BF16X2 1024
#define I2SDF_OPT_SAVES24 2048
int64_t i2sdf_blocked_points(const i2sdf_plan* plan, int32_t which, int64_t M, int64_t Mp, int32_t has_feat);
int i2sdf_plan_set_option(i2sdf_plan* plan, int32_t option, int32_t value);
int i2sdf_chain_begin(const i2sdf_plan* plan, int64_t M, void* stream);
int i2sdf_chain_fence(const i2sdf_plan* plan, void* stream);
int i2sdf_chain_end(const i2sdf_plan* plan, void* stream);
int64_t i2sdf_plan_pack_floats(const i2sdf_plan* plan);
int64_t i2sdf_plan_wgrad_floats(const i2sdf_plan* plan);

int i2sdf_pack_weights(const i2sdf_plan* plan, const float* params, float* packed, void* stream);

int i2sdf_sdf_forward(const i2sdf_plan* plan, const float* packed, const float* points, int64_t M,
                      float* sdf_out, float* feat_out, int64_t ld_feat, void* stream);


int i2sdf_sdf_forward_grad(const i2sdf_plan* plan, const float* packed, const float* points, const float* cam,
                           const float* dirs, const float* z, int64_t ldz, int32_t n_per_ray, int64_t n_ray_pts, int64_t M,
                           int64_t Mp, float* sdf, float* feat, float* grad, float* hs, float* abars, float* pe_save,
                           void* stream);

int i2sdf_rgb_forward(const i2sdf_plan* plan, const float* packed, const float* dirs, int32_t n_per_ray, const float* feat,
                      int64_t M, int64_t Mp, float* rgb, float* rs, float* pev_save, void* stream);

int i2sdf_rgb_backward(const i2sdf_plan* plan, const float* packed, const float* rgb, const float* rgb_bar, const float* rs,
                       int64_t M, int64_t Mp, float* gar, float* ga_last, float* fbar, void* stream);

int i2sdf_sdf_backward(const i2sdf_plan* plan, const float* packed, const float* points, const float* cam, const float* dirs,
                       const float* z, int64_t ldz, int32_t n_per_ray, int64_t n_ray_pts, int64_t M, int64_t Mp,
                       const float* hs, const float* abars, const float* sbar, const float* fbar, int64_t m_fbar,
                       const float* nbar, float* gus, float* gpbar, float* gas, float* ga_last4, float* ones4, void* stream);

int i2sdf_ray_setup(const float* uv, const float* pose, const float* intrinsics, int64_t batch, int32_t pixels,
                    float* cam_loc, float* dirs, float* dnorm, void* stream);
int i2sdf_ray_setup_ex(const float* uv, const float* pose, int32_t pose_is_quat, const float* intrinsics, int64_t batch,
                       int32_t pixels, float* cam_loc, float* dirs, float* dnorm, void* stream);

typedef struct i2sdf_ray_tables {
  const float* intrinsics;
  const float* pose;
  int32_t pose_is_quat;
  int32_t n_images, height, width;
  const float* rgb;
  const float* depth;
  const float* normal;
  const float* mask;
  const float* light_mask;
  const uint8_t* depth_mask;
  const uint8_t* normal_mask;
} i2sdf_ray_tables;

typedef struct i2sdf_ray_batch_out {
  int64_t* image_idx;
  float* uv;
  float* cam_loc;
  float* dirs;
  float* dnorm;
  float* rgb;
  float* depth;
  float* normal;
  float* mask;
  float* light_mask;
  uint8_t* depth_mask;
  uint8_t* normal_mask;
  int32_t* n_bad;
} i2sdf_ray_batch_out;

int i2sdf_ray_batch(const i2sdf_ray_tables* tables, const int64_t* tidx, int64_t n_rays, const i2sdf_ray_batch_out* out, void* stream);

int i2sdf_sphere_intersections(const float* cam_loc, const float* dirs, int64_t n_rays, float radius, float* t_near_far,
                               int32_t* n_miss, void* stream);

int i2sdf_composite_forward(const float* beta_param, float beta_min, const float* z, int64_t ldz, const float* sdf,
                            const float* rgb, const float* grad, const float* lmask, const float* dnorm, int64_t B, int32_t n,
                            float* o_rgb, float* o_depth, float* o_wsum, float* o_normal, float* o_lmask, float* w_save,
                            float* nsum_save, void* stream);

int i2sdf_composite_forward_eik(const float* beta_param, float beta_min, const float* z, int64_t ldz, const float* sdf,
                                const float* rgb, const float* grad, const float* lmask, const float* dnorm, int64_t B, int32_t n,
                                float* o_rgb, float* o_depth, float* o_wsum, float* o_normal, float* o_lmask, float* w_save,
                                float* nsum_save, const float* grad_all, float* grad_theta, float* diff_norm, void* stream);

int i2sdf_composite_backward(const float* beta_param, float beta_min, const float* z, int64_t ldz, const float* sdf,
                             const float* rgb, const float* grad, const float* dnorm, const float* nsum_save, int64_t B, int32_t n,
                             const float* g_rgb, const float* g_depth, const float* g_wsum, const float* g_normal,
                             const float* g_lmask, float* sdf_bar, float* rgb_bar, float* grad_bar, float* lmask_bar,
                             float* beta_partial, float* beta_grad_accum, void* stream);


typedef struct i2sdf_train_buffers {
  int64_t M_sdf;
  int64_t M_main;
  int64_t Mp;
  const float *pe, *hs, *abars, *gus, *gpbar, *gas, *ga_last4, *ones4, *fbar;
  const float *pev, *feat, *rs, *gar, *ga_last_rgb;
  const float *hl, *gal0, *gal_last;
} i2sdf_train_buffers;

int64_t i2sdf_wgrad_chunk_points(void);
int i2sdf_weight_grads(const i2sdf_plan* plan, const i2sdf_train_buffers* bufs, const float* params, float* partials,
                       int64_t n_chunks_cap, float* grad_flat, void* stream);


typedef struct i2sdf_comm i2sdf_comm;
#define I2SDF_COMM_UNIQUE_ID_BYTES 128
#define I2SDF_DP_GLOBAL_SAMPLER 1
#define I2SDF_XCHG_F32 0
#define I2SDF_XCHG_I32 1
#define I2SDF_XCHG_SUM 0
#define I2SDF_XCHG_AVG 1
#define I2SDF_XCHG_MAX 2
typedef struct i2sdf_exchange {
  int (*allreduce)(void* ctx, void* buf, int64_t n, int32_t dtype, int32_t op, void* stream);
  void* ctx;
} i2sdf_exchange;
int32_t i2sdf_comm_available(void);
int i2sdf_comm_unique_id(void* out, int64_t out_bytes);
int i2sdf_comm_init_rank(const void* unique_id, int32_t nranks, int32_t rank, i2sdf_comm** out);
void i2sdf_comm_destroy(i2sdf_comm* comm);
int32_t i2sdf_comm_size(const i2sdf_comm* comm);
int32_t i2sdf_comm_rank(const i2sdf_comm* comm);
const char* i2sdf_last_comm_error(void);
int i2sdf_allreduce_grads(float* flat, int64_t n, const i2sdf_comm* comm, void* stream);
int i2sdf_allreduce_max_i32(int32_t* flags, int64_t n, const i2sdf_comm* comm, void* stream);
int i2sdf_broadcast(void* buf, int64_t bytes, int32_t root, const i2sdf_comm* comm, void* stream);
int i2sdf_comm_as_exchange(const i2sdf_comm* comm, i2sdf_exchange* out);
int i2sdf_plan_set_exchange(i2sdf_plan* plan, const i2sdf_exchange* ex, int32_t flags);

int i2sdf_adam_step(float* params, const float* grads, float* exp_avg, float* exp_avg_sq, int64_t n, double lr, double beta1,
                    double beta2, double eps, double weight_decay, int64_t step, double grad_scale, void* stream);

typedef struct i2sdf_sampler_cfg {
  float near, eps, add_tiny;
  int32_t N_samples, N_samples_eval, N_samples_extra, beta_iters, max_total_iters;
} i2sdf_sampler_cfg;

int i2sdf_error_bound(const float* z, const float* sdf, int64_t B, int32_t n, const float* beta, int64_t ldbeta,
                      const float* d_star_in, float* d_star_out, float* bound, void* stream);

int64_t i2sdf_sampler_workspace_floats(int64_t B);
int i2sdf_sample_rays(const i2sdf_plan* plan, const float* packed, const float* params, const i2sdf_sampler_cfg* cfg,
                      const float* cam, const float* dirs, int64_t B, int32_t training, const float* t_lin, const float* u_more,
                      const float* u_final, int64_t ldu_final, const int32_t* extra_tab, const float* strat_u,
                      const int32_t* extra_idx, const int32_t* eik_idx, int32_t force_iters, float* workspace, float* z_out,
                      int64_t ldz, float* z_eik, int32_t* iters_out, void* stream);


int i2sdf_light_forward(const i2sdf_plan* plan, const float* packed, const float* feat, int64_t M, int64_t Mp, float* lm, float* hl,
                        void* stream);
int i2sdf_light_backward(const i2sdf_plan* plan, const float* packed, const float* lm, const float* lm_bar, const float* hl, int64_t M,
                         int64_t Mp, float* gal0, float* gal_last, void* stream);


typedef struct i2sdf_loss_cfg {
  float eikonal_w, smooth_w, mask_w, depth_w, normal_w, angular_w, bubble_w, light_w;
  int32_t smooth_on;
  int32_t reserved;
  const i2sdf_exchange* exchange;
} i2sdf_loss_cfg;

int64_t i2sdf_loss_scratch_floats(void);
int i2sdf_loss_forward_backward(const i2sdf_loss_cfg* cfg, int64_t B, int64_t n_pc, const float* rgb, const float* depth,
                                const float* wsum, const float* normal, const float* grad_theta, const float* diff_norm,
                                const float* surface, const float* lmask, const float* gt_rgb, const float* gt_depth,
                                const uint8_t* depth_mask, const float* gt_normal, const uint8_t* normal_mask, const float* gt_mask,
                                const float* gt_lmask, float* scratch, float* losses, float* loss_value, float* g_rgb, float* g_depth, float* g_wsum,
                                float* g_normal, float* g_grad_theta, float* g_diff_norm, float* g_surface, float* g_lmask,
                                void* stream);

int i2sdf_eikonal_outputs_forward(const float* grad_all, int64_t B, float* grad_theta, float* diff_norm, void* stream);
int i2sdf_eikonal_outputs_backward(const float* grad_all, const float* grad_theta_bar, const float* diff_norm_bar, int64_t B,
                                   float* grad_all_bar, void* stream);

int i2sdf_extra_points(const float* cam, const float* dirs, const float* z_eik, const float* eik_pts, const float* nbr_off, int64_t B,
                       float* out, void* stream);

int i2sdf_backward_seeds(float* beta_grad, int64_t n_beta, float* sdf_bar, float* grad_bar, int64_t M_main, int64_t M_sdf,
                         const float* g_eik, int64_t n_eik, const float* g_surf, int64_t n_pc, int32_t zero_main_grad, void* stream);

int64_t i2sdf_render_loss_scratch_floats(int64_t B);
int i2sdf_render_loss_backward(const i2sdf_loss_cfg* cfg, int64_t B, int32_t n, int64_t n_pc, int64_t M_main, int64_t M_sdf, int64_t n_eik,
                               const float* beta_param, float beta_min, const float* z, int64_t ldz, const float* sdf, const float* rgb_pts,
                               const float* grad_pts, const float* dnorm, const float* nsum_save,
                               const float* rgb, const float* depth, const float* wsum, const float* normal, const float* grad_theta,
                               const float* diff_norm, const float* surface, const float* lmask,
                               const float* gt_rgb, const float* gt_depth, const uint8_t* depth_mask, const float* gt_normal,
                               const uint8_t* normal_mask, const float* gt_mask, const float* gt_lmask,
                               float* scratch, float* losses, float* loss_value,
                               float* g_rgb, float* g_depth, float* g_wsum, float* g_normal, float* g_grad_theta, float* g_diff_norm,
                               float* g_surface, float* g_lmask,
                               float* sdf_bar, float* rgb_bar, float* grad_bar, int32_t normal_term, float* lmask_bar, float* beta_grad,
                               void* stream);
int i2sdf_scale_seeds(const float* g, float* sdf_bar, int64_t n_sdf, float* grad_bar, int64_t n_grad, float* rgb_bar, int64_t n_rgb,
                      float* lmask_bar, int64_t n_lmask, const float* beta_in, float* beta_out, void* stream);

int64_t i2sdf_render_image_workspace_floats(const i2sdf_plan* plan, const i2sdf_sampler_cfg* cfg, int64_t chunk);
int i2sdf_render_image(const i2sdf_plan* plan, const float* packed, const float* params, const i2sdf_sampler_cfg* cfg,
                       const float* uv, const float* pose, int32_t pose_is_quat, const float* intrinsics, int64_t P, int64_t chunk,
                       const float* t_lin, const float* u_more, const float* u_final, const int32_t* extra_tab, float* workspace,
                       float* o_rgb, float* o_depth, float* o_wsum, float* o_normal, float* o_lmask, float* o_z, int32_t* o_iters,
                       void* stream);

#define I2SDF_GRID_ORDER_MESHGRID 0
#define I2SDF_GRID_ORDER_VOLUME 1
int64_t i2sdf_sdf_grid_workspace_floats(int64_t chunk_points);
int i2sdf_sdf_grid(const i2sdf_plan* plan, const float* packed, const float* x, const float* y, const float* z, int32_t nx,
                   int32_t ny, int32_t nz, int32_t order, const float* rot, const float* trans, int64_t first, int64_t count,
                   float* sdf_out, float* workspace, int64_t chunk_points, void* stream);

int64_t i2sdf_marching_cubes_workspace_bytes(int32_t nx, int32_t ny, int32_t nz);
int i2sdf_marching_cubes_count(const float* vol, int32_t nx, int32_t ny, int32_t nz, float level, void* workspace, int64_t* counts_out,
                               void* stream);
int i2sdf_marching_cubes_emit(const float* vol, int32_t nx, int32_t ny, int32_t nz, float level, const float* spacing,
                              const float* origin, void* workspace, float* verts, float* normals, int32_t* faces, int64_t cap_v,
                              int64_t cap_f, void* stream);

int64_t i2sdf_mesh_scan_workspace_bytes(int64_t n);
int i2sdf_mesh_status(const int32_t* status, void* stream);
int i2sdf_mesh_edge_keys(const int32_t* faces, int64_t F, int64_t n_verts, int64_t* keys, int32_t* status, void* stream);
int i2sdf_mesh_face_components(const int64_t* sorted_keys, const int64_t* perm, int64_t F, int32_t* labels, void* stream);
int i2sdf_mesh_face_areas(const float* verts, int64_t n_verts, const int32_t* faces, int64_t F, float* area, int32_t* status,
                          void* stream);
int i2sdf_mesh_cumsum_f64(const float* x, int64_t n_x, const int64_t* order, int64_t n, double* cdf, void* workspace, void* stream);
int i2sdf_mesh_largest_label(const int32_t* sorted_labels, const double* cdf, int64_t F, int64_t* best, void* stream);
int i2sdf_mesh_compact_mark(const int32_t* faces, const uint8_t* mask, int64_t F, int64_t n_verts, int32_t* fkeep, int32_t* vflag,
                            int32_t* status, void* stream);
int i2sdf_mesh_compact_gather(const float* verts, const float* normals, int64_t n_verts, const int32_t* faces, int64_t F,
                              const int32_t* fkeep, const int32_t* fscan, const int32_t* vflag, const int32_t* vscan,
                              float* out_verts, float* out_normals, int32_t* out_faces, int64_t cap_v, int64_t cap_f, void* stream);
int i2sdf_mesh_sample_surface(const float* verts, int64_t n_verts, const int32_t* faces, int64_t F, const double* cdf,
                              const float* u_face, const float* u_bary, int64_t count, float* points, int32_t* face_index,
                              int32_t* status, void* stream);

int i2sdf_points_bounds(const float* points, int64_t n, int32_t* bounds, int32_t* status, void* stream);
int i2sdf_points_voxel_keys(const float* points, int64_t n, const int32_t* bounds, double voxel_size, int64_t* keys, int32_t* status,
                            void* stream);
int i2sdf_points_voxel_heads(const int64_t* sorted_keys, int64_t n, int32_t* heads, void* stream);
int i2sdf_points_voxel_mean(const float* points, int64_t n, const int64_t* sorted_keys, const int64_t* perm, const int32_t* head_scan,
                            float* out_points, int32_t* out_counts, int64_t cap_m, void* stream);
int64_t i2sdf_points_grid_workspace_bytes(int64_t n_ref);
int i2sdf_points_grid_keys(const float* ref, int64_t n_ref, void* workspace, int64_t* keys, int32_t* status, void* stream);
int i2sdf_points_grid_build(const float* ref, int64_t n_ref, const int64_t* sorted_keys, const int64_t* perm, void* workspace,
                            float* sorted_ref, void* stream);
int i2sdf_points_nn_query(const float* query, int64_t n_query, const float* sorted_ref, int64_t n_ref, const void* workspace,
                          int32_t max_ring, float* dist, int32_t* index, int32_t* fallback_list, int32_t* status, void* stream);
int i2sdf_points_nn_fallback(const float* query, int64_t n_query, const float* ref, int64_t n_ref, const int32_t* fallback_list,
                             const int32_t* status, float* dist, int32_t* index, void* stream);
int64_t i2sdf_points_reduce_workspace_bytes(int64_t n);
int i2sdf_points_threshold_reduce(const float* dist, int64_t n, double threshold, void* workspace, double* out, void* stream);

int i2sdf_pdf_update(const float* pred, const float* target, int32_t channels, const int64_t* pixel_idx, int64_t first_pixel,
                     int64_t n, const int64_t* pointlinks, int64_t n_links, double pdf_max, double pdf_prune, float* pdf,
                     int64_t n_pdf, int32_t* n_bad, void* stream);

int i2sdf_training_draws(uint64_t seed, int64_t B, int32_t n_eval, int32_t n_samples, int32_t n_extra, int32_t max_iters,
                         int32_t n_z, float eik_radius, float nbr_half_width, float* strat_u, float* cdf_u,
                         int32_t* extra_idx, int32_t* eik_idx, float* eik_pts, float* nbr_off, void* stream);

#ifdef __cplusplus
}
#endif
#endif
```

Before: 20.60 million.

## Split weight packing for early sampler start, fuse sampler final sort, vectorize wn reduction

Weight packing now runs in two parts on the side stream. The sampler's sdf-only span is packed first with its own event, so the sampler can start while the remaining chunks are still packing. The separate sampler_final kernel is folded into the last resample iteration as an epilogue, which removes one launch and the re-read of state. The weight-norm backward reduction now loads partials as float4 with 4-way unrolling, and the bias is summed via per-lane loads plus shuffles; this adds alignment requirements that are checked at launch.

```diff
diff --git a/i2sdf_amd/csrc/mlp_fwd.hip b/i2sdf_amd/csrc/mlp_fwd.hip
--- a/i2sdf_amd/csrc/mlp_fwd.hip
+++ b/i2sdf_amd/csrc/mlp_fwd.hip
@@ -70,14 +70,15 @@
   const bool full = feat_out != nullptr;
   const unsigned grid = (unsigned)((M + PTS_PER_WG - 1) / PTS_PER_WG);
   if (!full && sdf_out != nullptr && p->sdf_fwd_bf16x3 && H == 256 && span_chunks(p->sdf, SPAN_FWD3H) > 0) {
-    const int PL = (sampler_pass && p->sampler_bf16x2 && span_chunks(p->sdf, SPAN_FWD2H) > 0) ? 2 : 3;
-    const Span s3 = span(p, packed, p->sdf, PL == 2 ? SPAN_FWD2H : SPAN_FWD3H_SDF);
+    const SpanId id = sdf_only_span(p, sampler_pass);
+    const int PL = id.from == FWD2H ? 2 : 3;
+    const Span s3 = span(p, packed, p->sdf, id);
     if (!s3.n_stages) return I2SDF_EINVAL;
     i2sdf_launch_sdf_fwd3h(s3.w, s3.n_stages, d.n_lin, d.skip_layer, points, skip_flag, M, sdf_out, PL, st);
     return i2sdf_hip_check(hipGetLastError(), "sdf_forward (bf16x3, 16-point waves) launch");
   }
   if (!full && sdf_out != nullptr && p->sdf_fwd_bf16x3 && H == 64 && span_chunks(p->sdf, SPAN_FWD3) > 0) {
-    const Span s3 = span(p, packed, p->sdf, SPAN_FWD3);
+    const Span s3 = span(p, packed, p->sdf, sdf_only_span(p, sampler_pass));
     if (!s3.n_stages) return I2SDF_EINVAL;
     i2sdf_launch_sdf_fwd3(H, s3.w, s3.n_stages, d.n_lin, d.skip_layer, points, skip_flag, M, sdf_out, grid, st);
     return i2sdf_hip_check(hipGetLastError(), "sdf_forward (bf16x3) launch");
@@ -91,7 +92,7 @@
     i2sdf_launch_train_fwd3h(a, grid, st);
     return i2sdf_hip_check(hipGetLastError(), "sdf_forward (features, bf16x3, 16-point waves) launch");
   }
-  const Span s = span(p, packed, p->sdf, full ? SPAN_FWD : SPAN_FWD_SDF);
+  const Span s = span(p, packed, p->sdf, full ? SPAN_FWD : sdf_only_span(p, sampler_pass));
   if (!s.n_stages) return I2SDF_EINVAL;
   if (full)
     launch_lds(sdf_fwd_kernel<H, F, LF, true>, grid, st, s.w, s.n_stages, d.n_lin, d.skip_layer, points, skip_flag, M, sdf_out, feat_out, ld_feat);
diff --git a/i2sdf_amd/csrc/pack.hip b/i2sdf_amd/csrc/pack.hip
--- a/i2sdf_amd/csrc/pack.hip
+++ b/i2sdf_amd/csrc/pack.hip
@@ -37,11 +37,12 @@
 
 __global__ __launch_bounds__(256) void pack_kernel(const Seg* __restrict__ segs, int n_segs, const float* __restrict__ params,
                                                     const float* __restrict__ scale, float* __restrict__ chunks,
-                                                    int64_t total_chunks) {
+                                                    int64_t first, int64_t n_chunks, int64_t skip_lo, int64_t skip_n) {
   const int64_t gid = (int64_t)blockIdx.x * 256 + threadIdx.x;
-  const int64_t chunk = gid >> 6;
+  if ((gid >> 6) >= n_chunks) return;
+  int64_t chunk = first + (gid >> 6);
+  if (chunk >= skip_lo) chunk += skip_n;
   const int lane = (int)(gid & 63);
-  if (chunk >= total_chunks) return;
   int lo = 0, hi_ = n_segs - 1;
   while (lo < hi_) {
     const int mid = (lo + hi_ + 1) >> 1;
@@ -208,16 +209,38 @@
 
 }
 
-extern "C" int i2sdf_pack_weights(const i2sdf_plan* p, const float* params, float* packed, void* stream) {
-  if (!p || !params || !packed) return I2SDF_EINVAL;
+extern "C" int i2sdf_plan_sdf_only_span(const i2sdf_plan* p, int32_t sampler_pass, int64_t* first_chunk, int64_t* n_chunks) {
+  if (!p || !first_chunk || !n_chunks) return I2SDF_EINVAL;
+  const SpanId id = sdf_only_span(p, sampler_pass != 0);
+  *first_chunk = p->sdf.mark[id.from];
+  *n_chunks = span_chunks(p->sdf, id);
+  return I2SDF_OK;
+}
+
+extern "C" int i2sdf_pack_weights_part(const i2sdf_plan* p, const float* params, float* packed, int32_t part, void* stream) {
+  if (!p || !params || !packed || part < I2SDF_PACK_ALL || part > I2SDF_PACK_REST) return I2SDF_EINVAL;
   if (!p->d_segs) return I2SDF_EHIP;
   hipStream_t st = (hipStream_t)stream;
-  RowTab tab{};
-  fill_tab(tab, p->sdf); fill_tab(tab, p->rgb);
-  if (p->light.d.n_lin) fill_tab(tab, p->light);
-  rowscale_kernel<<<cdiv(p->n_scale, 4), 256, 0, st>>>(tab, params, packed, p->n_scale);
-  const int64_t threads = p->total_chunks * 64;
-  pack_kernel<<<(unsigned)((threads + 255) / 256), 256, 0, st>>>(p->d_segs, p->n_segs, params, packed, packed + p->scale_floats,
-                                                                 p->total_chunks);
+  if (part != I2SDF_PACK_REST) {
+    RowTab tab{};
+    fill_tab(tab, p->sdf); fill_tab(tab, p->rgb);
+    if (p->light.d.n_lin) fill_tab(tab, p->light);
+    rowscale_kernel<<<cdiv(p->n_scale, 4), 256, 0, st>>>(tab, params, packed, p->n_scale);
+  }
+  const SpanId id = sdf_only_span(p, true);
+  const int64_t lo = p->sdf.mark[id.from], n = span_chunks(p->sdf, id);
+  if (lo < 0 || n < 0 || lo + n > p->total_chunks) return I2SDF_EINVAL;
+  int64_t first = 0, count = p->total_chunks, skip_lo = p->total_chunks, skip_n = 0;
+  if (part == I2SDF_PACK_FIRST) { first = lo; count = n; }
+  else if (part == I2SDF_PACK_REST) { count = p->total_chunks - n; skip_lo = lo; skip_n = n; }
+  if (count > 0) {
+    const int64_t threads = count * 64;
+    pack_kernel<<<(unsigned)((threads + 255) / 256), 256, 0, st>>>(p->d_segs, p->n_segs, params, packed, packed + p->scale_floats, first, count,
+                                                                   skip_lo, skip_n);
+  }
   return i2sdf_hip_check(hipGetLastError(), "pack_weights launch");
 }
+
+extern "C" int i2sdf_pack_weights(const i2sdf_plan* p, const float* params, float* packed, void* stream) {
+  return i2sdf_pack_weights_part(p, params, packed, I2SDF_PACK_ALL, stream);
+}
diff --git a/i2sdf_amd/csrc/plan.h b/i2sdf_amd/csrc/plan.h
--- a/i2sdf_amd/csrc/plan.h
+++ b/i2sdf_amd/csrc/plan.h
@@ -106,6 +106,12 @@
   if (n <= 0 || n % id.stage_chunks) return Span{};
   return Span{packed + p->scale_floats + np.mark[id.from] * CHUNK_FLOATS, (int)(n / id.stage_chunks)};
 }
+inline SpanId sdf_only_span(const i2sdf_plan* p, bool sampler_pass) {
+  if (p->sdf_fwd_bf16x3 && p->H == 256 && span_chunks(p->sdf, SPAN_FWD3H) > 0)
+    return (sampler_pass && p->sampler_bf16x2 && span_chunks(p->sdf, SPAN_FWD2H) > 0) ? SPAN_FWD2H : SPAN_FWD3H_SDF;
+  if (p->sdf_fwd_bf16x3 && p->H == 64 && span_chunks(p->sdf, SPAN_FWD3) > 0) return SPAN_FWD3;
+  return SPAN_FWD_SDF;
+}
 }
 
 struct PartRun {
diff --git a/i2sdf_amd/csrc/sampler.hip b/i2sdf_amd/csrc/sampler.hip
--- a/i2sdf_amd/csrc/sampler.hip
+++ b/i2sdf_amd/csrc/sampler.hip
@@ -161,6 +161,10 @@
   float* samples;
   float* beta;
   const float* u_more; const float* u_final; int64_t ldu_final;
+  int epilogue, N_extra;
+  const float* z_a; const float* z_b;
+  const int* extra_idx; const int* extra_tab; const int* eik_idx;
+  float* z_out; int64_t ldz; float* z_eik; int* iters_out;
 };
 
 template <int E>
@@ -318,6 +322,51 @@
   }
 }
 
+__device__ __forceinline__ void sampler_epilogue(const SamplerArgs& a, int iters, const float* smp, const float* zr, float* buf, int64_t ray,
+                                                 bool active, int lane) {
+  if (a.iters_out != nullptr && blockIdx.x == 0 && threadIdx.x == 0) a.iters_out[0] = iters;
+  const int N_final = a.N_final, N_extra = a.N_extra;
+  const int n_row = a.N_eval * iters;
+  const int total = N_final + 2 + N_extra;
+  for (int k = lane; k < 256; k += 64) {
+    float v = 3.0e38f;
+    if (k < N_final) v = smp[k];
+    else if (k == N_final) v = a.near;
+    else if (k == N_final + 1) v = a.far;
+    else if (k < total) {
+      const int e = k - N_final - 2;
+      int id;
+      if (a.extra_idx) id = a.extra_idx[(iters - 1) * N_extra + e];
+      else id = a.extra_tab[(iters - 1) * N_extra + e];
+      id = id < 0 ? 0 : (id > n_row - 1 ? n_row - 1 : id);
+      v = zr[id];
+    }
+    buf[k] = v;
+  }
+  __syncthreads();
+  for (int k = 2; k <= 256; k <<= 1) {
+    for (int j = k >> 1; j > 0; j >>= 1) {
+      for (int i = lane; i < 256; i += 64) {
+        const int l = i ^ j;
+        if (l > i) {
+          const float x = buf[i], y = buf[l];
+          const bool up = (i & k) == 0;
+          if ((x > y) == up) { buf[i] = y; buf[l] = x; }
+        }
+      }
+      __syncthreads();
+    }
+  }
+  if (active) {
+    for (int k = lane; k < total; k += 64) a.z_out[ray * a.ldz + k] = buf[k];
+    if (lane == 0 && a.z_eik) {
+      int id = a.eik_idx ? a.eik_idx[ray] : 0;
+      id = id < 0 ? 0 : (id > total - 1 ? total - 1 : id);
+      a.z_eik[ray] = buf[id];
+    }
+  }
+}
+
 __device__ __forceinline__ void iteration_done(const SamplerArgs& a, bool more) {
   __syncthreads();
   if (threadIdx.x == 0) {
@@ -332,11 +381,17 @@
   __shared__ float s_cdf[4][NMAX + 1];
   __shared__ float s_z[4][NMAX];
   __shared__ float s_new[4][NNEW];
-  if (a.state[ST_DONE]) return;
   const int lane = threadIdx.x & 63, wv = threadIdx.x >> 6;
   const int64_t ray = (int64_t)blockIdx.x * 4 + wv;
   const bool active = ray < a.B;
   const int64_t rc = active ? ray : a.B - 1;
+  if (a.state[ST_DONE]) {
+    if (a.epilogue) {
+      const int iters = a.state[ST_ITERS];
+      sampler_epilogue(a, iters, a.samples + rc * NNEW, ((iters & 1) ? a.z_a : a.z_b) + rc * NMAX, s_cdf[wv], ray, active, lane);
+    }
+    return;
+  }
   bool not_conv = a.state[ST_FLAG0 + a.it] != 0;
   if (a.force_iters > 0) not_conv = (a.it + 1) < a.force_iters;
   const bool more = not_conv && (a.it + 1 < a.max_iters);
@@ -345,6 +400,7 @@
   row_intervals<E>(r, lane);
   resample_step<E>(a, r, a.beta[rc], more, ray, rc, active, s_cdf, s_z, s_new, lane, wv);
   iteration_done(a, more);
+  if (a.epilogue) sampler_epilogue(a, a.it + 1, s_new[wv], s_z[wv], s_cdf[wv], ray, active, lane);
 }
 
 template <int E>
@@ -362,6 +418,7 @@
   if (active && lane == 0) a.beta[ray] = beta;
   resample_step<E>(a, r, beta, more, ray, rc, active, s_cdf, s_z, s_new, lane, wv);
   iteration_done(a, more);
+  if (a.epilogue) sampler_epilogue(a, a.it + 1, s_new[wv], s_z[wv], s_cdf[wv], ray, active, lane);
 }
 
 __global__ __launch_bounds__(256) void sampler_init_kernel(int64_t B, int N, const float* __restrict__ t_lin, const float* __restrict__ strat_u,
@@ -397,60 +454,6 @@
   if (lane == 0) beta[ray] = sqrtf((1.0f / (4.0f * logf(eps + 1.0f))) * acc);
 }
 
-__global__ __launch_bounds__(256) void sampler_final_kernel(int64_t B, const int* __restrict__ state, int N_eval, const float* z_a,
-                                                             const float* z_b, const float* __restrict__ samples, int N_final, int N_extra,
-                                                             const int* __restrict__ extra_idx, const int* __restrict__ extra_tab,
-                                                             float near, float far, const int* __restrict__ eik_idx, float* __restrict__ z_out,
-                                                             int64_t ldz, float* __restrict__ z_eik, int* __restrict__ iters_out) {
-  __shared__ float buf[4][256];
-  const int lane = threadIdx.x & 63, wv = threadIdx.x >> 6;
-  const int64_t ray = (int64_t)blockIdx.x * 4 + wv;
-  const bool active = ray < B;
-  const int64_t rc = active ? ray : B - 1;
-  const int iters = state[ST_ITERS];
-  if (iters_out != nullptr && blockIdx.x == 0 && threadIdx.x == 0) iters_out[0] = iters;
-  const int n_row = N_eval * iters;
-  const float* zr = ((iters & 1) ? z_a : z_b) + rc * NMAX;
-  const int total = N_final + 2 + N_extra;
-  for (int k = lane; k < 256; k += 64) {
-    float v = 3.0e38f;
-    if (k < N_final) v = samples[rc * NNEW + k];
-    else if (k == N_final) v = near;
-    else if (k == N_final + 1) v = far;
-    else if (k < total) {
-      const int e = k - N_final - 2;
-      int id;
-      if (extra_idx) id = extra_idx[(iters - 1) * N_extra + e];
-      else id = extra_tab[(iters - 1) * N_extra + e];
-      id = id < 0 ? 0 : (id > n_row - 1 ? n_row - 1 : id);
-      v = zr[id];
-    }
-    buf[wv][k] = v;
-  }
-  __syncthreads();
-  for (int k = 2; k <= 256; k <<= 1) {
-    for (int j = k >> 1; j > 0; j >>= 1) {
-      for (int i = lane; i < 256; i += 64) {
-        const int l = i ^ j;
-        if (l > i) {
-          const float x = buf[wv][i], y = buf[wv][l];
-          const bool up = (i & k) == 0;
-          if ((x > y) == up) { buf[wv][i] = y; buf[wv][l] = x; }
-        }
-      }
-      __syncthreads();
-    }
-  }
-  if (active) {
-    for (int k = lane; k < total; k += 64) z_out[ray * ldz + k] = buf[wv][k];
-    if (lane == 0 && z_eik) {
-      int id = eik_idx ? eik_idx[ray] : 0;
-      id = id < 0 ? 0 : (id > total - 1 ? total - 1 : id);
-      z_eik[ray] = buf[wv][id];
-    }
-  }
-}
-
 template <int E>
 __global__ __launch_bounds__(256) void error_bound_kernel(int64_t B, int n, const float* __restrict__ z, const float* __restrict__ sdf,
                                                            const float* __restrict__ beta, int64_t ldbeta, const float* __restrict__ d_star_in,
@@ -530,7 +533,8 @@
                                  int64_t ldz, float* z_eik, int32_t* iters_out, void* stream) {
   if (B == 0) return I2SDF_OK;
   if (!p || !packed || !params || !sc || !cam || !dirs || !t_lin || !u_more || !u_final || !workspace || !z_out || B < 0) return I2SDF_EINVAL;
-  if (sc->N_samples_eval > NNEW || sc->N_samples > NNEW || sc->N_samples_eval * sc->max_total_iters > NMAX || sc->max_total_iters > 12)
+  if (sc->N_samples_eval > NNEW || sc->N_samples > NNEW || sc->N_samples_eval * sc->max_total_iters > NMAX || sc->max_total_iters > 12 ||
+      sc->max_total_iters < 1)
     return I2SDF_EINVAL;
   if (sc->N_samples + 2 + sc->N_samples_extra > 256 || ldz < sc->N_samples + 2 + sc->N_samples_extra) return I2SDF_EINVAL;
   if (training && (!strat_u || (sc->N_samples_extra > 0 && !extra_idx))) return I2SDF_EINVAL;
@@ -569,6 +573,11 @@
     a.idx = even ? iB : iA; a.idx_nxt = even ? iA : iB;
     a.sdf_new = sdf_new; a.samples = samples; a.beta = beta;
     a.u_more = u_more; a.u_final = u_final; a.ldu_final = ldu_final;
+    if (it == n_it - 1) {
+      a.epilogue = 1; a.N_extra = sc->N_samples_extra; a.z_a = zA; a.z_b = zB;
+      a.extra_idx = training ? (const int*)extra_idx : nullptr; a.extra_tab = (const int*)extra_tab; a.eik_idx = (const int*)eik_idx;
+      a.z_out = z_out; a.ldz = ldz; a.z_eik = z_eik; a.iters_out = iters_out;
+    }
     const int E = cdiv(a.n, 64);
     int xrc = I2SDF_OK;
     switch (E) {
@@ -585,8 +594,5 @@
     }
     if (xrc) return xrc;
   }
-  sampler_final_kernel<<<grid, 256, 0, st>>>(B, state, sc->N_samples_eval, zA, zB, samples, sc->N_samples, sc->N_samples_extra,
-                                             training ? (const int*)extra_idx : nullptr, (const int*)extra_tab, near, far, (const int*)eik_idx, z_out, ldz,
-                                             z_eik, iters_out);
   return i2sdf_hip_check(hipGetLastError(), "sample_rays launch");
 }
diff --git a/i2sdf_amd/csrc/wgrad.hip b/i2sdf_amd/csrc/wgrad.hip
--- a/i2sdf_amd/csrc/wgrad.hip
+++ b/i2sdf_amd/csrc/wgrad.hip
@@ -784,7 +784,10 @@
 
 __global__ __launch_bounds__(256) void wn_backward_kernel(WnTab tab, const float* __restrict__ params, const float* __restrict__ partials,
                                                            int n_chunks, int64_t chunk_stride, float* __restrict__ grad) {
-  __shared__ float s_dw[4][5 * 64];
+  constexpr int MAXC = 5;
+  constexpr int MAXV = 2;
+  constexpr int UNR = 4;
+  __shared__ float s_dw[4][MAXV * 256];
   __shared__ float s_b[4];
   const int row = blockIdx.x;
   const int lane = threadIdx.x & 63, wv = threadIdx.x >> 6;
@@ -794,31 +797,48 @@
   const int r = row - y.row0;
   const int brow = r < y.rsplit ? r : r - y.rsplit + y.rbase;
   const float* v = params + y.off_v + (int64_t)r * y.cols;
-  constexpr int MAXC = 5;
-  const float* src[MAXC];
-  float sacc[MAXC];
-#pragma unroll
-  for (int q = 0; q < MAXC; ++q) {
-    const int c = lane + 64 * q;
-    const int kp = c < y.valid0 ? c : y.split + (c - y.base1);
-    src[q] = (c < y.cols) ? partials + y.blk_off + (int64_t)brow * y.ldo + kp : nullptr;
-    sacc[q] = 0.f;
-  }
-#pragma unroll 2
-  for (int ch = wv; ch < n_chunks; ch += 4) {
-    float x[MAXC];
-#pragma unroll
-    for (int q = 0; q < MAXC; ++q) x[q] = src[q] ? src[q][ch * chunk_stride] : 0.f;
-#pragma unroll
-    for (int q = 0; q < MAXC; ++q) sacc[q] += x[q];
-  }
-#pragma unroll
-  for (int q = 0; q < MAXC; ++q) s_dw[wv][lane + 64 * q] = sacc[q];
-  if (lane == 0) {
+  const float* bs = partials + y.bias_blk_off + brow;
+  const int n_mine = n_chunks > wv ? (n_chunks - wv + 3) / 4 : 0;
+  float bval = (lane < n_mine) ? bs[(int64_t)(wv + 4 * lane) * chunk_stride] : 0.f;
+  const float* src[MAXV];
+  f32x4 sacc[MAXV];
+#pragma unroll
+  for (int q = 0; q < MAXV; ++q) {
+    const int kp = 4 * (lane + 64 * q);
+    src[q] = (kp < y.ldo) ? partials + y.blk_off + (int64_t)brow * y.ldo + kp : nullptr;
+    sacc[q] = f32x4{0.f, 0.f, 0.f, 0.f};
+  }
+  int ch = wv;
+  for (; ch + 4 * (UNR - 1) < n_chunks; ch += 4 * UNR) {
+    f32x4 x[UNR][MAXV];
+#pragma unroll
+    for (int u = 0; u < UNR; ++u)
+#pragma unroll
+      for (int q = 0; q < MAXV; ++q)
+        x[u][q] = src[q] ? *reinterpret_cast<const f32x4*>(src[q] + (int64_t)(ch + 4 * u) * chunk_stride) : f32x4{0.f, 0.f, 0.f, 0.f};
+#pragma unroll
+    for (int u = 0; u < UNR; ++u)
+#pragma unroll
+      for (int q = 0; q < MAXV; ++q) sacc[q] += x[u][q];
+  }
+  for (; ch < n_chunks; ch += 4) {
+    f32x4 x[MAXV];
+#pragma unroll
+    for (int q = 0; q < MAXV; ++q) x[q] = src[q] ? *reinterpret_cast<const f32x4*>(src[q] + (int64_t)ch * chunk_stride) : f32x4{0.f, 0.f, 0.f, 0.f};
+#pragma unroll
+    for (int q = 0; q < MAXV; ++q) sacc[q] += x[q];
+  }
+#pragma unroll
+  for (int q = 0; q < MAXV; ++q)
+    if (src[q]) *reinterpret_cast<f32x4*>(&s_dw[wv][4 * (lane + 64 * q)]) = sacc[q];
+  {
     float b = 0.f;
-    const float* bs = partials + y.bias_blk_off + brow;
-    for (int ch = wv; ch < n_chunks; ch += 4) b += bs[ch * chunk_stride];
-    s_b[wv] = b;
+    for (int base = 0; base < n_mine; base += 64) {
+      if (base > 0) bval = (base + lane < n_mine) ? bs[(int64_t)(wv + 4 * (base + lane)) * chunk_stride] : 0.f;
+      const int m = n_mine - base < 64 ? n_mine - base : 64;
+      for (int i = 0; i < m; ++i) b += __shfl(bval, i);
+    }
+    if (lane == 0) s_b[wv] = b;
   }
   __syncthreads();
   if (wv != 0) return;
@@ -829,7 +849,8 @@
     const int c = lane + 64 * q;
     dw[q] = 0.f; vv[q] = 0.f;
     if (c < y.cols) {
-      dw[q] = (s_dw[0][c] + s_dw[1][c] + s_dw[2][c] + s_dw[3][c]) * y.mult;
+      const int kp = c < y.valid0 ? c : y.split + (c - y.base1);
+      dw[q] = (s_dw[0][kp] + s_dw[1][kp] + s_dw[2][kp] + s_dw[3][kp]) * y.mult;
       vv[q] = v[c];
       dot = fmaf(dw[q], vv[q], dot);
       nrm2 = fmaf(vv[q], vv[q], nrm2);
@@ -1087,6 +1108,9 @@
   if (Mm > 0 && tb->gar) fill_wn(tab, p->rgb, 1, row0);
   if (has_light) fill_wn(tab, p->light, 2, row0);
   tab.n_rows = row0;
+  if (p->wgrad_floats % 4 != 0 || ((uintptr_t)partials & 15) != 0) return I2SDF_EINVAL;
+  for (int i = 0; i < tab.n; ++i)
+    if (tab.l[i].ldo % 4 != 0 || tab.l[i].ldo > 512 || tab.l[i].blk_off % 4 != 0 || tab.l[i].cols > 320) return I2SDF_EINVAL;
   wn_backward_kernel<<<row0, 256, 0, st>>>(tab, params, partials, n_chunks, p->wgrad_floats, grad_flat);
   return i2sdf_hip_check(hipGetLastError(), "weight_grads launch");
 }
diff --git a/i2sdf_amd/engine.py b/i2sdf_amd/engine.py
--- a/i2sdf_amd/engine.py
+++ b/i2sdf_amd/engine.py
@@ -25,7 +25,7 @@
         self.pack_floats = int(self._lib.i2sdf_plan_pack_floats(plan))
         self.wgrad_floats = int(self._lib.i2sdf_plan_wgrad_floats(plan))
         self.packed = torch.zeros(self.pack_floats, dtype=torch.float32, device=self.device)
-        self._pack_stream, self._pack_event, self._pack_readers = None, None, {}
+        self._pack_stream, self._pack_events, self._pack_first, self._pack_readers = None, None, None, {}
         self.F = cfg.feature_size
         wide = cfg.sdf.hidden == 256 and cfg.feature_size == 256
         self.set_sdf_forward_bf16x3(bool(cfg.bf16x3 and cfg.sdf.hidden % 64 == 0))
@@ -84,7 +84,7 @@
         for name in L.SIGNATURES:
             fn = getattr(self._lib, name)
             if name in ("i2sdf_sdf_forward", "i2sdf_sdf_forward_grad", "i2sdf_rgb_forward", "i2sdf_rgb_backward", "i2sdf_sdf_backward",
-                        "i2sdf_weight_grads", "i2sdf_sample_rays", "i2sdf_composite_forward", "i2sdf_composite_backward", "i2sdf_pack_weights",
+                        "i2sdf_weight_grads", "i2sdf_sample_rays", "i2sdf_composite_forward", "i2sdf_composite_backward", "i2sdf_pack_weights", "i2sdf_pack_weights_part",
                         "i2sdf_ray_setup", "i2sdf_light_forward", "i2sdf_light_backward"):
                 fn = _Timed(fn, name)
             setattr(self._timed_lib, name, fn)
@@ -122,19 +122,32 @@
             if st != cur:
                 side.wait_stream(st)
         with torch.cuda.stream(side):
-            L.check(self._lib.i2sdf_pack_weights(self._plan, L.ptr(flat_params), L.ptr(self.packed), L.stream_ptr()), "i2sdf_pack_weights")
-            self._pack_event = side.record_event()
+            L.check(self._lib.i2sdf_pack_weights_part(self._plan, L.ptr(flat_params), L.ptr(self.packed), L.PACK_FIRST, L.stream_ptr()),
+                    "i2sdf_pack_weights_part")
+            ev_first = side.record_event()
+            L.check(self._lib.i2sdf_pack_weights_part(self._plan, L.ptr(flat_params), L.ptr(self.packed), L.PACK_REST, L.stream_ptr()),
+                    "i2sdf_pack_weights_part")
+            self._pack_events = (ev_first, side.record_event())
+        self._pack_first = self._sdf_only_span(True)
         flat_params.record_stream(side)
         self._pack_readers = {}
 
-    def _pk(self):
-        ev = self._pack_event
-        if ev is not None:
+    def _sdf_only_span(self, sampler_pass: bool):
+        lo, n = C.c_int64(), C.c_int64()
+        L.check(self._lib.i2sdf_plan_sdf_only_span(self._plan, 1 if sampler_pass else 0, C.byref(lo), C.byref(n)), "i2sdf_plan_sdf_only_span")
+        return (lo.value, n.value)
+
+    def _pk(self, sdf_only=None):
+        evs = self._pack_events
+        if evs is not None:
+            level = 2
+            if sdf_only is not None and self._sdf_only_span(sdf_only == "sampler") == self._pack_first:
+                level = 1
             cur = torch.cuda.current_stream(self.packed.device)
             readers = self.__dict__.setdefault("_pack_readers", {})
-            if cur not in readers:
-                cur.wait_event(ev)
-                readers[cur] = True
+            if readers.get(cur, 0) < level:
+                cur.wait_event(evs[level - 1])
+                readers[cur] = level
         return L.ptr(self.packed)
 
     def set_sdf_forward_bf16x3(self, on: bool):
@@ -268,7 +281,7 @@
         M = pts.shape[0]
         sdf = torch.empty(M, 1, dtype=torch.float32, device=pts.device)
         feat = torch.empty(M, self.F, dtype=torch.float32, device=pts.device) if want_features else None
-        L.check(self._lib.i2sdf_sdf_forward(self._plan, self._pk(), L.ptr(pts), M, L.ptr(sdf), L.ptr(feat), self.F,
+        L.check(self._lib.i2sdf_sdf_forward(self._plan, self._pk(None if want_features else "points"), L.ptr(pts), M, L.ptr(sdf), L.ptr(feat), self.F,
                                             L.stream_ptr()), "i2sdf_sdf_forward")
         return (sdf, feat) if want_features else sdf
 
@@ -452,7 +465,7 @@
             u_final, ldu = self.u_final, 0
         ex, ek = i32(extra_idx), i32(eik_idx)
         su = None if strat_u is None else strat_u.contiguous()
-        L.check(self._lib.i2sdf_sample_rays(self._plan, self._pk(), L.ptr(flat_params), C.byref(self._scfg), L.ptr(cam.contiguous()),
+        L.check(self._lib.i2sdf_sample_rays(self._plan, self._pk("sampler"), L.ptr(flat_params), C.byref(self._scfg), L.ptr(cam.contiguous()),
                                              L.ptr(dirs.contiguous()), B, 1 if training else 0, L.ptr(self.t_lin), L.ptr(self.u_more),
                                              L.ptr(u_final), ldu, L.ptr(self.extra_tab), L.ptr(su), L.ptr(ex), L.ptr(ek), force_iters,
                                              L.ptr(ws), L.ptr(z_out), self.n_z, L.ptr(z_eik), L.ptr(iters), L.stream_ptr()),
@@ -514,7 +527,7 @@
         out = torch.empty(count, dtype=torch.float32, device=dev)
         host = lambda v, n: None if v is None else (C.c_float * n)(*[float(a) for a in torch.as_tensor(v, dtype=torch.float32).reshape(-1).tolist()])
         r, t = host(rot, 9), host(trans, 3)
-        L.check(self._lib.i2sdf_sdf_grid(self._plan, self._pk(), L.ptr(x), L.ptr(y), L.ptr(z), nx, ny, nz, int(order),
+        L.check(self._lib.i2sdf_sdf_grid(self._plan, self._pk("points"), L.ptr(x), L.ptr(y), L.ptr(z), nx, ny, nz, int(order),
                                          C.cast(r, C.c_void_p) if r is not None else None, C.cast(t, C.c_void_p) if t is not None else None,
                                          int(first), int(count), L.ptr(out), L.ptr(ws), chunk, L.stream_ptr()), "i2sdf_sdf_grid")
         return out
diff --git a/i2sdf_amd/lib.py b/i2sdf_amd/lib.py
--- a/i2sdf_amd/lib.py
+++ b/i2sdf_amd/lib.py
@@ -46,6 +46,7 @@
 XCHG_F32, XCHG_I32 = 0, 1
 XCHG_SUM, XCHG_AVG, XCHG_MAX = 0, 1, 2
 DP_GLOBAL_SAMPLER = 1
+PACK_ALL, PACK_FIRST, PACK_REST = 0, 1, 2
 COMM_UNIQUE_ID_BYTES = 128
 
 
@@ -96,6 +97,8 @@
     "i2sdf_plan_pack_floats": (_I64, [_P]),
     "i2sdf_plan_wgrad_floats": (_I64, [_P]),
     "i2sdf_pack_weights": (C.c_int, [_P, _P, _P, _P]),
+    "i2sdf_pack_weights_part": (C.c_int, [_P, _P, _P, _I32, _P]),
+    "i2sdf_plan_sdf_only_span": (C.c_int, [_P, _I32, _P, _P]),
     "i2sdf_sdf_forward": (C.c_int, [_P, _P, _P, _I64, _P, _P, _I64, _P]),
     "i2sdf_sdf_forward_grad": (C.c_int, [_P] * 6 + [_I64, _I32, _I64, _I64, _I64] + [_P] * 7),
     "i2sdf_rgb_forward": (C.c_int, [_P, _P, _P, _I32, _P, _I64, _I64, _P, _P, _P, _P]),
diff --git a/include/i2sdf.h b/include/i2sdf.h
--- a/include/i2sdf.h
+++ b/include/i2sdf.h
@@ -73,6 +73,11 @@
 int64_t i2sdf_plan_wgrad_floats(const i2sdf_plan* plan);
 
 int i2sdf_pack_weights(const i2sdf_plan* plan, const float* params, float* packed, void* stream);
+#define I2SDF_PACK_ALL 0
+#define I2SDF_PACK_FIRST 1
+#define I2SDF_PACK_REST 2
+int i2sdf_pack_weights_part(const i2sdf_plan* plan, const float* params, float* packed, int32_t part, void* stream);
+int i2sdf_plan_sdf_only_span(const i2sdf_plan* plan, int32_t sampler_pass, int64_t* first_chunk, int64_t* n_chunks);
 
 int i2sdf_sdf_forward(const i2sdf_plan* plan, const float* packed, const float* points, int64_t M,
                       float* sdf_out, float* feat_out, int64_t ld_feat, void* stream);
```

New measurement: 20.34 million. -1.3%, worse.
